# cxy1997/3D_adapt_auto_driving

Hardware: AMD Instinct MI355X
Metric: KITTI scenes/s end-to-end eval_rcnn (joint RPN+RCNN, synthetic 16384-pt scenes) (higher is better)
Workload: dtype f32; 1 GPU; BASELINE.json configs[2]: full PointRCNN RPN+RCNN inference, default.yaml shapes, random-init weights, batch=8 synthetic KITTI scenes x 16384 pts per GPU per step; scene=synth.scenes (SURVEY 8d: uniform clutter + ground + 10 dense cars), parallelism=scene-sharded x1, one final all_gather of detections, detections_gathered=652455, batch_slots=14, look_ahead=12, steps_per_launch=2

## Files before the change

3d_adapt_auto_driving_amd/csrc/layer_tile.hpp:

```cpp
#pragma once
#include "common.hpp"
#include "segmax.hpp"

namespace prcnn {

typedef float f32x4 __attribute__((ext_vector_type(4)));
constexpr int PL_ROWS = 64;
constexpr int PL_LD = 128 + 4;

constexpr int PL_MAX_BATCH = 4;
struct PLProblem {
    const unsigned int *hdr; long rows_host; int K, N; const float *A; long lda; const float *W; const float *bias; int do_relu;
    float *out; long ldo; const unsigned int *rowinfo; const int *tilecloud; int m, out_col, n_store;
    int lds_pool;
    const float *addG; const int *addIdx; const float *addW; int add_n, add_m; long add_ldg;
};
struct PLBatch { PLProblem p[PL_MAX_BATCH]; };

#define PL_LOAD_W(dst, kk)                                                                              \
    _Pragma("unroll") for (int s = 0; s < 64; ++s)                                                      \
        dst[s] = __uint_as_float(__builtin_amdgcn_raw_buffer_load_b32(wrs, lane_off, (unsigned int)((kk) + s) * row_bytes, 0));
#define PL_VM_DRAIN __builtin_amdgcn_s_waitcnt(0x0F70);
#define PL_SADD(x, y) asm volatile("s_add_u32 %0, %0, %1" : "+s"(x) : "s"(y) : "scc");

#define PL_FETCH_TILE(T, NI, soff)                                                                      \
    _Pragma("unroll") for (int i = 0; i < (NI); ++i)                                                    \
        *reinterpret_cast<f32x4 *>((T) + (r0 + 8 * i) * PL_LD + 4 * chunk) = __builtin_bit_cast(        \
            f32x4, __builtin_amdgcn_raw_buffer_load_b128(ars, a_lane, (soff) + (unsigned int)(8 * i) * a_row_bytes, 0));

#define PL_BOTH_HALVES(...) __VA_ARGS__
#define PL_ONE_HALF(...)
#define PL_MFMA(H2, wf, c, s)                                                                           \
    acc0 = __builtin_amdgcn_mfma_f32_32x32x2f32(a0.c, wf[4 * g + s], acc0, 0, 0, 0);                    \
    H2(acc1 = __builtin_amdgcn_mfma_f32_32x32x2f32(a1.c, wf[4 * g + s], acc1, 0, 0, 0);)
#define PL_STAGE_HEAD(T, H2)                                                                            \
    const float *a0p = (T) + j * PL_LD + 64 * h;                                                        \
    H2(const float *a1p = (T) + (32 + j) * PL_LD + 64 * h;)                                             \
    f32x4 a0 = *reinterpret_cast<const f32x4 *>(a0p);                                                   \
    H2(f32x4 a1 = *reinterpret_cast<const f32x4 *>(a1p);)
#define PL_STAGE_GROUPS(wf, H2, STATE, SIDE)                                                            \
    {                                                                                                   \
        STATE                                                                                           \
        _Pragma("unroll") for (int g = 0; g < 16; ++g) {                                                \
            f32x4 n0_ = a0;                                                                             \
            H2(f32x4 n1_ = a1;)                                                                         \
            if (g < 15) {                                                                               \
                n0_ = *reinterpret_cast<const f32x4 *>(a0p + 4 * (g + 1));                              \
                H2(n1_ = *reinterpret_cast<const f32x4 *>(a1p + 4 * (g + 1));)                          \
            }                                                                                           \
            __builtin_amdgcn_sched_barrier(0);                                                          \
            PL_MFMA(H2, wf, x, 0)                                                                       \
            SIDE                                                                                        \
            PL_MFMA(H2, wf, y, 1) PL_MFMA(H2, wf, z, 2) PL_MFMA(H2, wf, w, 3)                           \
            a0 = n0_;                                                                                   \
            H2(a1 = n1_;)                                                                               \
        }                                                                                               \
    }
#define PL_STAGE_SIDE(T, wf, STATE, SIDE) { PL_STAGE_HEAD(T, PL_BOTH_HALVES) PL_STAGE_GROUPS(wf, PL_BOTH_HALVES, STATE, SIDE) }
#define PL_FENCE __builtin_amdgcn_sched_barrier(0);
#define PL_NO_SIDE
#define PL_STAGE(T, wf) PL_STAGE_SIDE(T, wf, PL_NO_SIDE, PL_NO_SIDE)
#define PL_NEXT_PANEL_STATE(kn)                                                                         \
    f32x4 ar[8];                                                                                        \
    unsigned int wo_ = (unsigned int)(kn) * row_bytes;                                                  \
    unsigned int ao_ = (unsigned int)(kn) * 4u;                                                         \
    const unsigned int a8_ = 8u * a_row_bytes;
#define PL_NEXT_PANEL(TN, wn, ARS, LOFF)                                                                \
    if (g < 8) {                                                                                        \
        ar[g] = __builtin_bit_cast(f32x4, __builtin_amdgcn_raw_buffer_load_b128((ARS), a_lane, ao_, 0)); \
        PL_SADD(ao_, a8_)                                                                               \
    } else                                                                                              \
        *reinterpret_cast<f32x4 *>((TN) + (r0 + 8 * (g - 8)) * PL_LD + 4 * chunk) = ar[g - 8];          \
    _Pragma("unroll") for (int q = 0; q < 6; ++q)                                                       \
        if (6 * g + q < 64) {                                                                           \
            wn[6 * g + q] = __uint_as_float(__builtin_amdgcn_raw_buffer_load_b32(wrs, (LOFF), wo_, 0)); \
            PL_SADD(wo_, row_bytes)                                                                     \
        }                                                                                               \
    PL_FENCE
#define PL_STAGE_PREFETCH_X(T, TN, wf, wn, kn, ARS, LOFF) PL_STAGE_SIDE(T, wf, PL_NEXT_PANEL_STATE(kn), PL_NEXT_PANEL(TN, wn, ARS, LOFF))
#define PL_STAGE_PREFETCH(T, TN, wf, wn, kn) PL_STAGE_PREFETCH_X(T, TN, wf, wn, kn, ars, lane_off)
#define PL_NEXT_ROWS(TN, soff)                                                                          \
    if (g < 8)                                                                                          \
        ar[g] = __builtin_bit_cast(f32x4, __builtin_amdgcn_raw_buffer_load_b128(                        \
            ars, a_lane, (soff) + (unsigned int)(8 * g) * a_row_bytes, 0));                             \
    else                                                                                                \
        *reinterpret_cast<f32x4 *>((TN) + (r0 + 8 * (g - 8)) * PL_LD + 4 * chunk) = ar[g - 8];          \
    PL_FENCE
#define PL_STAGE_ROWS(T, TN, wf, soff) PL_STAGE_SIDE(T, wf, f32x4 ar[8];, PL_NEXT_ROWS(TN, soff))

#define PL32_NEXT_PANEL(TN, wn, kn)                                                                     \
    if (g < 4)                                                                                          \
        ar[g] = __builtin_bit_cast(f32x4, __builtin_amdgcn_raw_buffer_load_b128(                        \
            ars, a_lane, (unsigned int)(8 * g) * a_row_bytes + (unsigned int)(kn) * 4u, 0));            \
    else if (g >= 8 && g < 12)                                                                          \
        *reinterpret_cast<f32x4 *>((TN) + (r0 + 8 * (g - 8)) * PL_LD + 4 * chunk) = ar[g - 8];          \
    _Pragma("unroll") for (int q = 0; q < 6; ++q)                                                       \
        if (6 * g + q < 64)                                                                             \
            wn[6 * g + q] = __uint_as_float(__builtin_amdgcn_raw_buffer_load_b32(                       \
                wrs, lane_off, (unsigned int)((kn) + 6 * g + q) * row_bytes, 0));

__device__ __forceinline__ void pl_store_direct(const f32x16 &acc0, const f32x16 &acc1, float bcol, int do_relu, float *out, long ldo,
                                                long t, long rows, unsigned int col)
{
    const int h = (threadIdx.x & 63) >> 5;
    const long left = rows - t * PL_ROWS;
    const unsigned int o_row_bytes = (unsigned int)ldo * 4u;
    const __amdgpu_buffer_rsrc_t ors = __builtin_amdgcn_make_buffer_rsrc(
        (void *)(out + t * PL_ROWS * ldo), 0, (int)((left < PL_ROWS ? left : PL_ROWS) * (long)o_row_bytes), 0x00020000);
    const unsigned int o_lane = (unsigned int)(4 * h) * o_row_bytes + col * 4u;
#pragma unroll
    for (int r = 0; r < 16; ++r) {
        const unsigned int so = (unsigned int)((r & 3) + 8 * (r >> 2)) * o_row_bytes;
        const float v0 = acc0[r] + bcol, v1 = acc1[r] + bcol;
        __builtin_amdgcn_raw_buffer_store_b32(__float_as_uint(do_relu ? fmaxf(v0, 0.f) : v0), ors, o_lane, so, 0);
        __builtin_amdgcn_raw_buffer_store_b32(__float_as_uint(do_relu ? fmaxf(v1, 0.f) : v1), ors, o_lane, so + 32u * o_row_bytes, 0);
    }
}

template <int TR>
__device__ __forceinline__ void pl_store_rows(const float *tile, long t, long rows, int n0, const PLProblem &pb, bool with_add)
{
    const int chunk = threadIdx.x & 31, r0 = threadIdx.x >> 5;
    float *out = pb.out;
    const long ldo = pb.ldo;
    const int n_store = pb.n_store;
#pragma unroll
    for (int i = 0; i < TR / 8; ++i) {
        const int row = r0 + 8 * i;
        const long g = t * TR + row;
        if (g < rows) {
            const int c0 = n0 + 4 * chunk;
            float4 v = *reinterpret_cast<const float4 *>(tile + row * PL_LD + 4 * chunk);
            if (with_add) {
                const int *ix = pb.addIdx + g * 3;
                const float *wv = pb.addW + g * 3;
                const long cb = (g / pb.add_n) * (long)pb.add_m;
                const float4 g0 = *reinterpret_cast<const float4 *>(pb.addG + (cb + ix[0]) * pb.add_ldg + c0);
                const float4 g1 = *reinterpret_cast<const float4 *>(pb.addG + (cb + ix[1]) * pb.add_ldg + c0);
                const float4 g2 = *reinterpret_cast<const float4 *>(pb.addG + (cb + ix[2]) * pb.add_ldg + c0);
                const float w0 = wv[0], w1 = wv[1], w2 = wv[2];
                v.x = __fadd_rn(v.x, __fadd_rn(__fadd_rn(__fmul_rn(w0, g0.x), __fmul_rn(w1, g1.x)), __fmul_rn(w2, g2.x)));
                v.y = __fadd_rn(v.y, __fadd_rn(__fadd_rn(__fmul_rn(w0, g0.y), __fmul_rn(w1, g1.y)), __fmul_rn(w2, g2.y)));
                v.z = __fadd_rn(v.z, __fadd_rn(__fadd_rn(__fmul_rn(w0, g0.z), __fmul_rn(w1, g1.z)), __fmul_rn(w2, g2.z)));
                v.w = __fadd_rn(v.w, __fadd_rn(__fadd_rn(__fmul_rn(w0, g0.w), __fmul_rn(w1, g1.w)), __fmul_rn(w2, g2.w)));
                if (pb.do_relu) v = make_float4(fmaxf(v.x, 0.f), fmaxf(v.y, 0.f), fmaxf(v.z, 0.f), fmaxf(v.w, 0.f));
            }
            if (c0 + 4 <= n_store && (ldo & 3) == 0) {
                *reinterpret_cast<float4 *>(out + g * ldo + c0) = v;
            } else {
                const float e[4] = {v.x, v.y, v.z, v.w};
#pragma unroll
                for (int q = 0; q < 4; ++q)
                    if (c0 + q < n_store) out[g * ldo + c0 + q] = e[q];
            }
        }
    }
}

template <bool SEGMAX>
__device__ __forceinline__ void pl_epilogue(const f32x16 &acc0, const f32x16 &acc1, float *tile, int *ctr, long t, long rows, int n0,
                                            const PLProblem &pb)
{
    const int tid = threadIdx.x, lane = tid & 63, w = tid >> 6, j = lane & 31, h = lane >> 5;
    const int chunk = tid & 31;
    const float bcol = pb.bias[n0 + 32 * w + j];
    if constexpr (SEGMAX) {
        if (tid < PL_ROWS) {
            const unsigned int info = pb.rowinfo[t * PL_ROWS + tid];
            ctr[tid] = pb.tilecloud[t] * pb.m + (int)(info >> 16);
        }
        __syncthreads();
        const int myc = ctr[lane], prevc = ctr[lane ? lane - 1 : 0];
        const unsigned long long start = __ballot(lane == 0 || myc != prevc);
        if (!pb.lds_pool || __popcll(start) <= PK_LDS_MIN) {
            pk_segmented_max(acc0, acc1, ctr, start, h, pb.out, (int)pb.ldo, pb.out_col + n0 + 32 * w + j, bcol);
        } else {
            const float4 bias4 = *reinterpret_cast<const float4 *>(pb.bias + n0 + 4 * chunk);
            pk_park(acc0, acc1, tile, PL_LD, 32 * w + j, h);
            lds_barrier();
            pk_segmented_max_lds(tile, PL_LD, ctr, tid, pb.out, (int)pb.ldo, pb.out_col + n0, bias4);
        }
    } else {
        const bool with_add = pb.addG != nullptr;
        const int do_relu = pb.do_relu;
        __syncthreads();
#pragma unroll
        for (int r = 0; r < 16; ++r) {
            const int row = (r & 3) + 8 * (r >> 2) + 4 * h;
            const float v0 = acc0[r] + bcol, v1 = acc1[r] + bcol;
            tile[row * PL_LD + 32 * w + j] = (do_relu && !with_add) ? fmaxf(v0, 0.f) : v0;
            tile[(32 + row) * PL_LD + 32 * w + j] = (do_relu && !with_add) ? fmaxf(v1, 0.f) : v1;
        }
        __syncthreads();
        pl_store_rows<PL_ROWS>(tile, t, rows, n0, pb, with_add);
    }
}

}
```

3d_adapt_auto_driving_amd/csrc/packed_layer.hip:

```cpp
#include "layer_tile.hpp"
#include <cstdlib>

namespace prcnn {

#define PL_LOAD_A(dst, kk)                                                                              \
    _Pragma("unroll") for (int i = 0; i < 8; ++i) {                                                     \
        long g = t * PL_ROWS + r0 + 8 * i;                                                              \
        if (g >= rows) g = rows - 1;    \
        dst[i] = *reinterpret_cast<const f32x4 *>(pb.A + g * pb.lda + (kk) + 4 * chunk);               \
    }
#define PL_STORE_A(src)                                                                                 \
    _Pragma("unroll") for (int i = 0; i < 8; ++i)                                                       \
        *reinterpret_cast<f32x4 *>(tile + (r0 + 8 * i) * PL_LD + 4 * chunk) = src[i];

template <bool SEGMAX>
__global__ __launch_bounds__(256, 2) void packed_layer_kernel(const PLBatch bt)
{
    const PLProblem pb = bt.p[blockIdx.z];
    __shared__ float tile[PL_ROWS * PL_LD];
    __shared__ int ctr[PL_ROWS];
    const long t = blockIdx.x;
    const long rows = pb.hdr ? (long)pb.hdr[0] * PL_ROWS : pb.rows_host;
    const int n0 = blockIdx.y * 128;
    if (t * PL_ROWS >= rows || n0 >= pb.n_store) return;
    const int tid = threadIdx.x, lane = tid & 63, w = tid >> 6, j = lane & 31, h = lane >> 5;
    const int chunk = tid & 31, r0 = tid >> 5;
    const int K = pb.K, N = pb.N;
    f32x16 acc0 = {0}, acc1 = {0};
    const __amdgpu_buffer_rsrc_t wrs = __builtin_amdgcn_make_buffer_rsrc((void *)pb.W, 0, K * N * 4, 0x00020000);
    const unsigned int row_bytes = (unsigned int)N * 4u;
    const unsigned int lane_off = ((unsigned int)(64 * h) * (unsigned int)N + (unsigned int)(n0 + 32 * w + j)) * 4u;
    for (int k0 = 0; k0 < K; k0 += 128) {
        float wf[64];
        f32x4 ar[8];
        PL_LOAD_W(wf, k0)
        PL_LOAD_A(ar, k0)
        if (k0) __syncthreads();
        PL_STORE_A(ar)
        __syncthreads();
        PL_STAGE(tile, wf)
    }
    pl_epilogue<SEGMAX>(acc0, acc1, tile, ctr, t, rows, n0, pb);
}

template <bool SEGMAX>
__global__ __launch_bounds__(256, 2) void packed_layer_pipe_kernel(const PLBatch bt)
{
    const PLProblem pb = bt.p[blockIdx.z];
    __shared__ float tiles[2 * PL_ROWS * PL_LD];
    __shared__ int ctr[PL_ROWS];
    const long t = blockIdx.x;
    const long rows = pb.hdr ? (long)pb.hdr[0] * PL_ROWS : pb.rows_host;
    const int n0 = blockIdx.y * 128;
    if (t * PL_ROWS >= rows || n0 >= pb.n_store) return;
    const int tid = threadIdx.x, lane = tid & 63, j = lane & 31, h = lane >> 5;
    const int w = __builtin_amdgcn_readfirstlane(tid >> 6);
    const int chunk = tid & 31, r0 = tid >> 5;
    const int K = pb.K, N = pb.N;
    f32x16 acc0 = {0}, acc1 = {0};
    const __amdgpu_buffer_rsrc_t wrs = __builtin_amdgcn_make_buffer_rsrc((void *)pb.W, 0, K * N * 4, 0x00020000);
    const unsigned int row_bytes = (unsigned int)N * 4u;
    const unsigned int lane_off = ((unsigned int)(64 * h) * (unsigned int)N + (unsigned int)(n0 + 32 * w + j)) * 4u;
    const long left = rows - t * PL_ROWS;
    const unsigned int a_row_bytes = (unsigned int)pb.lda * 4u;
    const __amdgpu_buffer_rsrc_t ars = __builtin_amdgcn_make_buffer_rsrc(
        (void *)(pb.A + t * PL_ROWS * pb.lda), 0, (int)((left < PL_ROWS ? left : PL_ROWS) * (long)a_row_bytes), 0x00020000);
    const unsigned int a_lane = (unsigned int)r0 * a_row_bytes + 16u * chunk;
    float wa[64], wb[64];
    PL_LOAD_W(wa, 0)
    PL_FETCH_TILE(tiles, 8, 0)
    const int np = K >> 7;
    for (int p = 0; p < np; ++p) {
        PL_VM_DRAIN
        lds_barrier();
        const float *T = tiles + (p & 1) * (PL_ROWS * PL_LD);
        float *TN = tiles + ((p + 1) & 1) * (PL_ROWS * PL_LD);
        if (p + 1 < np) {
            PL_STAGE_PREFETCH(T, TN, wa, wb, (p + 1) * 128)
#pragma unroll
            for (int s = 0; s < 64; ++s) wa[s] = wb[s];
        } else {
            PL_STAGE(T, wa)
        }
    }
    if constexpr (!SEGMAX) {
        if (n0 + 128 <= pb.n_store && !pb.addG) {
            pl_store_direct(acc0, acc1, pb.bias[n0 + 32 * w + j], pb.do_relu, pb.out, pb.ldo, t, rows, (unsigned int)(n0 + 32 * w + j));
            return;
        }
    }
    pl_epilogue<SEGMAX>(acc0, acc1, tiles, ctr, t, rows, n0, pb);
}

template <bool ADD>
__global__ __launch_bounds__(256, 2) void packed_layer_persist_kernel(const PLProblem pb, unsigned int *__restrict__ ticket)
{
    __shared__ float tiles[2 * PL_ROWS * PL_LD];
    __shared__ unsigned int s_item[2];
    const int tid = threadIdx.x, lane = tid & 63, j = lane & 31, h = lane >> 5;
    const int w = __builtin_amdgcn_readfirstlane(tid >> 6);
    const int chunk = tid & 31, r0 = tid >> 5;
    const long rows = pb.rows_host;
    const int K = pb.K, N = pb.N;
    const unsigned int col_blocks = (unsigned int)(N >> 7);
    const unsigned int n_tiles = (unsigned int)((rows + PL_ROWS - 1) / PL_ROWS);
    const unsigned int n_items = n_tiles * col_blocks;
    const __amdgpu_buffer_rsrc_t wrs = __builtin_amdgcn_make_buffer_rsrc((void *)pb.W, 0, K * N * 4, 0x00020000);
    const unsigned int row_bytes = (unsigned int)N * 4u;
    const unsigned int a_row_bytes = (unsigned int)pb.lda * 4u;
    const unsigned int a_lane = (unsigned int)r0 * a_row_bytes + 16u * chunk;
    const int np = K >> 7;
    auto tile_rsrc = [&](unsigned int t) __attribute__((always_inline)) {
        const long left = rows - (long)t * PL_ROWS;
        return __builtin_amdgcn_make_buffer_rsrc((void *)(pb.A + (long)t * PL_ROWS * pb.lda), 0,
                                                 (int)((left < PL_ROWS ? left : PL_ROWS) * (long)a_row_bytes), 0x00020000);
    };
    auto loff = [&](unsigned int cb) __attribute__((always_inline)) {
        return ((unsigned int)(64 * h) * (unsigned int)N + (cb * 128u + (unsigned int)(32 * w + j))) * 4u;
    };
    unsigned int item = blockIdx.x;
    unsigned int t = item / col_blocks, cb = item - t * col_blocks;
    __amdgpu_buffer_rsrc_t ars = tile_rsrc(t);
    unsigned int lane_off = loff(cb);
    float wa[64], wb[64];
    PL_LOAD_W(wa, 0)
    PL_FETCH_TILE(tiles, 8, 0)
    int pp = 0;
    int slot = 1;
    PL_VM_DRAIN
    while (true) {
        f32x16 acc0 = {0}, acc1 = {0};
        unsigned int next = 0xffffffffu, tn = 0, cbn = 0, drawn = 0;
        const float bcol = pb.bias[(int)cb * 128 + 32 * w + j];
        for (int p = 0; p < np; ++p, ++pp) {
            if (p > 0) {
                PL_VM_DRAIN
                if (p == 1 && tid == 0) s_item[slot] = drawn;
            }
            lds_barrier();
            if (p == 0 && tid == 0) drawn = gridDim.x + atomicAdd(ticket, 1u);
            const float *T = tiles + (pp & 1) * (PL_ROWS * PL_LD);
            float *TN = tiles + ((pp + 1) & 1) * (PL_ROWS * PL_LD);
            if (p + 1 < np) {
                PL_STAGE_PREFETCH(T, TN, wa, wb, (p + 1) * 128)
#pragma unroll
                for (int s2 = 0; s2 < 64; ++s2) wa[s2] = wb[s2];
            } else {
                next = s_item[slot];
                if (next < n_items) {
                    tn = next / col_blocks; cbn = next - tn * col_blocks;
                    const __amdgpu_buffer_rsrc_t ars_n = tile_rsrc(tn);
                    const unsigned int loff_n = loff(cbn);
                    PL_STAGE_PREFETCH_X(T, TN, wa, wb, 0, ars_n, loff_n)
#pragma unroll
                    for (int s2 = 0; s2 < 64; ++s2) wa[s2] = wb[s2];
                    PL_VM_DRAIN
                } else {
                    PL_STAGE(T, wa)
                }
            }
        }
        if constexpr (ADD) {
            float *Tlast = tiles + ((pp - 1) & 1) * (PL_ROWS * PL_LD);
            pl_epilogue<false>(acc0, acc1, Tlast, nullptr, (long)t, rows, (int)cb * 128, pb);
            __syncthreads();
        } else {
            pl_store_direct(acc0, acc1, bcol, pb.do_relu, pb.out, pb.ldo, (long)t, rows, cb * 128u + (unsigned int)(32 * w + j));
        }
        if (next >= n_items) break;
        t = tn; cb = cbn;
        ars = tile_rsrc(t);
        lane_off = loff(cb);
        slot ^= 1;
    }
    if (tid == 0) ticket_release(ticket);
}

__global__ __launch_bounds__(256, 2) void packed_layer_stream_kernel(const PLProblem pb)
{
    __shared__ float tiles[2 * PL_ROWS * PL_LD];
    const int tid = threadIdx.x, lane = tid & 63, j = lane & 31, h = lane >> 5;
    const int w = __builtin_amdgcn_readfirstlane(tid >> 6);
    const int chunk = tid & 31, r0 = tid >> 5;
    const int n0 = blockIdx.y * 128;
    const long rows = pb.rows_host;
    const int N = pb.N;
    const long ntiles = (rows + PL_ROWS - 1) / PL_ROWS;
    long t = blockIdx.x;
    if (t >= ntiles || n0 >= pb.n_store) return;
    const __amdgpu_buffer_rsrc_t wrs = __builtin_amdgcn_make_buffer_rsrc((void *)pb.W, 0, 128 * N * 4, 0x00020000);
    const unsigned int row_bytes = (unsigned int)N * 4u;
    const unsigned int lane_off = ((unsigned int)(64 * h) * (unsigned int)N + (unsigned int)(n0 + 32 * w + j)) * 4u;
    float wf[64];
    PL_LOAD_W(wf, 0)
    const unsigned int a_row_bytes = (unsigned int)pb.lda * 4u;
    const __amdgpu_buffer_rsrc_t ars = __builtin_amdgcn_make_buffer_rsrc((void *)pb.A, 0, (int)(rows * (long)a_row_bytes), 0x00020000);
    const unsigned int a_lane = (unsigned int)r0 * a_row_bytes + 16u * chunk;
    PL_FETCH_TILE(tiles, 8, (unsigned int)(t * PL_ROWS) * a_row_bytes)
    const float bcol = pb.bias[n0 + 32 * w + j];
    const bool direct = n0 + 128 <= pb.n_store && !pb.addG;
    PL_VM_DRAIN
    for (int it = 0;; ++it) {
        lds_barrier();
        float *T = tiles + (it & 1) * (PL_ROWS * PL_LD);
        float *TN = tiles + ((it + 1) & 1) * (PL_ROWS * PL_LD);
        const long tn = t + gridDim.x;
        f32x16 acc0 = {0}, acc1 = {0};
        if (tn < ntiles) {
            const unsigned int soff = (unsigned int)(tn * PL_ROWS) * a_row_bytes;
            PL_STAGE_ROWS(T, TN, wf, soff)
        } else {
            PL_STAGE(T, wf)
        }
        if (direct) {
            pl_store_direct(acc0, acc1, bcol, pb.do_relu, pb.out, pb.ldo, t, rows, (unsigned int)(n0 + 32 * w + j));
        } else {
            pl_epilogue<false>(acc0, acc1, T, nullptr, t, rows, n0, pb);
            __syncthreads();
        }
        if (tn >= ntiles) break;
        t = tn;
    }
}

__global__ __launch_bounds__(256, 2) void packed_layer_pipe32_kernel(const PLBatch bt)
{
    const PLProblem pb = bt.p[blockIdx.z];
    const long rows = pb.rows_host;
    const int K = pb.K, N = pb.N;
    constexpr int R = 32;
    __shared__ float tiles[2 * R * PL_LD];
    const long t = blockIdx.x;
    const int n0 = blockIdx.y * 128;
    if (t * R >= rows || n0 >= pb.n_store) return;
    const int tid = threadIdx.x, lane = tid & 63, j = lane & 31, h = lane >> 5;
    const int w = __builtin_amdgcn_readfirstlane(tid >> 6);
    const int chunk = tid & 31, r0 = tid >> 5;
    f32x16 acc0 = {0};
    const __amdgpu_buffer_rsrc_t wrs = __builtin_amdgcn_make_buffer_rsrc((void *)pb.W, 0, K * N * 4, 0x00020000);
    const unsigned int row_bytes = (unsigned int)N * 4u;
    const unsigned int lane_off = ((unsigned int)(64 * h) * (unsigned int)N + (unsigned int)(n0 + 32 * w + j)) * 4u;
    const long left = rows - t * R;
    const unsigned int a_row_bytes = (unsigned int)pb.lda * 4u;
    const __amdgpu_buffer_rsrc_t ars =
        __builtin_amdgcn_make_buffer_rsrc((void *)(pb.A + t * R * pb.lda), 0, (int)((left < R ? left : R) * (long)a_row_bytes), 0x00020000);
    const unsigned int a_lane = (unsigned int)r0 * a_row_bytes + 16u * chunk;
    float wa[64], wb[64];
    PL_LOAD_W(wa, 0)
    PL_FETCH_TILE(tiles, R / 8, 0)
    const int np = K >> 7;
    for (int p = 0; p < np; ++p) {
        PL_VM_DRAIN
        lds_barrier();
        const float *T = tiles + (p & 1) * (R * PL_LD);
        float *TN = tiles + ((p + 1) & 1) * (R * PL_LD);
        PL_STAGE_HEAD(T, PL_ONE_HALF)
        if (p + 1 < np) {
            PL_STAGE_GROUPS(wa, PL_ONE_HALF, f32x4 ar[4];, PL32_NEXT_PANEL(TN, wb, (p + 1) * 128) PL_FENCE)
#pragma unroll
            for (int s = 0; s < 64; ++s) wa[s] = wb[s];
        } else {
            PL_STAGE_GROUPS(wa, PL_ONE_HALF, PL_NO_SIDE, PL_FENCE)
        }
    }
    const float bcol = pb.bias[n0 + 32 * w + j];
    const int do_relu = pb.do_relu;
    __syncthreads();
#pragma unroll
    for (int r = 0; r < 16; ++r) {
        const float v = acc0[r] + bcol;
        tiles[((r & 3) + 8 * (r >> 2) + 4 * h) * PL_LD + 32 * w + j] = do_relu ? fmaxf(v, 0.f) : v;
    }
    __syncthreads();
    pl_store_rows<R>(tiles, t, rows, n0, pb, false);
}

}

using namespace prcnn;

namespace {
enum PLForm { PL_ONE, PL_PIPE, PL_PIPE32, PL_STREAM, PL_PERSIST };
struct PLPlan { PLForm form; long gx; int gy; };
long env_long(const char *v, long dflt) { return v ? atol(v) : dflt; }

PLPlan pl_plan(const PLProblem &p, long tiles, bool segmax, bool single)
{
    static const long stream_min = env_long(getenv("PRCNN_PL_STREAM_MIN"), 512), stream_cap = env_long(getenv("PRCNN_PL_STREAM_CAP"), 512),
                      persist_min = env_long(getenv("PRCNN_PL_PERSIST_MIN"), 256);
    const int col_blocks = (p.n_store + 127) / 128;
    const long items = tiles * col_blocks;
    const bool host_plain = !p.hdr && !segmax;
    if (p.K == 128) {
        if (host_plain && items >= stream_min && p.rows_host * p.lda * 4 < (1L << 31)) {
            const long cap = stream_cap / col_blocks > 0 ? stream_cap / col_blocks : 1;
            return {PL_STREAM, tiles < cap ? tiles : cap, col_blocks};
        }
        return {PL_ONE, tiles, col_blocks};
    }
    if (host_plain && !p.addG && items < 256) return {PL_PIPE32, (p.rows_host + 31) / 32, col_blocks};
    if (host_plain && single && p.n_store == p.N && items > stream_cap && items >= persist_min)
        return {PL_PERSIST, items < stream_cap ? items : stream_cap, 1};
    return {PL_PIPE, tiles, col_blocks};
}

int pl_launch(PLForm form, const PLBatch &bt, int k, long gx, int gy, bool segmax, hipStream_t st, const char *what)
{
    const dim3 grid((unsigned)gx, gy, k), wg(256);
    switch (form) {
    case PL_ONE:
        if (segmax) hipLaunchKernelGGL(packed_layer_kernel<true>, grid, wg, 0, st, bt);
        else hipLaunchKernelGGL(packed_layer_kernel<false>, grid, wg, 0, st, bt);
        break;
    case PL_PIPE:
        if (segmax) hipLaunchKernelGGL(packed_layer_pipe_kernel<true>, grid, wg, 0, st, bt);
        else hipLaunchKernelGGL(packed_layer_pipe_kernel<false>, grid, wg, 0, st, bt);
        break;
    case PL_PIPE32: hipLaunchKernelGGL(packed_layer_pipe32_kernel, grid, wg, 0, st, bt); break;
    case PL_STREAM: hipLaunchKernelGGL(packed_layer_stream_kernel, grid, wg, 0, st, bt.p[0]); break;
    case PL_PERSIST: {
        unsigned int *ticket = next_ticket(st);
        if (!ticket) { set_error("%s: cannot set up the item ticket", what); return PRCNN_ELAUNCH; }
        if (bt.p[0].addG) hipLaunchKernelGGL(packed_layer_persist_kernel<true>, grid, wg, 0, st, bt.p[0], ticket);
        else hipLaunchKernelGGL(packed_layer_persist_kernel<false>, grid, wg, 0, st, bt.p[0], ticket);
        break;
    }
    }
    return check_launch(what);
}

PLProblem pl_problem(const prcnn_layer_problem &q, bool segmax)
{
    PLProblem p = {};
    p.hdr = q.hdr; p.rows_host = q.rows; p.K = q.K; p.N = q.N; p.A = q.A; p.lda = q.lda; p.W = q.W; p.bias = q.bias;
    p.do_relu = segmax ? 1 : q.relu; p.out = q.out; p.ldo = q.ldo; p.n_store = segmax ? q.N : q.n_store;
    if (segmax) {
        p.rowinfo = q.rowinfo; p.tilecloud = q.tilecloud; p.m = q.m; p.out_col = q.out_col;
        p.lds_pool = (((uintptr_t)q.out | (uintptr_t)q.bias) & 15) == 0 && (q.ldo & 3) == 0 && (q.out_col & 3) == 0;
    }
    return p;
}
}

extern "C" int prcnn_packed_layer_batch(int nprob, const prcnn_layer_problem *pr, int segmax, void *stream)
{
    PRCNN_REQUIRE(nprob >= 0 && nprob <= PL_MAX_BATCH && (nprob == 0 || pr), "packed_layer: 0..%d problems", PL_MAX_BATCH);
    hipStream_t st = (hipStream_t)stream;
    const char *what = segmax ? "packed_layer_segmax" : "packed_layer";
    PLBatch bt;
    long tiles_of[PL_MAX_BATCH];
    int k = 0;
    for (int i = 0; i < nprob; ++i) {
        const prcnn_layer_problem &q = pr[i];
        PRCNN_REQUIRE(q.K > 0 && q.N > 0 && q.K % 128 == 0 && q.N % 128 == 0, "packed_layer: K=%d, N=%d must be multiples of 128", q.K, q.N);
        PRCNN_REQUIRE(q.lda >= q.K && q.lda % 4 == 0, "packed_layer: bad leading dimension of A");
        long tiles;
        if (segmax) {
            PRCNN_REQUIRE(q.b >= 0 && q.m >= 0 && q.max_tiles >= 0 && q.out_col >= 0 && q.ldo >= q.out_col + q.N, "packed_layer_segmax: bad layout");
            if ((long)q.b * q.m == 0) continue;
            PRCNN_REQUIRE(q.A && q.W && q.bias && q.rowinfo && q.tilecloud && q.hdr && q.out, "packed_layer_segmax: null pointer");
            PRCNN_REQUIRE(((uintptr_t)q.A & 15) == 0 && q.max_tiles <= 0x7fffffffL, "packed_layer_segmax: alignment / size");
            if (!q.out_is_zero && hipMemset2DAsync(q.out + q.out_col, (size_t)q.ldo * sizeof(float), 0, (size_t)q.N * sizeof(float),
                                                    (size_t)q.b * q.m, st) != hipSuccess) {
                set_error("packed_layer_segmax: cannot zero the output slice");
                return PRCNN_ELAUNCH;
            }
            tiles = q.max_tiles;
        } else {
            PRCNN_REQUIRE(q.n_store >= 1 && q.n_store <= q.N && q.ldo >= q.n_store, "packed_layer: n_store=%d outside 1..N (or ldo too small)", q.n_store);
            tiles = q.hdr ? q.max_tiles : (q.rows + PL_ROWS - 1) / PL_ROWS;
            PRCNN_REQUIRE(tiles >= 0 && tiles <= 0x7fffffffL && q.rows >= 0, "packed_layer: bad row count");
            if (tiles > 0) {
                PRCNN_REQUIRE(q.A && q.W && q.bias && q.out, "packed_layer: null pointer");
                PRCNN_REQUIRE(((uintptr_t)q.A & 15) == 0 && (((uintptr_t)q.out & 15) == 0 || (q.ldo & 3) != 0), "packed_layer: 16-byte alignment required");
            }
        }
        if (tiles == 0) continue;
        tiles_of[k] = tiles;
        bt.p[k++] = pl_problem(q, segmax);
    }
    if (k == 0) return PRCNN_OK;
    PLPlan plan[PL_MAX_BATCH];
    bool together = true;
    long gx = 0;
    int gy = 0;
    for (int i = 0; i < k; ++i) {
        plan[i] = pl_plan(bt.p[i], tiles_of[i], segmax, k == 1);
        together = together && plan[i].form == plan[0].form && (plan[i].form == PL_ONE || plan[i].form == PL_PIPE || plan[i].form == PL_PIPE32);
        if (plan[i].gx > gx) gx = plan[i].gx;
        if (plan[i].gy > gy) gy = plan[i].gy;
    }
    if (together || k == 1) return pl_launch(plan[0].form, bt, k, gx, gy, segmax, st, what);
    for (int i = 0; i < k; ++i) {
        PLBatch one;
        one.p[0] = bt.p[i];
        const int rc = pl_launch(plan[i].form, one, 1, plan[i].gx, plan[i].gy, segmax, st, what);
        if (rc != PRCNN_OK) return rc;
    }
    return PRCNN_OK;
}

extern "C" int prcnn_packed_layer(const unsigned int *hdr, long rows, long max_tiles, int K, int N, int n_store, const float *A,
                                  long lda, const float *W, const float *bias, int relu, float *out, long ldo, void *stream)
{
    prcnn_layer_problem q = {};
    q.hdr = hdr; q.rows = rows; q.max_tiles = max_tiles; q.K = K; q.N = N; q.n_store = n_store; q.A = A; q.lda = lda; q.W = W;
    q.bias = bias; q.relu = relu; q.out = out; q.ldo = ldo;
    return prcnn_packed_layer_batch(1, &q, 0, stream);
}

extern "C" int prcnn_packed_layer_segmax(int b, int m, long max_tiles, int K, int N, const float *A, long lda, const float *W,
                                         const float *bias, const unsigned int *rowinfo, const int *tilecloud,
                                         const unsigned int *hdr, float *out, int out_stride, int out_col, int out_is_zero, void *stream)
{
    prcnn_layer_problem q = {};
    q.hdr = hdr; q.max_tiles = max_tiles; q.K = K; q.N = N; q.n_store = N; q.A = A; q.lda = lda; q.W = W; q.bias = bias; q.relu = 1;
    q.out = out; q.ldo = out_stride; q.b = b; q.m = m; q.rowinfo = rowinfo; q.tilecloud = tilecloud; q.out_col = out_col;
    q.out_is_zero = out_is_zero;
    return prcnn_packed_layer_batch(1, &q, 1, stream);
}


extern "C" int prcnn_packed_layer_interp(long rows, int K, int N, const float *A, long lda, const float *W, const float *bias, int relu,
                                         float *out, long ldo, int n_per_cloud, int m_known, const float *G, long ldg, const int *idx,
                                         const float *weight, void *stream)
{
    PRCNN_REQUIRE(rows >= 0 && K > 0 && N > 0 && K % 128 == 0 && N % 128 == 0, "packed_layer_interp: K=%d, N=%d must be multiples of 128", K, N);
    PRCNN_REQUIRE(lda >= K && lda % 4 == 0 && ldo >= N && ldo % 4 == 0 && ldg >= N && ldg % 4 == 0, "packed_layer_interp: bad leading dimensions");
    PRCNN_REQUIRE(n_per_cloud >= 1 && m_known >= 1 && rows % n_per_cloud == 0, "packed_layer_interp: rows must be whole clouds");
    if (rows == 0) return PRCNN_OK;
    PRCNN_REQUIRE(A && W && bias && out && G && idx && weight, "packed_layer_interp: null pointer");
    PRCNN_REQUIRE((((uintptr_t)A | (uintptr_t)out | (uintptr_t)G) & 15) == 0, "packed_layer_interp: 16-byte alignment required");
    const long tiles = (rows + PL_ROWS - 1) / PL_ROWS;
    PRCNN_REQUIRE(tiles <= 0x7fffffffL, "packed_layer_interp: too many rows");
    prcnn_layer_problem q = {};
    q.rows = rows; q.K = K; q.N = N; q.n_store = N; q.A = A; q.lda = lda; q.W = W; q.bias = bias; q.relu = relu; q.out = out; q.ldo = ldo;
    PLBatch bt;
    PLProblem &p = bt.p[0] = pl_problem(q, false);
    p.addG = G; p.addIdx = idx; p.addW = weight; p.add_n = n_per_cloud; p.add_m = m_known; p.add_ldg = ldg;
    const PLPlan plan = pl_plan(p, tiles, false, true);
    return pl_launch(plan.form, bt, 1, plan.gx, plan.gy, false, (hipStream_t)stream, "packed_layer_interp");
}
```

3d_adapt_auto_driving_amd/csrc/sa_wide.hpp:

```cpp
#pragma once
#include "common.hpp"

namespace prcnn {

typedef float f32x4 __attribute__((ext_vector_type(4)));

constexpr int SW_R = 32;
constexpr int SW_LD = 128 + 4;
constexpr int SW_PANEL = SW_R * SW_LD;

__device__ __forceinline__ void sw_segmented_max(const f32x16 &acc, const int *ctr, unsigned int start, int h, float *__restrict__ out,
                                                 int out_stride, int col, float bias)
{
    auto rowof = [](int q) { return (q & 3) + 8 * (q >> 2); };
    auto upto = [](int row) { return row >= 31 ? 0xffffffffu : ((2u << row) - 1u); };
    auto flush = [&](int row, float v) {
        atomicMax(reinterpret_cast<int *>(out + (long)ctr[row] * out_stride + col), __float_as_int(fmaxf(v + bias, 0.f)));
    };
    float cur = acc[0];
#pragma unroll
    for (int q = 1; q < 16; ++q) {
        const float v = acc[q];
        const int prev = rowof(q - 1), row = rowof(q);
        const unsigned int m0 = upto(row) & ~upto(prev), m1 = upto(row + 4) & ~upto(prev + 4);
        const bool b0 = (start & m0) != 0, b1 = (start & m1) != 0;
        if (b0 | b1) {
            if (h ? b1 : b0) {
                flush(prev + 4 * h, cur);
                cur = v;
            } else {
                cur = fmax_raw(cur, v);
            }
        } else {
            cur = fmax_raw(cur, v);
        }
    }
    flush(rowof(15) + 4 * h, cur);
}

#define SW_VM_DRAIN __builtin_amdgcn_s_waitcnt(0x0F70);
#define SW_STAGE(T, wf, wn, RS, VOFF, SOFF, RB, FIRST)                                                    \
    {                                                                                                     \
        const float *ap = (T) + j * SW_LD + 64 * h;                                                       \
        f32x4 a = *reinterpret_cast<const f32x4 *>(ap);                                                   \
        _Pragma("unroll") for (int g = 0; g < 16; ++g) {                                                  \
            f32x4 nx = a;                                                                                 \
            if (g < 15) nx = *reinterpret_cast<const f32x4 *>(ap + 4 * (g + 1));                          \
            __builtin_amdgcn_sched_barrier(0);                                                            \
            if ((FIRST) && g == 0) {                                                                      \
                const f32x16 zero = {0};                                                                  \
                acc = __builtin_amdgcn_mfma_f32_32x32x2f32(a.x, wf[0], zero, 0, 0, 0);                    \
            } else {                                                                                      \
                acc = __builtin_amdgcn_mfma_f32_32x32x2f32(a.x, wf[4 * g + 0], acc, 0, 0, 0);             \
            }                                                                                             \
            _Pragma("unroll") for (int q = 0; q < 6; ++q)       \
                if (6 * g + q < 64)                                                                       \
                    wn[6 * g + q] = __uint_as_float(__builtin_amdgcn_raw_buffer_load_b32(                 \
                        RS, VOFF, (SOFF) + (unsigned int)(6 * g + q) * (RB), 0));                         \
            __builtin_amdgcn_sched_barrier(0);                                                            \
            acc = __builtin_amdgcn_mfma_f32_32x32x2f32(a.y, wf[4 * g + 1], acc, 0, 0, 0);                 \
            acc = __builtin_amdgcn_mfma_f32_32x32x2f32(a.z, wf[4 * g + 2], acc, 0, 0, 0);                 \
            acc = __builtin_amdgcn_mfma_f32_32x32x2f32(a.w, wf[4 * g + 3], acc, 0, 0, 0);                 \
            a = nx;                                                                                       \
        }                                                                                                 \
    }

}
```

3d_adapt_auto_driving_amd/csrc/sa_wide3.hip:

```cpp
#include <hip/hip_runtime.h>

#include "common.hpp"
#include "sa_wide.hpp"
#include "../../include/prcnn_hip.h"

namespace prcnn {

struct SaWide3Args {
    int n, m, c0, c1, c2, c3;
    const unsigned int *hdr;
    const float4 *rowdxyz;
    const float *F;
    const float *wxyz;
    const unsigned int *rowinfo;
    const int *tilecloud;
    const float *wcat;
    const float *b1, *b2, *b3;
    float *out;
    int out_stride, out_col;
    unsigned int *ticket;
};

struct S3Stage {
    int layer, nb, kp, kpn;
    unsigned int rb, soff;
};

__global__ __launch_bounds__(256, 2) void sa_wide3_kernel(const SaWide3Args a)
{
    extern __shared__ __align__(16) float sw_lds[];
    const int kp0 = a.c0 >> 7, kp1 = a.c1 >> 7, kp2 = a.c2 >> 7, nb3 = a.c3 >> 7;
    const int kx = kp0 > kp2 ? kp0 : kp2;
    float *X = sw_lds;
    float *A1 = sw_lds + kx * SW_PANEL;
    float4 *s_d = reinterpret_cast<float4 *>(A1 + kp1 * SW_PANEL);
    int *ctr = reinterpret_cast<int *>(s_d + SW_R);
    unsigned int *slot = reinterpret_cast<unsigned int *>(ctr + SW_R);
    float *sb1 = reinterpret_cast<float *>(slot + 2), *sb2 = sb1 + a.c1, *sb3 = sb2 + a.c2, *swx = sb3 + a.c3;
    const int tid = threadIdx.x, lane = tid & 63, j = lane & 31, h = lane >> 5;
    const int w = __builtin_amdgcn_readfirstlane(tid >> 6);
    const int chunk = tid & 31, r0 = tid >> 5;
    const bool rowcloud = a.tilecloud == nullptr;
    const long nrows = (long)a.hdr[1];
    const long units = rowcloud ? (nrows + 31) >> 5 : 2L * (long)a.hdr[0];
    const long last_row = rowcloud ? nrows - 1 : 0x7fffffffffffL;
    const int ns1 = kp0 * kp1, ns2 = kp1 * kp2, ns = ns1 + ns2 + kp2 * nb3;
    const unsigned int o2 = (unsigned int)(a.c0 * a.c1) * 4u, o3 = o2 + (unsigned int)(a.c1 * a.c2) * 4u;
    const unsigned int total = o3 + (unsigned int)(a.c2 * a.c3) * 4u;
    const __amdgpu_buffer_rsrc_t rs = __builtin_amdgcn_make_buffer_rsrc((void *)a.wcat, 0, (int)total, 0x00020000);
    const unsigned int lane_k = (unsigned int)(64 * h), lane_c = (unsigned int)(32 * w + j) * 4u;
    const unsigned int voff1 = lane_k * (unsigned int)a.c1 * 4u + lane_c, voff2 = lane_k * (unsigned int)a.c2 * 4u + lane_c,
                       voff3 = lane_k * (unsigned int)a.c3 * 4u + lane_c;
    const float4 *F4 = reinterpret_cast<const float4 *>(a.F);
    const int q0 = a.c0 >> 2;

    auto stage_of = [&](int sc) __attribute__((always_inline)) {
        S3Stage st;
        int si;
        unsigned int base;
        if (sc < ns1) { st.layer = 0; st.kpn = kp0; si = sc; st.rb = (unsigned int)a.c1 * 4u; base = 0u; }
        else if (sc < ns1 + ns2) { st.layer = 1; st.kpn = kp1; si = sc - ns1; st.rb = (unsigned int)a.c2 * 4u; base = o2; }
        else { st.layer = 2; st.kpn = kp2; si = sc - ns1 - ns2; st.rb = (unsigned int)a.c3 * 4u; base = o3; }
        st.nb = si / st.kpn;
        st.kp = si - st.nb * st.kpn;
        st.soff = base + (unsigned int)(st.kp * 128) * st.rb + (unsigned int)st.nb * 512u;
        return st;
    };

    if (tid == 0) slot[0] = atomicAdd(a.ticket, 1u);
    for (int i = tid; i < a.c1; i += 256) sb1[i] = a.b1[i];
    for (int i = tid; i < a.c2; i += 256) sb2[i] = a.b2[i];
    for (int i = tid; i < a.c3; i += 256) sb3[i] = a.b3[i];
    for (int i = tid; i < 3 * a.c1; i += 256) swx[i] = a.wxyz[i];
    __syncthreads();
    long u = __builtin_amdgcn_readfirstlane((int)slot[0]);
    if (u >= units) { if (tid == 0) ticket_release(a.ticket); return; }
    float wa[64], wb[64];
    f32x16 acc;
#pragma unroll
    for (int s = 0; s < 64; ++s) wa[s] = __uint_as_float(__builtin_amdgcn_raw_buffer_load_b32(rs, voff1, (unsigned int)s * (unsigned int)a.c1 * 4u, 0));

    for (unsigned int served = 0; u < units; ++served) {
        const long t = u >> 1;
        const long row0 = rowcloud ? u * 32 : t * 64 + 32 * (u & 1);
        {
            const int cloud = rowcloud ? 0 : a.tilecloud[t];
            unsigned int info[4];
            long prow[4];
#pragma unroll
            for (int i = 0; i < 4; ++i) {
                info[i] = a.rowinfo[min(row0 + r0 + 8 * i, last_row)];
                prow[i] = rowcloud ? (long)(info[i] >> 16) * a.n + (long)(info[i] & 0x1ffu) : (long)cloud * a.n + (long)(info[i] & 0xffffu);
            }
            if (tid == 0) slot[(served + 1) & 1] = atomicAdd(a.ticket, 1u);
            if (tid < SW_R) {
                const unsigned int wd = a.rowinfo[min(row0 + tid, last_row)];
                ctr[tid] = rowcloud ? (int)(wd >> 16) * a.m + (int)((wd >> 9) & 0x7fu) : cloud * a.m + (int)(wd >> 16);
                s_d[tid] = a.rowdxyz[min(row0 + tid, last_row)];
            }
            for (int pc = 0; pc < kp0; ++pc) {
                float4 v[4];
#pragma unroll
                for (int i = 0; i < 4; ++i) v[i] = F4[prow[i] * q0 + pc * 32 + chunk];
#pragma unroll
                for (int i = 0; i < 4; ++i) *reinterpret_cast<float4 *>(X + pc * SW_PANEL + (r0 + 8 * i) * SW_LD + 4 * chunk) = v[i];
            }
        }
        SW_VM_DRAIN
        lds_barrier();
        for (int s = 0; s < ns; s += 2) {
#pragma unroll
            for (int half = 0; half < 2; ++half) {
                const int sc = s + half;
                const S3Stage st = stage_of(sc);
                const S3Stage nst = stage_of(sc + 1 == ns ? 0 : sc + 1);
                const float *T = (st.layer == 0 ? X : (st.layer == 1 ? A1 : X)) + st.kp * SW_PANEL;
                const unsigned int voffn = nst.layer == 0 ? voff1 : (nst.layer == 1 ? voff2 : voff3);
                if (st.layer > 0 && st.kp == 0 && st.nb == 0) lds_barrier();
                if (half == 0) { SW_STAGE(T, wa, wb, rs, voffn, nst.soff, nst.rb, st.kp == 0) } else { SW_STAGE(T, wb, wa, rs, voffn, nst.soff, nst.rb, st.kp == 0) }
                SW_VM_DRAIN
                if (st.kp == st.kpn - 1) {
                    const int col = st.nb * 128 + 32 * w + j;
                    if (st.layer == 0) {
                        const float bcol = sb1[col], wxc = swx[col], wyc = swx[a.c1 + col], wzc = swx[2 * a.c1 + col];
                        float *Y = A1 + st.nb * SW_PANEL;
#pragma unroll
                        for (int r = 0; r < 16; ++r) {
                            const int row = (r & 3) + 8 * (r >> 2) + 4 * h;
                            const float4 d = s_d[row];
                            const float p = acc[r] + bcol;
                            Y[row * SW_LD + 32 * w + j] = fmaxf(fmaf(wzc, d.z, fmaf(wyc, d.y, fmaf(wxc, d.x, p))), 0.f);
                        }
                    } else if (st.layer == 1) {
                        const float bcol = sb2[col];
                        float *Y = X + st.nb * SW_PANEL;
#pragma unroll
                        for (int r = 0; r < 16; ++r) Y[((r & 3) + 8 * (r >> 2) + 4 * h) * SW_LD + 32 * w + j] = fmaxf(acc[r] + bcol, 0.f);
                    } else {
                        const int myc = ctr[j], prevc = ctr[j ? j - 1 : 0];
                        const unsigned int start = (unsigned int)__ballot(lane < 32 && (lane == 0 || myc != prevc));
                        sw_segmented_max(acc, ctr, start, h, a.out, a.out_stride, a.out_col + col, sb3[col]);
                    }
                }
            }
        }
        const long un = __builtin_amdgcn_readfirstlane((int)slot[(served + 1) & 1]);
        lds_barrier();
        u = un;
    }
    if (tid == 0) ticket_release(a.ticket);
}

}

using namespace prcnn;

static size_t sa_wide3_lds(int c0, int c1, int c2, int c3)
{
    const int kp0 = c0 / 128, kp1 = c1 / 128, kp2 = c2 / 128;
    return (size_t)((kp0 > kp2 ? kp0 : kp2) + kp1) * SW_PANEL * sizeof(float) + SW_R * sizeof(float4) + SW_R * sizeof(int) +
           2 * sizeof(unsigned int) + (size_t)(c1 + c2 + c3 + 3 * c1) * sizeof(float);
}

extern "C" int prcnn_sa_wide_fused3_supported(int c0, int c1, int c2, int c3)
{
    if (c0 <= 0 || c1 <= 0 || c2 <= 0 || c3 <= 0 || c0 % 128 || c1 % 128 || c2 % 128 || c3 % 128) return 0;
    const int kp0 = c0 / 128, kp1 = c1 / 128, kp2 = c2 / 128, nb3 = c3 / 128;
    if ((kp0 * kp1 + kp1 * kp2 + kp2 * nb3) % 2) return 0;
    return sa_wide3_lds(c0, c1, c2, c3) <= 96 * 1024 ? 1 : 0;
}

extern "C" int prcnn_sa_wide_fused3(int b, int n, int m, int c0, int c1, int c2, int c3, long max_tiles, const float *F, const float *wxyz,
                                    const unsigned int *rowinfo, const float *rowdxyz, const int *tilecloud, const unsigned int *hdr,
                                    const float *wcat, const float *b1, const float *b2, const float *b3, float *out, int out_stride,
                                    int out_col, int out_is_zero, void *stream)
{
    PRCNN_REQUIRE(b >= 0 && n >= 0 && m >= 0 && max_tiles >= 0, "sa_wide_fused3: bad sizes");
    PRCNN_REQUIRE(prcnn_sa_wide_fused3_supported(c0, c1, c2, c3), "sa_wide_fused3: unsupported widths %d-%d-%d-%d", c0, c1, c2, c3);
    PRCNN_REQUIRE(n <= 65536 && m <= 65536, "sa_wide_fused3: cloud too large for the 16-bit row descriptors");
    PRCNN_REQUIRE(out_stride >= out_col + c3 && out_col >= 0, "sa_wide_fused3: bad output slice");
    if ((long)b * m == 0) return PRCNN_OK;
    PRCNN_REQUIRE(F && wxyz && rowinfo && rowdxyz && hdr && wcat && b1 && b2 && b3 && out, "sa_wide_fused3: null pointer");
    PRCNN_REQUIRE(tilecloud || (n <= 512 && m <= 128 && b <= 65536), "sa_wide_fused3: a list without tilecloud holds clouds of <= 512 points, <= 128 centres");
    PRCNN_REQUIRE((((uintptr_t)F | (uintptr_t)wcat | (uintptr_t)rowdxyz) & 15) == 0, "sa_wide_fused3: 16-byte alignment required");
    hipStream_t st = (hipStream_t)stream;
    if (!out_is_zero && hipMemset2DAsync(out + out_col, (size_t)out_stride * sizeof(float), 0, (size_t)c3 * sizeof(float), (size_t)b * m, st) != hipSuccess) {
        set_error("sa_wide_fused3: cannot zero the output slice");
        return PRCNN_ELAUNCH;
    }
    if (max_tiles == 0) return PRCNN_OK;
    const size_t lds = sa_wide3_lds(c0, c1, c2, c3);
    const int rc = ensure_dynamic_lds((const void *)sa_wide3_kernel, lds, "sa_wide_fused3");
    if (rc != PRCNN_OK) return rc;
    SaWide3Args a;
    a.n = n; a.m = m; a.c0 = c0; a.c1 = c1; a.c2 = c2; a.c3 = c3; a.hdr = hdr; a.rowdxyz = (const float4 *)rowdxyz; a.F = F; a.wxyz = wxyz;
    a.rowinfo = rowinfo; a.tilecloud = tilecloud; a.wcat = wcat; a.b1 = b1; a.b2 = b2; a.b3 = b3; a.out = out; a.out_stride = out_stride;
    a.out_col = out_col;
    a.ticket = next_ticket(st);
    if (!a.ticket) { set_error("sa_wide_fused3: cannot set up the unit ticket"); return PRCNN_ELAUNCH; }
    const long units = 2 * max_tiles;
    const long grid = units < mfma_grid_cap() ? units : mfma_grid_cap();
    hipLaunchKernelGGL(sa_wide3_kernel, dim3((unsigned)grid), dim3(256), lds, st, a);
    return check_launch("sa_wide_fused3");
}
```

3d_adapt_auto_driving_amd/dropin/pointnet2_cuda.py:

```python
import ctypes
import importlib
import os
import sys

import torch

_pkg_dir = os.path.dirname(os.path.dirname(os.path.abspath(__file__)))
if os.path.dirname(_pkg_dir) not in sys.path:
    sys.path.insert(0, os.path.dirname(_pkg_dir))
_lib = importlib.import_module(os.path.basename(_pkg_dir) + "._lib")
IS_HIP_EXTENSION = True


def _chk(dtype, *tensors):
    for t in tensors:
        if not t.is_cuda:
            raise RuntimeError("pointnet2_cuda: tensor must be a CUDA tensor")
        if not t.is_contiguous():
            raise RuntimeError("pointnet2_cuda: tensor must be contiguous")
        if t.dtype != dtype:
            raise RuntimeError("pointnet2_cuda: expected %s, got %s" % (dtype, t.dtype))


def ball_query_wrapper(b, n, m, radius, nsample, new_xyz, xyz, idx):
# ... 287 lines not shown
                                    group_all=False, hdr_c1=None, centre_rows=False):
    _chk(torch.float32, xyz); _chk(torch.int32, limit)
    b, n, _ = xyz.shape
    dev = xyz.device
    new1 = torch.empty((b, m1, 3), dtype=torch.float32, device=dev)
    if want_idx:
        idx1 = torch.empty((b, m1, ns1), dtype=torch.int32, device=dev)
        idx2 = torch.empty((b, m2, ns2), dtype=torch.int32, device=dev)
    else:
        idx1 = torch.empty((b, m1, ns1), dtype=torch.int32, device="meta")
        idx2 = torch.empty((b, m2, ns2), dtype=torch.int32, device="meta")
    rep1 = torch.empty((b, m1), dtype=torch.int32, device=dev)
    new2 = torch.empty((b, m2, 3), dtype=torch.float32, device=dev)
    rep2 = torch.empty((b, m2), dtype=torch.int32, device=dev)
    if (hdr1 is None) != (hdr2 is None):
        raise ValueError("rcnn_roi_geometry_packs: both headers or none")
    packs = []
    for idx, lim_, rep_, crep_, hdr in ((idx1, limit, None, rep1, hdr1), (idx2, None, rep1, rep2, hdr2)):
        m, ns = idx.shape[1], idx.shape[2]
        cap = (m * ns + 63) // 64
        pk = BallPack()
        pk.idx, pk.limit, pk.rep, pk.crep = idx, lim_, rep_, crep_
        pk.rowinfo = torch.empty((b * cap * 64,), dtype=torch.int32, device=dev)
        pk.rowdxyz = torch.empty((b * cap * 64, 4), dtype=torch.float32, device=dev)
        pk.tilecloud = None if row_clouds else torch.empty((b * cap,), dtype=torch.int32, device=dev)
        pk.max_tiles = b * cap
        if hdr is not None:
            _chk(torch.int32, hdr)
            if hdr.numel() != 4:
                raise ValueError("rcnn_roi_geometry_packs: a header must hold 4 int32")
        pk.hdr = hdr if hdr is not None else torch.empty((4,), dtype=torch.int32, device=dev)
        packs.append(pk)
    p1, p2 = packs
    p3 = None
    if group_all:
        if not row_clouds or (hdr3 is None) != (hdr1 is None):
            raise ValueError("rcnn_roi_geometry_packs: the GroupAll list comes in the row-carried form, its header like the others")
        p3 = BallPack()
        key = (m2, str(dev))
        if key not in _ARANGE:
            _ARANGE[key] = torch.arange(m2, dtype=torch.int32, device=dev)
        p3.idx = _ARANGE[key].view(1, 1, m2).expand(b, 1, m2)
        p3.limit, p3.rep, p3.crep = None, rep2, None
        p3.rowinfo = torch.empty((b * m2,), dtype=torch.int32, device=dev)
        p3.rowdxyz = torch.empty((b * m2, 4), dtype=torch.float32, device=dev)
        p3.tilecloud = None
        p3.max_tiles = (b * m2 + 63) // 64
        if hdr3 is not None:
            _chk(torch.int32, hdr3)
        p3.hdr = hdr3 if hdr3 is not None else torch.empty((4,), dtype=torch.int32, device=dev)
    crows = None
    if centre_rows:
        if (hdr_c1 is None) != (hdr1 is None):
            raise ValueError("rcnn_roi_geometry_packs: the centre rows' header comes like the others")
        if hdr_c1 is not None:
            _chk(torch.int32, hdr_c1)
        crows = (torch.empty((b * m1,), dtype=torch.int32, device=dev), hdr_c1 if hdr_c1 is not None else torch.empty((4,), dtype=torch.int32, device=dev))
    _lib.call("prcnn_rcnn_roi_geometry_packs", b, n, m1, float(r1), ns1, m2, float(r2), ns2, xyz.data_ptr(), limit.data_ptr(), new1.data_ptr(),
              idx1.data_ptr() if want_idx else None, rep1.data_ptr(), new2.data_ptr(), idx2.data_ptr() if want_idx else None, rep2.data_ptr(),
              p1.rowinfo.data_ptr(), p1.rowdxyz.data_ptr(), _lib.ptr(p1.tilecloud), p1.hdr.data_ptr(),
              p2.rowinfo.data_ptr(), p2.rowdxyz.data_ptr(), _lib.ptr(p2.tilecloud), p2.hdr.data_ptr(),
              None if p3 is None else p3.rowinfo.data_ptr(), None if p3 is None else p3.rowdxyz.data_ptr(),
              None if p3 is None else p3.hdr.data_ptr(), None if crows is None else crows[0].data_ptr(),
              None if crows is None else crows[1].data_ptr(), 1 if hdr1 is not None else 0, _lib.current_stream(xyz))
    return (new1, idx1, rep1, new2, idx2, rep2, p1, p2) + ((p3,) if p3 is not None else ()) + ((crows,) if crows is not None else ())


def dup_rep_wrapper(sel, n, limit=None, prev=None):
    _chk(torch.int32, sel)
    for t in (limit, prev):
        if t is not None:
            _chk(torch.int32, t)
    b, m = sel.shape
    rep = torch.empty((b, m), dtype=torch.int32, device=sel.device)
    _lib.call("prcnn_dup_rep", b, n, m, sel.data_ptr(), _lib.ptr(limit), _lib.ptr(prev), rep.data_ptr(), _lib.current_stream(sel))
    return rep


def ball_pack_groups_wrapper(idx, xyz, new_xyz, group, hdr=None):
    _chk(torch.int32, idx); _chk(torch.float32, xyz, new_xyz)
    b, m, ns = idx.shape
    if group < 1 or b % group:
        raise ValueError("ball_pack_groups: %d clouds do not split into lists of %d" % (b, group))
    lists, cap = b // group, (m * ns + 63) // 64
    L = group * cap
    rowinfo = torch.empty((lists, L * 64), dtype=torch.int32, device=idx.device)
    rowdxyz = torch.empty((lists, L * 64, 4), dtype=torch.float32, device=idx.device)
    tilecloud = torch.empty((lists, L), dtype=torch.int32, device=idx.device)
    if hdr is not None:
        _chk(torch.int32, hdr)
        if tuple(hdr.shape) != (lists, 4):
            raise ValueError("ball_pack_groups: hdr must be (lists, 4)")
        _lib.call("prcnn_ball_pack_ex", b, group, xyz.size(1), m, ns, idx.data_ptr(), None, None, None, xyz.data_ptr(), new_xyz.data_ptr(),
                  rowinfo.data_ptr(), rowdxyz.data_ptr(), tilecloud.data_ptr(), hdr.data_ptr(), 1, _lib.current_stream(idx))
    else:
        hdr = torch.empty((lists, 4), dtype=torch.int32, device=idx.device)
        _lib.call("prcnn_ball_pack_groups", b, group, xyz.size(1), m, ns, idx.data_ptr(), None, xyz.data_ptr(), new_xyz.data_ptr(),
                  rowinfo.data_ptr(), rowdxyz.data_ptr(), tilecloud.data_ptr(), hdr.data_ptr(), _lib.current_stream(idx))
    out = []
    for l in range(lists):
        pk = BallPack()
        pk.idx, pk.limit, pk.rep, pk.crep = idx[l * group:(l + 1) * group], None, None, None
        pk.rowinfo, pk.rowdxyz, pk.tilecloud, pk.hdr, pk.max_tiles = rowinfo[l], rowdxyz[l], tilecloud[l], hdr[l], L
        out.append(pk)
    return out


def sa_packed_mlp_wrapper(new_xyz, xyz, P, wxyz, pack, w2t, b2, w3t, b3, out, out_col, zeroed=False):
    _chk(torch.float32, new_xyz, xyz, P, wxyz, w2t, b2, w3t, b3, out)
    b, n, c1 = P.shape
    if c1 != 128 or w2t.shape != (128, 128) or w3t.size(0) != 128:
        raise RuntimeError("pointnet2_cuda: sa_packed_mlp needs 128-wide (zero-padded) layers 1 and 2")
    _lib.call("prcnn_sa_packed_mlp", b, n, new_xyz.size(1), w3t.size(1), pack.max_tiles,
              P.data_ptr(), wxyz.data_ptr(), pack.rowinfo.data_ptr(), pack.rowdxyz.data_ptr(), _lib.ptr(pack.tilecloud), pack.hdr.data_ptr(),
              w2t.data_ptr(), b2.data_ptr(), w3t.data_ptr(), b3.data_ptr(), out.data_ptr(), out.size(-1), out_col, int(zeroed),
              _lib.current_stream(xyz))
    return out


def sa_packed_mlp_batch_wrapper(problems):
    arr = (_lib.SaProblem * len(problems))()
    for q, prob in zip(arr, problems):
        new_xyz, xyz, P, wxyz, pack, w2t, b2, w3t, b3, out, out_col, zeroed = prob[:12]
        q.c1, q.c2 = (int(v) for v in prob[12]) if len(prob) > 12 and prob[12] is not None else (0, 0)
        _chk(torch.float32, new_xyz, xyz, wxyz, w2t, b2, w3t, b3, out)
        b, n, c1 = P.shape
        if c1 == 64:
            if not (P.is_cuda and P.dtype == torch.float32 and P.stride() == (n * 128, 128, 1) and P.data_ptr() % 16 == 0):
                raise RuntimeError("pointnet2_cuda: sa_packed_mlp_batch: a 64-wide P must be a column slice of a contiguous (b, n, 128) tensor")
            if not (len(problems) == 2 and all(len(pp) > 12 and pp[12] is not None and pp[12][0] == 64 and pp[12][1] in (64, 96) for pp in problems)):
                raise RuntimeError("pointnet2_cuda: sa_packed_mlp_batch: a 64-wide P needs two problems of real widths 64-64 / 64-96")
        else:
            _chk(torch.float32, P)
        if c1 not in (64, 128) or w2t.shape != (128, 128) or tuple(w3t.shape) != (128, 128):
            raise RuntimeError("pointnet2_cuda: sa_packed_mlp_batch takes 128-128-128 (zero-padded) problems")
        q.b, q.n, q.m, q.c3, q.max_tiles = b, n, new_xyz.size(1), 128, pack.max_tiles
        q.P, q.wxyz, q.rowinfo, q.rowdxyz = P.data_ptr(), wxyz.data_ptr(), pack.rowinfo.data_ptr(), pack.rowdxyz.data_ptr()
        q.tilecloud, q.hdr = pack.tilecloud.data_ptr(), pack.hdr.data_ptr()
        q.w2t, q.b2, q.w3t, q.b3 = w2t.data_ptr(), b2.data_ptr(), w3t.data_ptr(), b3.data_ptr()
        q.out, q.out_stride, q.out_col, q.out_is_zero = out.data_ptr(), out.size(-1), int(out_col), int(bool(zeroed))
    _lib.call("prcnn_sa_packed_mlp_batch", len(problems), arr, _lib.current_stream(problems[0][1]))
    return [p[9] for p in problems]


def packed_gather_affine_wrapper(new_xyz, xyz, P, wxyz, pack, out):
    _chk(torch.float32, new_xyz, xyz, P, wxyz, out)
    b, n, c1 = P.shape
    _lib.call("prcnn_packed_gather_affine", b, n, c1, pack.max_tiles,
              P.data_ptr(), wxyz.data_ptr(), pack.rowinfo.data_ptr(), pack.rowdxyz.data_ptr(), pack.tilecloud.data_ptr(), pack.hdr.data_ptr(),
              out.data_ptr(), _lib.current_stream(xyz))
    return out


def packed_layer_wrapper(a, wt, bias, relu, out, pack=None):
    _chk(torch.float32, wt, bias)
    for t in (a, out):
        if not t.is_cuda or t.dtype != torch.float32 or t.dim() != 2 or t.stride(1) != 1:
            raise RuntimeError("pointnet2_cuda: packed_layer expects 2-D float32 CUDA matrices with unit column stride")
    R, K = a.shape
    N = wt.size(1)
    n_store = out.size(1)
    if wt.size(0) != K or out.size(0) != R or n_store > N:
        raise RuntimeError("pointnet2_cuda: packed_layer shape mismatch")
    if pack is not None and pack.tilecloud is None:
        raise RuntimeError("pointnet2_cuda: packed_layer does not take a list whose rows carry their cloud (its tile count is not in hdr[0])")
    _lib.call("prcnn_packed_layer", None if pack is None else pack.hdr.data_ptr(), R, 0 if pack is None else pack.max_tiles,
              K, N, n_store, a.data_ptr(), a.stride(0), wt.data_ptr(), bias.data_ptr(), int(bool(relu)), out.data_ptr(), out.stride(0),
              _lib.current_stream(a))
    return out


_SPLIT_W = {}


def rows_layer_bf16x3_wrapper(a, wt, bias, relu, out):
    _chk(torch.float32, wt, bias)
    R, K = a.shape
    N = wt.size(1)
    key = (wt.data_ptr(), wt._version, K, N, str(wt.device))
    ws = _SPLIT_W.get(key)
    if ws is None:
        ws = torch.empty(((K // 16) * (N // 32) * 3 * 64 * 16,), dtype=torch.uint8, device=wt.device)
        _lib.call("prcnn_split_weights_bf16x3", K, N, wt.data_ptr(), ws.data_ptr(), _lib.current_stream(wt))
        _SPLIT_W[key] = ws
    _lib.call("prcnn_rows_layer_bf16x3", R, K, N, out.size(1), a.data_ptr(), a.stride(0), ws.data_ptr(), bias.data_ptr(), int(bool(relu)),
              out.data_ptr(), out.stride(0), _lib.current_stream(a))
    return out


def resplit_weights_bf16x3(tensors):
    done = 0
    for key in list(_SPLIT_W):
        ptr, _, K, N, dev = key
        for t in tensors:
            lo = t.data_ptr()
            if str(t.device) == dev and lo <= ptr and ptr + K * N * 4 <= lo + t.numel() * t.element_size():
                ws = _SPLIT_W.pop(key)
                _lib.call("prcnn_split_weights_bf16x3", K, N, ptr, ws.data_ptr(), _lib.current_stream(t))
                _SPLIT_W[(ptr, t._version, K, N, dev)] = ws
                done += 1
                break
    return done


def packed_layer_interp_wrapper(a, wt, bias, relu, out, G, idx, weight):
    _chk(torch.float32, wt, bias, G, weight)
    _chk(torch.int32, idx)
    for t in (a, out):
        if not t.is_cuda or t.dtype != torch.float32 or t.dim() != 2 or t.stride(1) != 1:
            raise RuntimeError("pointnet2_cuda: packed_layer_interp expects 2-D float32 CUDA matrices with unit column stride")
    R, K = a.shape
    N = wt.size(1)
    B, n = idx.shape[0], idx.shape[1]
    if wt.size(0) != K or tuple(out.shape) != (R, N) or R != B * n or G.shape[0] != B or G.shape[2] != N or tuple(weight.shape) != tuple(idx.shape):
        raise RuntimeError("pointnet2_cuda: packed_layer_interp shape mismatch")
    _lib.call("prcnn_packed_layer_interp", R, K, N, a.data_ptr(), a.stride(0), wt.data_ptr(), bias.data_ptr(), int(bool(relu)),
              out.data_ptr(), out.stride(0), n, G.shape[1], G.data_ptr(), G.stride(1), idx.data_ptr(), weight.data_ptr(),
              _lib.current_stream(a))
    return out


def sa_wide_fused_supported(c1, c2, c3):
    return bool(_lib.load().prcnn_sa_wide_fused_supported(int(c1), int(c2), int(c3)))


def sa_wide_fused_wrapper(new_xyz, xyz, P, wxyz, pack, w2t, b2, w3t, b3, out, out_col, zeroed=False):
    _chk(torch.float32, new_xyz, xyz, P, wxyz, w2t, b2, w3t, b3, out)
    b, n, c1 = P.shape
    if w2t.size(0) != c1 or w3t.size(0) != w2t.size(1) or wxyz.size(1) != c1:
        raise RuntimeError("pointnet2_cuda: sa_wide_fused shape mismatch")
    _lib.call("prcnn_sa_wide_fused", b, n, new_xyz.size(1), c1, w2t.size(1), w3t.size(1), pack.max_tiles, P.data_ptr(), wxyz.data_ptr(),
              pack.rowinfo.data_ptr(), pack.rowdxyz.data_ptr(), pack.tilecloud.data_ptr(), pack.hdr.data_ptr(), w2t.data_ptr(),
              b2.data_ptr(), w3t.data_ptr(), b3.data_ptr(), out.data_ptr(), out.size(-1), out_col, int(bool(zeroed)),
              _lib.current_stream(xyz))
    return out


def sa_wide_fused3_supported(c0, c1, c2, c3):
    return bool(_lib.load().prcnn_sa_wide_fused3_supported(int(c0), int(c1), int(c2), int(c3)))


def sa_wide_fused3_wrapper(new_xyz, xyz, feats, wcat, b1, wxyz, pack, b2, b3, widths, out, out_col, zeroed=False):
    _chk(torch.float32, new_xyz, xyz, feats, wcat, b1, wxyz, b2, b3, out)
    b, n, c0 = feats.shape
    c0w, c1, c2, c3 = (int(v) for v in widths)
    if c0 != c0w or wcat.numel() != c0 * c1 + c1 * c2 + c2 * c3 or wxyz.size(1) != c1 or b1.numel() != c1 or b2.numel() != c2 or b3.numel() != c3:
        raise RuntimeError("pointnet2_cuda: sa_wide_fused3 shape mismatch")
    _lib.call("prcnn_sa_wide_fused3", b, n, new_xyz.size(1), c0, c1, c2, c3, pack.max_tiles, feats.data_ptr(), wxyz.data_ptr(),
              pack.rowinfo.data_ptr(), pack.rowdxyz.data_ptr(), _lib.ptr(pack.tilecloud), pack.hdr.data_ptr(), wcat.data_ptr(),
              b1.data_ptr(), b2.data_ptr(), b3.data_ptr(), out.data_ptr(), out.size(-1), out_col, int(bool(zeroed)),
              _lib.current_stream(xyz))
    return out


def packed_gather_affine_batch_wrapper(problems):
    arr = (_lib.GatherProblem * len(problems))()
    for q, (new_xyz, xyz, P, wxyz, pack, out) in zip(arr, problems):
        _chk(torch.float32, new_xyz, xyz, P, wxyz, out)
        q.b, q.n, q.c1 = P.shape
        q.max_tiles = pack.max_tiles
        q.P, q.wxyz, q.out = P.data_ptr(), wxyz.data_ptr(), out.data_ptr()
        q.rowinfo, q.rowdxyz, q.tilecloud, q.hdr = pack.rowinfo.data_ptr(), pack.rowdxyz.data_ptr(), pack.tilecloud.data_ptr(), pack.hdr.data_ptr()
    _lib.call("prcnn_packed_gather_affine_batch", len(problems), arr, _lib.current_stream(problems[0][2]))
    return [p[5] for p in problems]


def packed_layer_batch_wrapper(problems):
    arr = (_lib.LayerProblem * len(problems))()
    for q, (a, wt, bias, relu, out, pack) in zip(arr, problems):
        _chk(torch.float32, wt, bias)
        if a.dim() != 2 or out.dim() != 2 or a.stride(1) != 1 or out.stride(1) != 1 or not a.is_cuda:
            raise RuntimeError("pointnet2_cuda: packed_layer expects 2-D float32 CUDA matrices with unit column stride")
        q.K, q.N = wt.shape
        q.n_store = out.size(1)
        q.A, q.lda, q.W, q.bias, q.relu = a.data_ptr(), a.stride(0), wt.data_ptr(), bias.data_ptr(), int(bool(relu))
        q.out, q.ldo = out.data_ptr(), out.stride(0)
        q.hdr, q.rows, q.max_tiles = (None, a.size(0), 0) if pack is None else (pack.hdr.data_ptr(), 0, pack.max_tiles)
    _lib.call("prcnn_packed_layer_batch", len(problems), arr, 0, _lib.current_stream(problems[0][0]))
    return [p[4] for p in problems]


def packed_layer_segmax_batch_wrapper(problems):
    arr = (_lib.LayerProblem * len(problems))()
    for q, (a, wt, bias, pack, b, m, out, out_col, zeroed) in zip(arr, problems):
        _chk(torch.float32, a, wt, bias, out)
        q.K, q.N = wt.shape
        q.n_store = q.N
        q.A, q.lda, q.W, q.bias, q.relu = a.data_ptr(), a.stride(0), wt.data_ptr(), bias.data_ptr(), 1
        q.out, q.ldo, q.out_col, q.out_is_zero = out.data_ptr(), out.size(-1), out_col, int(bool(zeroed))
        q.b, q.m = b, m
        q.hdr, q.max_tiles, q.rowinfo, q.tilecloud = pack.hdr.data_ptr(), pack.max_tiles, pack.rowinfo.data_ptr(), pack.tilecloud.data_ptr()
    _lib.call("prcnn_packed_layer_batch", len(problems), arr, 1, _lib.current_stream(problems[0][0]))
    return [p[6] for p in problems]


def rows_dot_wrapper(a, wt, bias, out):
    _chk(torch.float32, wt, bias)
    if a.dim() != 2 or a.stride(1) != 1 or out.stride(1) != 1 or not a.is_cuda:
        raise RuntimeError("pointnet2_cuda: rows_dot expects 2-D float32 CUDA matrices with unit column stride")
    _lib.call("prcnn_rows_dot", a.size(0), a.size(1), wt.size(1), a.data_ptr(), a.stride(0), wt.data_ptr(), bias.data_ptr(),
              out.data_ptr(), out.stride(0), _lib.current_stream(a))
    return out


def rpn_tail_wrapper(known, idx, weight, wcat, bcat, wc2, bc2, feats, cls, reg):
    _chk(torch.float32, known, weight, wcat, bcat, wc2, bc2, feats, cls, reg); _chk(torch.int32, idx)
    b, m, c = known.shape
    if c != 256 or tuple(wcat.shape) != (768, 128) or tuple(bcat.shape) != (5, 128) or wc2.numel() != 128 or feats.size(-1) != 128:
        raise RuntimeError("pointnet2_cuda: rpn_tail is written for 256 interpolated channels and 128-wide layers")
    _lib.call("prcnn_rpn_tail", b, idx.size(1), m, known.data_ptr(), idx.data_ptr(), weight.data_ptr(), wcat.data_ptr(),
              bcat.data_ptr(), wc2.data_ptr(), bc2.data_ptr(), reg.size(-1), feats.data_ptr(), cls.data_ptr(), reg.data_ptr(),
              _lib.current_stream(known))
    return feats, cls, reg


def rpn_tail_lin_wrapper(G, idx, weight, wcat, bcat, wc2, bc2, feats, cls, reg):
    _chk(torch.float32, G, weight, wcat, bcat, wc2, bc2, feats, cls, reg); _chk(torch.int32, idx)
    b, m, c = G.shape
    if c != 128 or tuple(wcat.shape) != (512, 128) or tuple(bcat.shape) != (5, 128) or wc2.numel() != 128 or feats.size(-1) != 128:
        raise RuntimeError("pointnet2_cuda: rpn_tail_lin is written for a 128-wide coarse product and 128-wide layers")
    _lib.call("prcnn_rpn_tail_lin", b, idx.size(1), m, G.data_ptr(), idx.data_ptr(), weight.data_ptr(), wcat.data_ptr(),
              bcat.data_ptr(), wc2.data_ptr(), bc2.data_ptr(), reg.size(-1), feats.data_ptr(), cls.data_ptr(), reg.data_ptr(),
              _lib.current_stream(G))
    return feats, cls, reg


def rpn_tail_boxes_supported(channels, loc_scope, loc_bin_size, num_head_bin, xz_fine):
    return bool(_lib.call("prcnn_rpn_tail_boxes_supported", int(channels), float(loc_scope), float(loc_bin_size), int(num_head_bin),
                          int(bool(xz_fine))))


def rpn_tail_lin_boxes_wrapper(G, idx, weight, wcat, bcat, wc2, bc2, n_reg, loc_scope, loc_bin_size, num_head_bin, xz_fine, anchor_size,
                               xyz, feats, cls, boxes):
    _chk(torch.float32, G, weight, wcat, bcat, wc2, bc2, feats, cls, boxes, xyz); _chk(torch.int32, idx)
    b, m, c = G.shape
    if c != 128 or tuple(wcat.shape) != (512, 128) or tuple(bcat.shape) != (5, 128) or wc2.numel() != 128 or feats.size(-1) != 128:
        raise RuntimeError("pointnet2_cuda: rpn_tail_lin is written for a 128-wide coarse product and 128-wide layers")
    if boxes.size(-1) != 7 or boxes.numel() != 7 * b * idx.size(1) or xyz.numel() != 3 * b * idx.size(1):
        raise RuntimeError("pointnet2_cuda: rpn_tail_lin_boxes wants xyz (b,n,3) and boxes (b,n,7)")
    anchor = (ctypes.c_float * 3)(*[float(v) for v in anchor_size])
    _lib.call("prcnn_rpn_tail_lin_boxes", b, idx.size(1), m, G.data_ptr(), idx.data_ptr(), weight.data_ptr(), wcat.data_ptr(),
              bcat.data_ptr(), wc2.data_ptr(), bc2.data_ptr(), int(n_reg), float(loc_scope), float(loc_bin_size), int(num_head_bin),
              int(bool(xz_fine)), ctypes.cast(anchor, ctypes.c_void_p), xyz.data_ptr(), feats.data_ptr(), cls.data_ptr(),
              boxes.data_ptr(), _lib.current_stream(G))
    return feats, cls, boxes


def selftest_fmod_two_pi(a):
    _chk(torch.float32, a)
    mine, lib = torch.empty_like(a), torch.empty_like(a)
    _lib.call("prcnn_selftest_fmod_two_pi", a.numel(), a.data_ptr(), mine.data_ptr(), lib.data_ptr(), _lib.current_stream(a))
    return mine, lib


def packed_layer_segmax_wrapper(a, wt, bias, pack, b, m, out, out_col, zeroed=False):
    _chk(torch.float32, a, wt, bias, out)
    K, N = wt.shape
    _lib.call("prcnn_packed_layer_segmax", b, m, pack.max_tiles, K, N, a.data_ptr(), a.stride(0), wt.data_ptr(), bias.data_ptr(),
              pack.rowinfo.data_ptr(), pack.tilecloud.data_ptr(), pack.hdr.data_ptr(), out.data_ptr(), out.size(-1), out_col, int(zeroed),
              _lib.current_stream(a))
    return out


def sa_xyz_mlp_supported(c1, c2, c3, nsample):
    return bool(_lib.load().prcnn_sa_xyz_mlp_supported(int(c1), int(c2), int(c3), int(nsample)))


def sa_xyz_mlp_wrapper(new_xyz, xyz, idx, w1, b1, w2, b2, w3, b3, out, out_col):
    _chk(torch.float32, new_xyz, xyz, w1, b1, w2, b2, w3, b3, out); _chk(torch.int32, idx)
    b, n, _ = xyz.shape
    _lib.call("prcnn_sa_xyz_mlp", b, n, idx.size(1), idx.size(2), w1.size(1), w2.size(1), w3.size(1),
              new_xyz.data_ptr(), xyz.data_ptr(), idx.data_ptr(), w1.data_ptr(), b1.data_ptr(), w2.data_ptr(),
              b2.data_ptr(), w3.data_ptr(), b3.data_ptr(), out.data_ptr(), out.size(-1), out_col,
              _lib.current_stream(xyz))
    return out


def pooled_tiles_wrapper(cnt, rows_per_cloud):
    _chk(torch.int32, cnt)
    clouds = cnt.numel()
    tilemap = torch.empty((max(1, clouds * (rows_per_cloud // 64)),), dtype=torch.int32, device=cnt.device)
    hdr = torch.empty((4,), dtype=torch.int32, device=cnt.device)
    _lib.call("prcnn_pooled_tiles", clouds, rows_per_cloud, cnt.data_ptr(), tilemap.data_ptr(), hdr.data_ptr(), _lib.current_stream(cnt))
    return tilemap, hdr


def pooled_rows_wrapper(cnt, rows_per_cloud, hdr=None):
    _chk(torch.int32, cnt)
    clouds = cnt.numel()
    rowmap = torch.empty((max(1, clouds * rows_per_cloud),), dtype=torch.int32, device=cnt.device)
    zero = hdr is not None
    if zero:
        _chk(torch.int32, hdr)
        if hdr.numel() != 4:
            raise ValueError("pooled_rows: hdr must hold 4 int32")
    else:
        hdr = torch.empty((4,), dtype=torch.int32, device=cnt.device)
    _lib.call("prcnn_pooled_rows", clouds, rows_per_cloud, cnt.data_ptr(), rowmap.data_ptr(), hdr.data_ptr(), int(zero), _lib.current_stream(cnt))
    return rowmap, hdr


def rcnn_point_mlp_rows_wrapper(rows, fcol, wu1, bu1, wu2, bu2, wm, bm, wp, bp, p, rowlist):
    _chk(torch.float32, rows, wu1, bu1, wu2, bu2, wm, bm, wp, bp, p)
    rowmap, hdr = rowlist
    _chk(torch.int32, rowmap, hdr)
    _lib.call("prcnn_rcnn_point_mlp_rows", rows.size(0), rows.size(1), int(fcol), rows.data_ptr(), wu1.data_ptr(), bu1.data_ptr(),
              wu2.data_ptr(), bu2.data_ptr(), wm.data_ptr(), bm.data_ptr(), wp.data_ptr(), bp.data_ptr(), p.data_ptr(),
              rowmap.data_ptr(), hdr.data_ptr(), _lib.current_stream(rows))
    return p


def sa_xyz_mlp_packed_wrapper(new_xyz, xyz, pack, w1, b1, w2, b2, w3, b3, out, out_col, zeroed=False):
    _chk(torch.float32, w1, b1, w2, b2, w3, b3, out)
    _lib.call("prcnn_sa_xyz_mlp_packed", new_xyz.size(0), new_xyz.size(1), w1.size(1), w2.size(1), w3.size(1), pack.max_tiles,
              pack.rowinfo.data_ptr(), pack.rowdxyz.data_ptr(), pack.tilecloud.data_ptr(), pack.hdr.data_ptr(), w1.data_ptr(),
              b1.data_ptr(), w2.data_ptr(), b2.data_ptr(), w3.data_ptr(), b3.data_ptr(), out.data_ptr(), out.size(-1), out_col,
              int(zeroed), _lib.current_stream(out))
    return out


def rcnn_point_mlp_wrapper(rows, fcol, wu1, bu1, wu2, bu2, wm, bm, wp, bp, xfeat, merged, p, tiles=None):
    _chk(torch.float32, rows, wu1, bu1, wu2, bu2, wm, bm, wp, bp, p)
    if (xfeat is None) != (merged is None):
        raise RuntimeError("pointnet2_cuda: rcnn_point_mlp takes xfeat and merged together or neither")
    if xfeat is not None:
        _chk(torch.float32, xfeat, merged)
    _lib.call("prcnn_rcnn_point_mlp", rows.size(0), rows.size(1), int(fcol), rows.data_ptr(), wu1.data_ptr(), bu1.data_ptr(),
              wu2.data_ptr(), bu2.data_ptr(), wm.data_ptr(), bm.data_ptr(), wp.data_ptr(), bp.data_ptr(), _lib.ptr(xfeat),
              _lib.ptr(merged), p.data_ptr(), None if tiles is None else tiles[0].data_ptr(),
              None if tiles is None else tiles[1].data_ptr(), _lib.current_stream(rows))
    return p


def rows_gemm128_rows_wrapper(a, wt, bias, relu, out, rowlist):
    if a.dim() != 2 or a.stride(1) != 1 or not a.is_cuda or a.dtype != torch.float32 or a.shape[1] != 128:
        raise RuntimeError("pointnet2_cuda: rows_gemm128_rows expects a 2-D float32 CUDA matrix of 128 columns with unit column stride")
    _chk(torch.float32, wt, bias, out)
    rowmap, hdr = rowlist
    _chk(torch.int32, rowmap, hdr)
    _lib.call("prcnn_rows_gemm128_rows", a.shape[0], a.data_ptr(), a.stride(0), 0, wt.data_ptr(), bias.data_ptr(), int(bool(relu)), out.data_ptr(),
              rowmap.data_ptr(), hdr.data_ptr(), _lib.current_stream(a))
    return out


def rows_gemm128_wrapper(a, wt, bias, relu, out=None):
    if a.dim() != 2 or a.stride(1) != 1 or not a.is_cuda or a.dtype != torch.float32:
        raise RuntimeError("pointnet2_cuda: rows_gemm128 expects a 2-D float32 CUDA matrix with unit column stride")
    _chk(torch.float32, wt, bias)
    R, K = a.shape
    if out is None:
        out = torch.empty((R, 128), dtype=torch.float32, device=a.device)
    ld = a.stride(0)
    off1 = a.data_ptr() + 128 * 4
    _lib.call("prcnn_rows_gemm128", R, K // 128, a.data_ptr(), ld, 0, off1 if K == 256 else None, ld, 0, wt.data_ptr(),
              bias.data_ptr(), int(bool(relu)), out.data_ptr(), _lib.current_stream(a))
    return out
```

3d_adapt_auto_driving_amd/net/fast_infer.py:

```python
import contextlib
import os
import typing

import torch

from ..pointnet2 import pointnet2_utils as pu
from ..pointnet2 import fused_mlp
from .._lib import has_entry
from .. import kitti_utils
from .. import roipool3d_utils
from .. import iou3d_utils


USE_ROIPOOL_CANONICAL = True
USE_RCNN_POINT_MLP = True
USE_XYZ_MLP = True
USE_PACKED = os.environ.get("PRCNN_NO_PACK") is None
USE_POOL_DEDUP = os.environ.get("PRCNN_NO_POOL_DEDUP") is None
NESTED_FPS_MAX_N = int(os.environ.get("PRCNN_NESTED_FPS", "4096"))
USE_POINT_LAYER = os.environ.get("PRCNN_LIB_GEMM") is None
PAD128 = USE_PACKED and USE_POINT_LAYER
USE_RPN_TAIL = os.environ.get("PRCNN_NO_RPN_TAIL") is None
USE_SCALE_BATCH = True
USE_SA_NARROW = True
USE_WIDE_FUSED = True
EARLY_LEVELS = int(os.environ.get("PRCNN_EARLY_LEVELS", "4"))
EARLY_FP = int(os.environ.get("PRCNN_EARLY_FP", "2"))
USE_FP_LINEAR = os.environ.get("PRCNN_NO_FP_LINEAR") is None


class ZeroArena:
    SIZES = {}

    def __init__(self, key, device):
        self.key, self.device = key, device
        self.used = 0
        self.parts = []
        total = ZeroArena.SIZES.get(key)
        self.buf = torch.zeros((total,), dtype=torch.float32, device=device) if total else None

    def take(self, shape, dtype=torch.float32):
        n = torch.Size(shape).numel()
        n4 = (n + 3) // 4 * 4
        if self.buf is None or self.used + n4 > self.buf.numel():
            self.used += n4
            part = torch.zeros(tuple(shape), dtype=dtype, device=self.device)
            self.parts.append(part)
            return part
        out = self.buf[self.used:self.used + n].view(dtype).view(tuple(shape))
        self.used += n4
        return out

    def done(self):
        if self.buf is None or self.used > self.buf.numel():
            ZeroArena.SIZES[self.key] = self.used

    def rezero(self):
        if self.buf is not None:
            self.buf.zero_()
        for part in self.parts:
            part.zero_()


def pl_ext():
    return iou3d_utils.iou3d_cuda


def _round4(c):
    return (c + 3) // 4 * 4


def _round128(c):
    return (c + 127) // 128 * 128


def _pad2(t, rows, cols):
    o = t.new_zeros((rows, cols))
    o[:t.shape[0], :t.shape[1]] = t
    return o.contiguous()


def _pad1(t, n):
    o = t.new_zeros((n,))
    o[:t.shape[0]] = t
    return o


USE_ROWS_GEMM128 = os.environ.get("PRCNN_ROWS_GEMM") is not None


_STRICT = [False]


def _lib_gemm_allowed():
    return (not _STRICT[0] or not USE_PACKED or not USE_POINT_LAYER or not USE_RCNN_POINT_MLP or not USE_POOL_DEDUP
            or not USE_ROIPOOL_CANONICAL or os.environ.get("PRCNN_ALLOW_LIB_GEMM") == "1")


def gemm_bias_act(a, wt, bias, relu):
    if (USE_ROWS_GEMM128 and a.is_cuda and wt.shape[1] == 128 and wt.shape[0] in (128, 256) and a.shape[1] == wt.shape[0]
            and a.shape[0] % 64 == 0 and a.shape[0] >= 4096 and a.stride(1) == 1 and a.stride(0) % 4 == 0
            and a.data_ptr() % 16 == 0):
        return pu.pointnet2.rows_gemm128_wrapper(a, wt, bias, relu)
    if a.is_cuda and not _lib_gemm_allowed():
        raise RuntimeError("FastPointRCNN: a %dx%d layer over %d rows would run on a GEMM library although no A/B switch selects one "
                           "(shape not covered by csrc/packed_layer.hip?); set PRCNN_ALLOW_LIB_GEMM=1 to permit it"
                           % (wt.shape[0], wt.shape[1], a.shape[0]))
    if relu:
        try:
            return torch._addmm_activation(bias, a, wt)
        except (AttributeError, RuntimeError):
            return torch.addmm(bias, a, wt).relu_()
    return torch.addmm(bias, a, wt)


SPLIT_BF16 = os.environ.get("PRCNN_SPLIT_BF16") == "1"


def point_layer(a, wt, bias, relu, n_out=None):
    K, N = wt.shape
    n_out = N if n_out is None else n_out
    if (USE_PACKED and K % 128 == 0 and N % 128 == 0 and a.dim() == 2 and a.shape[1] == K and a.stride(1) == 1
            and a.stride(0) % 4 == 0 and a.data_ptr() % 16 == 0):
        out = torch.empty((a.shape[0], n_out), dtype=torch.float32, device=a.device)
        if SPLIT_BF16 and getattr(pu.pointnet2, "IS_HIP_EXTENSION", False):
            return pu.pointnet2.rows_layer_bf16x3_wrapper(a, wt, bias, relu, out)
        return pu.pointnet2.packed_layer_wrapper(a, wt, bias, relu, out)
    y = gemm_bias_act(a, wt, bias, relu)
    return y if n_out == N else y[:, :n_out].contiguous()


PackedWeights = typing.NamedTuple("PackedWeights", [(name, torch.Tensor) for name in ("wf", "wx", "b1", "w2", "b2", "w3", "b3")])


class _Mlp:

    def __init__(self, layers, grouped_c=None, pad128=False, in_parts=None, pad_out=False):
        self.layers = []
        self.n_out = layers[-1][0].shape[0]
        self.split = self.packed = self.packed_widths = self.wide = self.wide_cat = self.narrow = None
        if pad128 and grouped_c is None:
            for i, (w, b, relu) in enumerate(layers):
                np_ = _round128(w.shape[0])
                if i == 0 and in_parts:
                    assert sum(in_parts) == w.shape[1]
                    wt = w.new_zeros((sum(_round128(c) for c in in_parts), np_))
                    src = dst = 0
                    for c in in_parts:
                        wt[dst:dst + c, :w.shape[0]] = w[:, src:src + c].t()
                        src, dst = src + c, dst + _round128(c)
                else:
                    wt = _pad2(w.t(), _round128(w.shape[1]), np_)
                self.layers.append((wt.contiguous(), _pad1(b, np_), relu))
            self.padded = not pad_out
            w, b, relu = layers[-1]
            if self.padded and w.shape[0] <= 4 and not relu:
                self.narrow = (_pad2(w.t(), _round128(w.shape[1]), w.shape[0]), b.clone())
            return
        self.padded = False
        for i, (w, b, relu) in enumerate(layers):
            if i == 0 and grouped_c is not None:
                c, c4 = grouped_c, _round4(grouped_c)
                wt = w.new_zeros((c4 + 4, w.shape[0]))
                if c:
                    wt[:c] = w[:, 3:3 + c].t()
                wt[c4:c4 + 3] = w[:, 0:3].t()
            else:
                k = w.shape[1]
                wt = w.new_zeros((_round4(k), w.shape[0]))
                wt[:k] = w.t()
            self.layers.append((wt.contiguous(), b.clone(), relu))

        if grouped_c is not None and grouped_c >= 32 and grouped_c % 4 == 0 and self.layers[0][2]:
            wt, b, _ = self.layers[0]
            c4 = _round4(grouped_c)
            self.split = (wt[:grouped_c].contiguous(), wt[c4:c4 + 3].contiguous(), b)
        if self.split is not None and len(self.layers) == 3 and all(l[2] for l in self.layers):
            wf, wx, b1 = self.split
            (w2, b2, _), (w3, b3, _) = self.layers[1], self.layers[2]
            c1, c2, c3 = wf.shape[1], w2.shape[1], w3.shape[1]
            kin = _round128(wf.shape[0]) if PAD128 else wf.shape[0]
            if c1 <= 128 and c2 <= 128 and c3 in (128, 256) and w2.shape[0] == c1 and w3.shape[0] == c2:
                self.packed = PackedWeights(_pad2(wf, kin, 128), _pad2(wx, 3, 128), _pad1(b1, 128),
                                            _pad2(w2, 128, 128), _pad1(b2, 128), _pad2(w3, 128, c3), b3)
                self.packed_widths = (c1, c2)
            elif c3 % 128 == 0 and w2.shape[0] == c1 and w3.shape[0] == c2:
                c1p, c2p = _round128(c1), _round128(c2)
                self.wide = PackedWeights(_pad2(wf, kin, c1p), _pad2(wx, 3, c1p), _pad1(b1, c1p),
                                          _pad2(w2, c1p, c2p), _pad1(b2, c2p), _pad2(w3, c2p, c3), b3)
                self.wide_cat = torch.cat([t.reshape(-1) for t in (self.wide.wf, self.wide.w2, self.wide.w3)]).contiguous()

    @property
    def out_width(self):
        return self.layers[-1][0].shape[1]

    @property
    def on_packed(self):
        return self.packed is not None or self.wide is not None

    def __call__(self, a, start=0):
        last = len(self.layers) - 1
        for i, (wt, b, relu) in enumerate(self.layers[start:], start):
            if USE_POINT_LAYER and i == last and self.narrow is not None and a.stride(1) == 1:
                out = torch.empty((a.shape[0], self.n_out), dtype=torch.float32, device=a.device)
                a = pu.pointnet2.rows_dot_wrapper(a, self.narrow[0], self.narrow[1], out)
            elif USE_POINT_LAYER:
                a = point_layer(a, wt, b, relu, self.n_out if (self.padded and i == last) else None)
            else:
                a = gemm_bias_act(a, wt, b, relu)
        return a


def _fold_shared_mlp(mlp, fresh=None):
    if fresh is None:
        layers = fused_mlp.folded_layers(mlp)
    else:
        if id(mlp) not in fresh:
            fresh[id(mlp)] = fused_mlp.fold_fresh(mlp)
        layers = fresh[id(mlp)]
    if layers is None:
        raise NotImplementedError("fast path: unsupported SharedMLP structure")
    return [(w, b, True) for w, b in layers]


def _fold_head(seq):
    out = []
    for block in seq:
        if isinstance(block, torch.nn.Dropout):
            continue
        fb = fused_mlp._fold_block(block)
        if fb is not None:
            out.append((fb[0], fb[1], True))
            continue
        names = [n for n, _ in block.named_children()]
        if names != ["conv"]:
            raise NotImplementedError("fast path: unsupported head block %s" % names)
        conv = block.conv
        w = conv.weight.detach().reshape(conv.out_channels, conv.in_channels)
        b = conv.bias.detach() if conv.bias is not None else w.new_zeros(conv.out_channels)
        out.append((w, b, False))
    return out


def _state_tensors(model):
    return list(model.parameters()) + list(model.buffers())


def _state_version(tensors):
    return sum(t._version for t in tensors)


def _state_shapes(model):
    return [(n, tuple(t.shape)) for n, t in list(model.named_parameters()) + list(model.named_buffers())]


def _mlp_tensors(name, mlp):
    out = []
    for i, (wt, b, _) in enumerate(mlp.layers):
        out += [("%s.layers[%d].w" % (name, i), wt), ("%s.layers[%d].b" % (name, i), b)]
    for form in ("split", "packed", "wide", "narrow"):
        for i, t in enumerate(getattr(mlp, form) or ()):
            out.append(("%s.%s[%d]" % (name, form, i), t))
    if mlp.wide_cat is not None:
        out.append((name + ".wide_cat", mlp.wide_cat))
    return out


class Scale(typing.NamedTuple):
    radius: float
    nsample: int
    mlp: _Mlp
    cin: int

    @property
    def on_packed(self):
        return self.mlp.on_packed or self.cin == 0


class SaLevel(typing.NamedTuple):
    npoint: int
    scales: list
    pcat: typing.Optional[tuple]

    @property
    def on_packed(self):
        return all(sc.on_packed for sc in self.scales)

    @property
    def columns(self):
        return [sum(sc.mlp.out_width for sc in self.scales[:j]) for j in range(len(self.scales))]

    @property
    def padded_width(self):
        width = sum(sc.mlp.out_width for sc in self.scales)
        return _round128(width) if PAD128 else width


class RcnnLevel(typing.NamedTuple):
    npoint: typing.Optional[int]
    radius: typing.Optional[float]
    nsample: typing.Optional[int]
    mlp: _Mlp
    cin: int


def _narrow_pair_weights(scales):
    pk = [sc.mlp.packed for sc in scales]
    if not (len(scales) == 2 and all(p is not None and p.w3.shape[1] == 128 for p in pk)
            and all(c1 == 64 and c2 in (64, 96) for c1, c2 in (sc.mlp.packed_widths for sc in scales))
            and pk[0].wf.shape[0] == pk[1].wf.shape[0] and pk[0].wf.shape[0] % 128 == 0):
        return None
    return (torch.cat([p.wf[:, :64] for p in pk], 1).contiguous(), torch.cat([p.b1[:64] for p in pk]).contiguous())


class FastPointRCNN:
    def __init__(self, model, cfg, _fresh=None):
        assert not model.training, "FastPointRCNN is an inference engine: call model.eval() first"
        if cfg.RCNN.ENABLED and cfg.RCNN.USE_INTENSITY:
            raise NotImplementedError("fast path: cfg.RCNN.USE_INTENSITY (reflectance as an RCNN input feature) is not covered")
        self.model, self.cfg = model, cfg
        self.in_feat = int(model.rpn.backbone_net.SA_modules[0].mlps[0][0].conv.in_channels) - 3
        self._state = _state_tensors(model)
        self._folded_at = _state_version(self._state)
        self._shapes = _state_shapes(model)
        rpn = model.rpn
        bb = rpn.backbone_net
        self.sa = []
        for sa in bb.SA_modules:
            cins = [mlp[0].conv.in_channels - 3 for mlp in sa.mlps]
            scales = [Scale(g.radius, g.nsample, _Mlp(_fold_shared_mlp(mlp, _fresh), grouped_c=cin), cin) for g, mlp, cin in zip(sa.groupers, sa.mlps, cins)]
            self.sa.append(SaLevel(sa.npoint, scales, _narrow_pair_weights(scales)))
        sa_w = [sum(sc.mlp.n_out for sc in level.scales) for level in self.sa]
        folded = [_fold_shared_mlp(fp.mlp, _fresh) for fp in bb.FP_modules]
        self.fp = []
        for k, lay in enumerate(folded):
            known = sa_w[-1] if k == len(folded) - 1 else folded[k + 1][-1][0].shape[0]
            skip = self.in_feat if k == 0 else sa_w[k - 1]
            self.fp.append(_Mlp(lay, pad128=PAD128, in_parts=[c for c in (known, skip) if c], pad_out=True))
        self.rpn_cls = _Mlp(_fold_head(rpn.rpn_cls_layer), pad128=PAD128)
        self.rpn_reg = _Mlp(_fold_head(rpn.rpn_reg_layer), pad128=PAD128)
        self.rpn_tail = self._fold_rpn_tail() if (USE_RPN_TAIL and PAD128 and USE_POINT_LAYER) else None
        self._zero_bias = self.rpn_cls.layers[0][0].new_zeros((max([1024] + [m.layers[0][0].shape[1] for m in self.fp]),))
        self._groupall = {}
        self._pm_ok = self._is_covered = None
        if cfg.RCNN.ENABLED:
            r = model.rcnn_net
            self.xyz_up = _Mlp(_fold_shared_mlp(r.xyz_up_layer, _fresh))
            self.merge_down = _Mlp(_fold_shared_mlp(r.merge_down_layer, _fresh))
            self.rcnn_sa = []
            for sa in r.SA_modules:
                mlp, g = sa.mlps[0], sa.groupers[0]
                cin = mlp[0].conv.in_channels - 3
                self.rcnn_sa.append(RcnnLevel(sa.npoint, getattr(g, "radius", None), getattr(g, "nsample", None),
                                              _Mlp(_fold_shared_mlp(mlp, _fresh), grouped_c=cin), cin))
            self.rcnn_cls = _Mlp(_fold_head(r.cls_layer), pad128=PAD128)
            self.rcnn_reg = _Mlp(_fold_head(r.reg_layer), pad128=PAD128)
            self.rcnn_head1 = None
            c0, r0 = self.rcnn_cls.layers[0], self.rcnn_reg.layers[0]
            if (USE_POINT_LAYER and USE_PACKED and len(self.rcnn_cls.layers) > 1 and len(self.rcnn_reg.layers) > 1 and c0[2] and r0[2] and
                    c0[0].shape == r0[0].shape and c0[0].shape[0] % 128 == 0 and c0[0].shape[1] % 128 == 0):
                self.rcnn_head1 = (torch.cat([c0[0], r0[0]], 1).contiguous(), torch.cat([c0[1], r0[1]]).contiguous(), c0[0].shape[1])

    def _covered(self):
        try:
            ok = bool(PAD128 and self.rpn_tail is not None) and all(level.on_packed for level in self.sa)
            if self.cfg.RCNN.ENABLED:
                ok = ok and self._point_mlp_ok() and all(level.mlp.on_packed for level in self.rcnn_sa)
            return ok
        except Exception:
            return False

    @contextlib.contextmanager
    def _strictly(self):
        if self._is_covered is None:
            self._is_covered = self._covered()
        prev, _STRICT[0] = _STRICT[0], bool(self._is_covered)
        try:
            yield
        finally:
            _STRICT[0] = prev

    def _fold_rpn_tail(self):
        fp0, cl, rg = self.fp[0], self.rpn_cls, self.rpn_reg
        shapes = lambda m: [tuple(l[0].shape) for l in m.layers]
        relus = lambda m: [bool(l[2]) for l in m.layers]
        if (shapes(fp0) != [(256, 128), (128, 128)] or relus(fp0) != [True, True] or
                shapes(cl) != [(128, 128), (128, 128)] or relus(cl) != [True, False] or cl.narrow is None or cl.n_out != 1 or
                shapes(rg) != [(128, 128), (128, 128)] or relus(rg) != [True, False] or rg.n_out % 4 or not 4 <= rg.n_out <= 128):
            return None
        mats = [fp0.layers[0], fp0.layers[1], cl.layers[0], rg.layers[0], rg.layers[1]]
        return {"wcat": torch.cat([m[0] for m in mats], dim=0).contiguous(), "bcat": torch.stack([m[1] for m in mats]).contiguous(),
                "wc2": cl.narrow[0].contiguous().view(-1), "bc2": cl.narrow[1].contiguous(), "n_reg": rg.n_out,
                "w1": mats[0][0].contiguous(), "wcat_lin": torch.cat([m[0] for m in mats[1:]], dim=0).contiguous(),
                "zero128": torch.zeros((128,), dtype=torch.float32, device=mats[0][0].device)}

    def check_weights(self):
        if _state_version(self._state) != self._folded_at:
            raise RuntimeError("FastPointRCNN: the model's parameters changed after the engine was built "
                               "(load the checkpoint first, then construct the engine / PipelinedRunner)")

    def weight_tensors(self):
        out = []
        for k, level in enumerate(self.sa):
            for j, sc in enumerate(level.scales):
                out += _mlp_tensors("sa[%d][%d]" % (k, j), sc.mlp)
        for k, m in enumerate(self.fp):
            out += _mlp_tensors("fp[%d]" % k, m)
        out += _mlp_tensors("rpn_cls", self.rpn_cls) + _mlp_tensors("rpn_reg", self.rpn_reg)
        out += [("rpn_tail[%s]" % key, self.rpn_tail[key]) for key in ("wcat", "bcat", "wc2", "bc2", "w1", "wcat_lin") if self.rpn_tail is not None]
        if self.cfg.RCNN.ENABLED:
            out += _mlp_tensors("xyz_up", self.xyz_up) + _mlp_tensors("merge_down", self.merge_down)
            for k, level in enumerate(self.rcnn_sa):
                out += _mlp_tensors("rcnn_sa[%d]" % k, level.mlp)
            out += _mlp_tensors("rcnn_cls", self.rcnn_cls) + _mlp_tensors("rcnn_reg", self.rcnn_reg)
            if self.rcnn_head1 is not None:
                out += list(zip(("rcnn_head1.w", "rcnn_head1.b"), self.rcnn_head1))
        return out + [("sa._pcat[%d]" % i, t) for level in self.sa if level.pcat is not None for i, t in enumerate(level.pcat)]

    @torch.no_grad()
    def reload_weights(self):
        model = self.model
        assert not model.training, "FastPointRCNN is an inference engine: call model.eval() first"
        now = _state_shapes(model)
        if [n for n, _ in now] != [n for n, _ in self._shapes]:
            odd = sorted(set(n for n, _ in now) ^ set(n for n, _ in self._shapes))
            raise ValueError("FastPointRCNN.reload_weights: the model's parameters and buffers are not the ones the engine was built for "
                             "(%s)" % ", ".join(odd[:4] or ["their order changed"]))
        for (n, shape), (_, built) in zip(now, self._shapes):
            if shape != built:
                raise ValueError("FastPointRCNN.reload_weights: %s has shape %s, the engine was built for %s" % (n, shape, built))
        folds = {}
        try:
            fresh = FastPointRCNN(model, self.cfg, _fresh=folds)
        except (AssertionError, NotImplementedError, IndexError, RuntimeError) as e:
            raise ValueError("FastPointRCNN.reload_weights: the model no longer folds into this engine (%s: %s)" % (type(e).__name__, e))
        mine, new = self.weight_tensors(), fresh.weight_tensors()
        if len(mine) != len(new):
            raise ValueError("FastPointRCNN.reload_weights: the model folds into %d weight tensors, the engine holds %d" % (len(new), len(mine)))
        for (n, old), (n2, t) in zip(mine, new):
            if n != n2 or old.shape != t.shape or old.dtype != t.dtype or old.device != t.device:
                raise ValueError("FastPointRCNN.reload_weights: %s is %s %s on %s, the engine holds %s %s %s on %s"
                                 % (n2, tuple(t.shape), t.dtype, t.device, n, tuple(old.shape), old.dtype, old.device))
        cached = [m for m in model.modules() if "_prcnn_folded" in m.__dict__]
        for m in cached:
            if id(m) not in folds:
                folds[id(m)] = fused_mlp.fold_fresh(m)
            bad = fused_mlp.refold_mismatch(m, folds[id(m)])
            if bad:
                raise ValueError("FastPointRCNN.reload_weights: " + bad)
        for m in cached:
            fused_mlp.refold_in_place(m, folds[id(m)])
        for (_, old), (_, t) in zip(mine, new):
            old.copy_(t)
        if SPLIT_BF16 and getattr(pu.pointnet2, "IS_HIP_EXTENSION", False) and has_entry(pu.pointnet2, "resplit_weights_bf16x3"):
            pu.pointnet2.resplit_weights_bf16x3([t for _, t in mine])
        self._state = _state_tensors(model)
        self._folded_at = _state_version(self._state)

    @torch.no_grad()
    def geometry_begin(self, xyz):
        state = {"l_xyz": [xyz], "sa": []}
        self._geometry_level(state, 0)
        return state

    @torch.no_grad()
    def geometry_finish(self, state):
        for k in range(len(state["sa"]), len(self.sa)):
            self._geometry_level(state, k)
        l_xyz = state["l_xyz"]
        interp = []
        ext = pu.pointnet2
        for k in range(len(self.fp)):
            unknown, known = l_xyz[k], l_xyz[k + 1]
            if has_entry(ext, "three_nn_weights_wrapper"):
                B, n, m = unknown.shape[0], unknown.shape[1], known.shape[1]
                idx = torch.empty((B, n, 3), dtype=torch.int32, device=unknown.device)
                weight = torch.empty((B, n, 3), dtype=torch.float32, device=unknown.device)
                ext.three_nn_weights_wrapper(B, n, m, unknown, known, idx, weight)
            else:
                dist, idx = pu.three_nn(unknown, known)
                dist_recip = 1.0 / (dist + 1e-8)
                weight = (dist_recip / torch.sum(dist_recip, dim=2, keepdim=True)).contiguous()
            interp.append((idx, weight))
        return {"l_xyz": l_xyz, "sa": state["sa"], "fp": interp}

    @staticmethod
    def _sample(cur_xyz, npoint, nested, roi_clouds=False):
        ext = pu.pointnet2
        n = cur_xyz.shape[1]
        fits = n <= 1024 if roi_clouds else (has_entry(ext, "fps_new_xyz_supported") and ext.fps_new_xyz_supported(n, npoint))
        if has_entry(ext, "fps_new_xyz_wrapper") and fits:
            nested = nested and n <= NESTED_FPS_MAX_N and has_entry(ext, "fps_new_xyz_nested_wrapper") and ext.fps_new_xyz_nested_supported(n, npoint)
            return ext.fps_new_xyz_wrapper(cur_xyz, ext.PrefixExpected(npoint) if nested else npoint)
        sel = pu.furthest_point_sample(cur_xyz, npoint)
        return sel, torch.gather(cur_xyz, 1, sel.long().unsqueeze(-1).expand(-1, -1, 3)).contiguous()

    def _geometry_level(self, state, k):
        npoint, scales, _ = self.sa[k]
        cur = state["l_xyz"][-1]
        ext = pu.pointnet2
        sel, new_xyz = self._sample(cur, npoint, k >= 1)
        if has_entry(ext, "ball_query_full_wrapper"):
            B_, N_ = cur.shape[0], cur.shape[1]
            idxs = []
            for sc in scales:
                ix = torch.empty((B_, npoint, sc.nsample), dtype=torch.int32, device=cur.device)
                ext.ball_query_full_wrapper(B_, N_, npoint, sc.radius, sc.nsample, new_xyz, cur, ix)
                idxs.append(ix)
        else:
            idxs = [pu.ball_query(sc.radius, sc.nsample, cur, new_xyz) for sc in scales]
        lev = {"sel": sel, "new_xyz": new_xyz, "idx": idxs, "pack": [None] * len(scales)}
        if not state.get("defer_packs"):
            self._pack_level(k, cur, lev)
        state["sa"].append(lev)
        state["l_xyz"].append(new_xyz)

    def _pack_level(self, k, cur, lev, arena=None):
        hdr = (lambda: (None, None, None, arena.take((4,), torch.int32))) if (arena is not None and getattr(pu.pointnet2, "IS_HIP_EXTENSION", False)) else (lambda: ())
        lev["pack"] = self._row_lists(k, lev, lambda ix: pu.pointnet2.ball_pack_wrapper(ix, cur, lev["new_xyz"], *hdr()))

    def _row_lists(self, k, lev, make):
        return [make(ix) if (USE_PACKED and sc.on_packed) else None for ix, sc in zip(lev["idx"], self.sa[k].scales)]

    @torch.no_grad()
    def geometry_group(self, xyz_list, on_batch_done=None, group_sa=True):
        sizes = [x.shape[0] for x in xyz_list]
        if len(xyz_list) == 1:
            geo1 = [self.geometry(xyz_list[0])]
            if on_batch_done is not None:
                on_batch_done(0)
            return geo1
        x0, whole = xyz_list[0], None
        if (x0.is_contiguous() and all(x.is_contiguous() and x.shape[1:] == x0.shape[1:] and x.dtype == x0.dtype for x in xyz_list)
                and all(xyz_list[i + 1].data_ptr() == xyz_list[i].data_ptr() + xyz_list[i].numel() * 4 for i in range(len(xyz_list) - 1))
                and x0._base is not None and x0._base.is_contiguous() and x0._base.dim() == 3 and x0._base.shape[1:] == x0.shape[1:]):
            lo_ = (x0.data_ptr() - x0._base.data_ptr()) // (x0[0].numel() * 4)
            if 0 <= lo_ and lo_ + sum(sizes) <= x0._base.shape[0] and x0._base[lo_].data_ptr() == x0.data_ptr():
                whole = x0._base[lo_:lo_ + sum(sizes)]
        state = {"l_xyz": [whole if whole is not None else torch.cat(list(xyz_list), dim=0)], "sa": [], "defer_packs": True}
        arena = ZeroArena(("geo", tuple(sizes), tuple(x0.shape[1:]), str(x0.device)), x0.device)
        self._geometry_level(state, 0)
        geo = self.geometry_finish(state)
        groups = self._point_groups(geo["l_xyz"][0])
        ext = pu.pointnet2
        same = len(set(sizes)) == 1 and has_entry(ext, "ball_pack_groups_wrapper")
        gpacks = None
        n_early = 0
        if group_sa:
            for k in range(min(EARLY_LEVELS, len(self.sa))):
                self._pack_level(k, geo["l_xyz"][k], geo["sa"][k], arena)
            self._xyz_level(geo, arena)
            while n_early < len(geo["sa"]) and geo["sa"][n_early].get("out") is not None:
                n_early += 1
        arena.done()
        if same and n_early < len(geo["sa"]):
            gpacks = [self._row_lists(k, lev, lambda ix: ext.ball_pack_groups_wrapper(ix, geo["l_xyz"][k], lev["new_xyz"], sizes[0]))
                      for k, lev in enumerate(geo["sa"])]
        out, lo = [], 0
        for bi, b in enumerate(sizes):
            hi = lo + b
            g = {"l_xyz": [t[lo:hi] for t in geo["l_xyz"]], "fp": [(i[lo:hi], w[lo:hi]) for i, w in geo["fp"]], "sa": [],
                 "groups": None if groups is None else (groups[0][lo:hi], groups[1][lo:hi])}
            if geo.get("fp_out"):
                g["fp_out"] = {kk: v[lo:hi] for kk, v in geo["fp_out"].items()}
            for k, lev in enumerate(geo["sa"]):
                part = {"sel": lev["sel"][lo:hi], "new_xyz": lev["new_xyz"][lo:hi], "idx": [ix[lo:hi] for ix in lev["idx"]],
                        "pack": [None] * len(lev["idx"])}
                if k < n_early:
                    part["out"] = lev["out"][lo:hi]
                elif gpacks is not None:
                    part["pack"] = [None if p is None else p[bi] for p in gpacks[k]]
                else:
                    self._pack_level(k, g["l_xyz"][k], part)
                g["sa"].append(part)
            if n_early == 0:
                self._xyz_level(g)
            out.append(g)
            if on_batch_done is not None:
                on_batch_done(bi)
            lo = hi
        return out

    def _point_groups(self, xyz):
        rp = roipool3d_utils.roipool3d_cuda
        if not (self.cfg.RCNN.ENABLED and has_entry(rp, "point_groups") and xyz.shape[1] % 64 == 0 and xyz.shape[1] <= 65536):
            return None
        return rp.point_groups(xyz)

    @torch.no_grad()
    def geometry(self, xyz):
        geo = self.geometry_finish(self.geometry_begin(xyz))
        geo["groups"] = self._point_groups(xyz)
        self._xyz_level(geo)
        return geo

    def _xyz_level(self, geo, arena=None):
        if not (USE_PACKED and USE_XYZ_MLP and self.sa and self.sa[0].scales and all(sc.cin == 0 for sc in self.sa[0].scales)):
            return
        l_xyz, prev = geo["l_xyz"], None
        B = l_xyz[0].shape[0]
        for k in range(min(EARLY_LEVELS, len(self.sa))):
            level, lev = self.sa[k], geo["sa"][k]
            packs = lev.get("pack") or [None] * len(level.scales)
            if not level.on_packed or any(pk is None for pk in packs):
                return
            oshape = (B, level.npoint, level.padded_width)
# ... 10 lines not shown

    @staticmethod
    def _sa_scale(xyz, new_xyz, feats, idx, mlp, cin, out, out_col, P_pre=None, pack=None, zeroed=False, dense=False):
        ext = pu.pointnet2
        B, N, _ = xyz.shape
        M, ns = idx.shape[1], idx.shape[2]
        if USE_PACKED and mlp.packed is not None:
            wf, wx, b1, w2, b2, w3, b3 = mlp.packed
            P = P_pre if P_pre is not None else point_layer(feats.view(B * N, feats.shape[2]), wf, b1, False).view(B, N, 128)
            pk = pack if pack is not None else ext.ball_pack_wrapper(idx, xyz, new_xyz)
            ext.sa_packed_mlp_wrapper(new_xyz, xyz, P, wx, pk, w2, b2, w3, b3, out, out_col, zeroed)
            return
        if USE_PACKED and mlp.wide is not None:
            wf, wx, b1, w2, b2, w3, b3 = mlp.wide
            pk = pack if pack is not None else ext.ball_pack_wrapper(idx, xyz, new_xyz)
            if (dense and USE_WIDE_FUSED and has_entry(ext, "sa_wide_fused3_wrapper") and feats.is_contiguous() and
                    feats.shape[2] == wf.shape[0] and ext.sa_wide_fused3_supported(wf.shape[0], wf.shape[1], w2.shape[1], w3.shape[1])):
                ext.sa_wide_fused3_wrapper(new_xyz, xyz, feats, mlp.wide_cat, b1, wx, pk, b2, b3,
                                           (wf.shape[0], wf.shape[1], w2.shape[1], w3.shape[1]), out, out_col, zeroed)
                return
            P = point_layer(feats.view(B * N, feats.shape[2]), wf, b1, False).view(B, N, -1)
            if (dense and USE_WIDE_FUSED and has_entry(ext, "sa_wide_fused_wrapper") and
                    ext.sa_wide_fused_supported(wf.shape[1], w2.shape[1], w3.shape[1])):
                ext.sa_wide_fused_wrapper(new_xyz, xyz, P, wx, pk, w2, b2, w3, b3, out, out_col, zeroed)
                return
            rows = pk.max_tiles * 64
            a1 = torch.empty((rows, wf.shape[1]), dtype=torch.float32, device=xyz.device)
            ext.packed_gather_affine_wrapper(new_xyz, xyz, P, wx, pk, a1)
            y2 = torch.empty((rows, w2.shape[1]), dtype=torch.float32, device=xyz.device)
            ext.packed_layer_wrapper(a1, w2, b2, True, y2, pk)
            ext.packed_layer_segmax_wrapper(y2, w3, b3, pk, B, M, out, out_col, zeroed)
            return
        if feats is not None and feats.shape[2] != cin:
            feats = feats[:, :, :cin].contiguous()
        if (mlp.split is not None and len(mlp.layers) == 3 and mlp.layers[1][2] and mlp.layers[2][2] and
                ext.sa_mlp_fused_supported(mlp.split[0].shape[1], mlp.layers[1][0].shape[1],
                                           mlp.layers[2][0].shape[1], ns)):
            wf, wx, b1 = mlp.split
            P = P_pre if P_pre is not None else gemm_bias_act(feats.view(B * N, cin), wf, b1, False).view(B, N, -1)
            ext.sa_mlp_fused_wrapper(new_xyz, xyz, P, wx, idx, mlp.layers[1][0], mlp.layers[1][1],
                                     mlp.layers[2][0], mlp.layers[2][1], out, out_col)
            return
        if (cin == 0 and USE_XYZ_MLP and len(mlp.layers) == 3 and all(l[2] for l in mlp.layers) and
                ext.sa_xyz_mlp_supported(mlp.layers[0][0].shape[1], mlp.layers[1][0].shape[1], mlp.layers[2][0].shape[1], ns)):
            (w1, b1, _), (w2, b2, _), (w3, b3, _) = mlp.layers
            if USE_PACKED:
                pk = pack if pack is not None else ext.ball_pack_wrapper(idx, xyz, new_xyz)
                ext.sa_xyz_mlp_packed_wrapper(new_xyz, xyz, pk, w1, b1, w2, b2, w3, b3, out, out_col, zeroed)
            else:
                ext.sa_xyz_mlp_wrapper(new_xyz, xyz, idx, w1, b1, w2, b2, w3, b3, out, out_col)
            return
        if mlp.split is not None and M * ns > N:
            wf, wx, b1 = mlp.split
            P = torch.addmm(b1, feats.view(B * N, cin), wf).view(B, N, -1)
            y = torch.empty((B, M * ns, wf.shape[1]), dtype=torch.float32, device=xyz.device)
            ext.gather_affine_relu_pm_wrapper(new_xyz, xyz, P, wx, idx, y)
            y = mlp(y.view(B * M * ns, -1), start=1)
        else:
            grouped = torch.empty((B, M * ns, _round4(cin) + 4), dtype=torch.float32, device=xyz.device)
            ext.group_cat_pm_wrapper(B, N, M, cin, ns, new_xyz, xyz, feats, idx, grouped)
            y = mlp(grouped.view(B * M * ns, -1))
        ext.maxpool_pm_wrapper(y, ns, out, out_col)

    @staticmethod
    def _sa_level_wide(xyz, new_xyz, feats, level, idxs, packs, out, zeroed):
        ext = pu.pointnet2
        B, N, _ = xyz.shape
        M = new_xyz.shape[1]
        dev = xyz.device
        wides = [sc.mlp.wide for sc in level.scales]
        flat = feats.view(B * N, feats.shape[2])
        Ps = [torch.empty((B * N, w.wf.shape[1]), dtype=torch.float32, device=dev) for w in wides]
        ext.packed_layer_batch_wrapper([(flat, w.wf, w.b1, False, P, None) for w, P in zip(wides, Ps)])
        pks = [pk if pk is not None else ext.ball_pack_wrapper(idx, xyz, new_xyz) for pk, idx in zip(packs, idxs)]
        a1s = [torch.empty((pk.max_tiles * 64, w.wf.shape[1]), dtype=torch.float32, device=dev) for pk, w in zip(pks, wides)]
        ext.packed_gather_affine_batch_wrapper([(new_xyz, xyz, P.view(B, N, -1), w.wx, pk, a1) for P, w, pk, a1 in zip(Ps, wides, pks, a1s)])
        y2s = [torch.empty((pk.max_tiles * 64, w.w2.shape[1]), dtype=torch.float32, device=dev) for pk, w in zip(pks, wides)]
        ext.packed_layer_batch_wrapper([(a1, w.w2, w.b2, True, y2, pk) for a1, w, y2, pk in zip(a1s, wides, y2s, pks)])
        ext.packed_layer_segmax_batch_wrapper([(y2, w.w3, w.b3, pk, B, M, out, c, zeroed) for y2, w, pk, c in zip(y2s, wides, pks, level.columns)])

    def _sa_level(self, level, lev, cur_xyz, cur_feat, out, pre):
        scales = level.scales
        packs = lev.get("pack") or [None] * len(scales)
        ext = pu.pointnet2
        if (USE_SCALE_BATCH and USE_PACKED and 2 <= len(scales) <= 4 and all(sc.mlp.wide is not None for sc in scales) and
                has_entry(ext, "packed_layer_batch_wrapper")):
            self._sa_level_wide(cur_xyz, lev["new_xyz"], cur_feat, level, lev["idx"], packs, out, pre)
        elif (USE_SCALE_BATCH and USE_PACKED and len(scales) == 2 and cur_feat is not None and cur_feat.shape[2] % 128 == 0 and
              all(sc.mlp.packed is not None and sc.mlp.packed.w3.shape[1] == 128 and sc.mlp.packed.wf.shape[0] == cur_feat.shape[2] for sc in scales) and
              all(pk is not None for pk in packs) and has_entry(ext, "sa_packed_mlp_batch_wrapper")
              and has_entry(ext, "packed_layer_batch_wrapper")):
            B, N, _ = cur_xyz.shape
            flat = cur_feat.view(B * N, cur_feat.shape[2])
            if USE_SA_NARROW and level.pcat is not None and getattr(ext, "IS_HIP_EXTENSION", False):
                Pcat = torch.empty((B * N, 128), dtype=torch.float32, device=cur_xyz.device)
                wcat, bcat = level.pcat
                ext.packed_layer_wrapper(flat, wcat, bcat, False, Pcat)
                Ps = [Pcat.view(B, N, 128)[:, :, 64 * k:64 * k + 64] for k in range(2)]
            else:
                Ps = [torch.empty((B * N, 128), dtype=torch.float32, device=cur_xyz.device) for _ in scales]
                ext.packed_layer_batch_wrapper([(flat, sc.mlp.packed.wf, sc.mlp.packed.b1, False, P, None) for sc, P in zip(scales, Ps)])
                Ps = [P.view(B, N, 128) for P in Ps]
            ext.sa_packed_mlp_batch_wrapper([(lev["new_xyz"], cur_xyz, P, m.packed.wx, pack, m.packed.w2, m.packed.b2, m.packed.w3, m.packed.b3,
                                              out, col, pre, m.packed_widths) for m, pack, P, col in zip((sc.mlp for sc in scales), packs, Ps, level.columns)])
        else:
            for sc, idx, pack, col in zip(scales, lev["idx"], packs, level.columns):
                self._sa_scale(cur_xyz, lev["new_xyz"], cur_feat, idx, sc.mlp, sc.cin, out, col, pack=pack, zeroed=pre)

    def _backbone(self, xyz, geo, fuse_tail=False, feats0=None):
        l_xyz, l_feat = geo["l_xyz"], [feats0]
        B = xyz.shape[0]
        shapes = [(B, level.npoint, level.padded_width) for level in self.sa]
        pres = [bool(USE_PACKED and level.on_packed) for level in self.sa]
        early = [lev.get("out") if (lev.get("out") is not None and tuple(lev["out"].shape) == sh) else None for lev, sh in zip(geo["sa"], shapes)]
        sizes = [sh[0] * sh[1] * sh[2] if (pr and e is None) else 0 for sh, pr, e in zip(shapes, pres, early)]
        arena = torch.zeros((sum(sizes),), dtype=torch.float32, device=xyz.device) if sum(sizes) else None
        offs = [sum(sizes[:k]) for k in range(len(sizes))]
        for k, (level, lev) in enumerate(zip(self.sa, geo["sa"])):
            if early[k] is not None:
                l_feat.append(early[k])
                continue
            cur_xyz, cur_feat = l_xyz[len(l_feat) - 1], l_feat[-1]
            width = sum(sc.mlp.out_width for sc in level.scales)
            pre = pres[k]
            out = (arena[offs[k]:offs[k] + sizes[k]].view(shapes[k]) if pre
                   else torch.empty(shapes[k], dtype=torch.float32, device=xyz.device))
            if level.padded_width > width and not pre:
                out[:, :, width:] = 0
            self._sa_level(level, lev, cur_xyz, cur_feat, out, pre)
            l_feat.append(out)
        for i in range(-1, -(len(self.fp) + 1), -1):
            k = len(self.fp) + i
            if geo.get("fp_out", {}).get(k) is not None:
                l_feat[k] = geo["fp_out"][k]
                continue
            known_feat, skip = l_feat[k + 1], l_feat[k]
            idx, weight = geo["fp"][k]
            if fuse_tail and k == 0 and self.rpn_tail is not None and skip is None and known_feat.shape[2] == 256:
                return None, (known_feat, idx, weight)
            l_feat[k] = self._fp_module(k, known_feat, skip, idx, weight)
        return (l_feat[0], None) if fuse_tail else l_feat[0]

    def _fp_module(self, k, known_feat, skip, idx, weight):
        ext = pu.pointnet2
        B, n = idx.shape[0], idx.shape[1]
        c2 = known_feat.shape[2]
        c1 = 0 if skip is None else skip.shape[2]
        mlp = self.fp[k]
        wt, b1, relu1 = mlp.layers[0]
        if (USE_FP_LINEAR and USE_POINT_LAYER and PAD128 and c1 and c1 % 128 == 0 and c2 % 128 == 0 and wt.shape[0] == c2 + c1
                and wt.shape[1] % 128 == 0 and len(mlp.layers) >= 2 and has_entry(ext, "packed_layer_interp_wrapper")):
            m = known_feat.shape[1]
            N1 = wt.shape[1]
            G = point_layer(known_feat.view(B * m, c2), wt[:c2], self._zero_bias[:N1], False).view(B, m, N1)
            y1 = torch.empty((B * n, N1), dtype=torch.float32, device=known_feat.device)
            ext.packed_layer_interp_wrapper(skip.view(B * n, c1), wt[c2:], b1, relu1, y1, G, idx, weight)
            return mlp(y1, start=1).view(B, n, -1)
        buf = torch.empty((B, n, c2 + c1), dtype=torch.float32, device=known_feat.device)
        if c1 and c1 % 4 == 0 and c2 % 4 == 0 and has_entry(ext, "three_interpolate_cat_pm_wrapper"):
            ext.three_interpolate_cat_pm_wrapper(known_feat, idx, weight, skip, buf)
        else:
            ext.three_interpolate_pm_wrapper(known_feat, idx, weight, buf, 0)
            if c1:
                buf[:, :, c2:] = skip
        return self.fp[k](buf.view(B * n, c2 + c1)).view(B, n, -1)

    @torch.no_grad()
    def _tail_decode_cfg(self, N):
        cfg, pl = self.cfg, self.model.rpn.proposal_layer
        M = cfg[pl.mode].RPN_POST_NMS_TOP_N
        ext3 = pl_ext()
        if not (USE_FP_LINEAR and self.rpn_tail is not None and getattr(pl, "fused", False) and N <= 65536
                and cfg.TEST.RPN_DISTANCE_BASED_PROPOSE and M <= 128 and cfg.RPN.NMS_TYPE in ("normal", "rotate")
                and has_entry(pu.pointnet2, "rpn_tail_lin_boxes_wrapper") and has_entry(ext3, "rpn_proposals_boxes")
                and pu.pointnet2.rpn_tail_boxes_supported(self.rpn_tail["n_reg"], cfg.RPN.LOC_SCOPE, cfg.RPN.LOC_BIN_SIZE,
                                                         cfg.RPN.NUM_HEAD_BIN, cfg.RPN.LOC_XZ_FINE)):
            return None
        return (cfg.RPN.LOC_SCOPE, cfg.RPN.LOC_BIN_SIZE, cfg.RPN.NUM_HEAD_BIN, cfg.RPN.LOC_XZ_FINE, pl._anchor)

    def rpn_stage(self, pts_input, geo=None, want_reg=False):
        self.check_weights()
        if pts_input.shape[-1] != 3 + self.in_feat:
            raise ValueError("pts_input has %d channels, the backbone was built for 3 + %d" % (pts_input.shape[-1], self.in_feat))
        feats0 = None
        if self.in_feat:
            xyz = pts_input[..., 0:3].contiguous()
            feats0 = pts_input.new_zeros((pts_input.shape[0], pts_input.shape[1], _round128(self.in_feat) if PAD128 else self.in_feat))
            feats0[..., :self.in_feat] = pts_input[..., 3:]
        else:
            xyz = pts_input.contiguous()
        if geo is None:
            geo = self.geometry(xyz)
        B, N, _ = xyz.shape
        with self._strictly():
            feats, tail = self._backbone(xyz, geo, fuse_tail=True, feats0=feats0)
        rpn_boxes = None
        if tail is not None:
            known_feat, idx, weight = tail
            tw = self.rpn_tail
            feats = torch.empty((B, N, 128), dtype=torch.float32, device=xyz.device)
            rpn_cls = torch.empty((B, N, 1), dtype=torch.float32, device=xyz.device)
            dec = None if want_reg or self.in_feat else self._tail_decode_cfg(N)
            rpn_reg = torch.empty((B, N, tw["n_reg"]), dtype=torch.float32, device=xyz.device) if dec is None else None
            if USE_FP_LINEAR and has_entry(pu.pointnet2, "rpn_tail_lin_wrapper"):
                m = known_feat.shape[1]
                G = point_layer(known_feat.view(B * m, known_feat.shape[2]), tw["w1"], tw["zero128"], False).view(B, m, 128)
                if dec is not None:
                    rpn_boxes = torch.empty((B, N, 7), dtype=torch.float32, device=xyz.device)
                    pu.pointnet2.rpn_tail_lin_boxes_wrapper(G, idx, weight, tw["wcat_lin"], tw["bcat"], tw["wc2"], tw["bc2"], tw["n_reg"],
                                                            dec[0], dec[1], dec[2], dec[3], dec[4], xyz, feats, rpn_cls, rpn_boxes)
                else:
                    pu.pointnet2.rpn_tail_lin_wrapper(G, idx, weight, tw["wcat_lin"], tw["bcat"], tw["wc2"], tw["bc2"], feats, rpn_cls, rpn_reg)
            else:
                pu.pointnet2.rpn_tail_wrapper(known_feat, idx, weight, tw["wcat"], tw["bcat"], tw["wc2"], tw["bc2"], feats, rpn_cls, rpn_reg)
        else:
            flat = feats.view(B * N, -1)
            rpn_cls = self.rpn_cls(flat).view(B, N, -1)
            rpn_reg = self.rpn_reg(flat).view(B, N, -1)
            if feats.shape[2] != self.fp[0].n_out:
                feats = feats[:, :, :self.fp[0].n_out].contiguous()
        out = {"rpn_cls": rpn_cls, "rpn_reg": rpn_reg, "rpn_boxes": rpn_boxes, "backbone_xyz": xyz, "rpn_features": feats, "groups": geo.get("groups")}
        out["rpn_scores_raw"] = rpn_cls[:, :, 0].contiguous()
        return out

    @torch.no_grad()
    def point_aux(self, st):
        if "seg_result" not in st:
            ext = pu.pointnet2
            if has_entry(ext, "point_aux_wrapper"):
                sc, xyz = st["rpn_scores_raw"], st["backbone_xyz"]
                seg, depth, dn = torch.empty_like(sc), torch.empty_like(sc), torch.empty_like(sc)
                ext.point_aux_wrapper(sc, xyz, float(self.cfg.RPN.SCORE_THRESH), seg, depth, dn)
                st["seg_result"], st["pts_depth"], st["depth_norm"] = seg, depth, dn
                return
            st["seg_result"] = (torch.sigmoid(st["rpn_scores_raw"]) > self.cfg.RPN.SCORE_THRESH).float()
            st["pts_depth"] = torch.norm(st["backbone_xyz"], p=2, dim=2)
            st["depth_norm"] = (st["pts_depth"] / 70.0 - 0.5).contiguous()

    @torch.no_grad()
    def propose(self, st):
        if self.cfg.RCNN.ENABLED:
            self.point_aux(st)
        if st.get("rpn_boxes") is not None:
            cfg, pl = self.cfg, self.model.rpn.proposal_layer
            boxes, scores = st["rpn_boxes"], st["rpn_scores_raw"]
            M = cfg[pl.mode].RPN_POST_NMS_TOP_N
            rois = torch.empty((boxes.shape[0], M, 7), dtype=torch.float32, device=boxes.device)
            roi_scores = torch.empty((boxes.shape[0], M), dtype=torch.float32, device=boxes.device)
            pl_ext().rpn_proposals_boxes(scores, boxes, cfg[pl.mode].RPN_PRE_NMS_TOP_N, M, cfg[pl.mode].RPN_NMS_THRESH,
                                         cfg.RPN.NMS_TYPE == "rotate", rois, roi_scores)
            return rois, roi_scores
        return self.model.rpn.proposal_layer(st["rpn_scores_raw"], st["rpn_reg"], st["backbone_xyz"])

    @torch.no_grad()
    def rcnn_stage(self, st, rois):
        return self.rcnn_features(self.rcnn_geometry(st, rois))

    @torch.no_grad()
    def rcnn_geometry(self, st, rois):
        self.point_aux(st)
        return self._rcnn_geometry(st["backbone_xyz"], st["rpn_features"], st["seg_result"], st["pts_depth"], rois,
                                   depth_norm=st["depth_norm"], groups=st.get("groups"))

    @torch.no_grad()
    def rcnn_features(self, rg):
        with self._strictly():
            return self._rcnn_features(rg)

    @torch.no_grad()
    def forward(self, pts_input, geo=None, want_reg=True):
        out = self.rpn_stage(pts_input, geo, want_reg=want_reg)
        rois, roi_scores_raw = self.propose(out)
        out.update({"rois": rois, "roi_scores_raw": roi_scores_raw})
        if not self.cfg.RCNN.ENABLED:
            return out
        out.update(self.rcnn_stage(out, rois))
        return out

    def _point_mlp_ok(self):
        if self._pm_ok is None:
            ok = len(self.xyz_up.layers) == 2 and len(self.merge_down.layers) == 1 and len(self.rcnn_sa) > 0
            if ok:
                (wu1, _, r1), (wu2, _, r2) = self.xyz_up.layers
                (wm, _, r3), = self.merge_down.layers
                sa1, mlp1 = self.rcnn_sa[0], self.rcnn_sa[0].mlp
                ok = (tuple(wu1.shape) == (8, 128) and tuple(wu2.shape) == (128, 128) and tuple(wm.shape) == (256, 128)
                      and r1 and r2 and r3 and mlp1.split is not None and tuple(mlp1.split[0].shape) == (128, 128)
                      and len(mlp1.layers) == 3 and sa1.npoint is not None
                      and pu.pointnet2.sa_mlp_fused_supported(128, mlp1.layers[1][0].shape[1], mlp1.layers[2][0].shape[1], sa1.nsample))
            self._pm_ok = bool(ok)
        return self._pm_ok

    def _rcnn(self, xyz, feats, seg_mask, pts_depth, rois, depth_norm=None, groups=None):
        return self._rcnn_features(self._rcnn_geometry(xyz, feats, seg_mask, pts_depth, rois, depth_norm=depth_norm, groups=groups))

    @staticmethod
    def _groupall_fused3_ok(mlp, below):
        ext = pu.pointnet2
        if not (USE_PACKED and mlp.packed is None and mlp.wide is not None and USE_WIDE_FUSED
                and has_entry(ext, "sa_wide_fused3_wrapper") and mlp.wide_cat is not None):
            return False
        w = mlp.wide
        return bool(below.out_width == w.wf.shape[0] and ext.sa_wide_fused3_supported(w.wf.shape[0], w.wf.shape[1], w.w2.shape[1], w.w3.shape[1]))

    def _pool_canonical(self, xyz, feats, seg_mask, pts_depth, rois, depth_norm, groups):
        R = self.cfg.RCNN
        B, M, P, W = rois.shape[0], rois.shape[1], R.NUM_POINTS, 8 + feats.shape[2]
        pooled = torch.empty((B, M, P, W), dtype=torch.float32, device=xyz.device)
        empty = torch.empty((B, M), dtype=torch.int32, device=xyz.device)
# ... 213 lines not shown
```

include/prcnn_hip.h:

```cpp
#ifndef PRCNN_HIP_H
#define PRCNN_HIP_H

#ifdef __cplusplus
extern "C" {
#endif

#define PRCNN_OK 0
#define PRCNN_EINVAL (-1)
#define PRCNN_ELAUNCH (-2)

int prcnn_version(void);
const char *prcnn_last_error(void);
int prcnn_opt_n_threads(int work_size);


int prcnn_ball_query(int b, int n, int m, float radius, int nsample,
                     const float *new_xyz, const float *xyz, int *idx, void *stream);

int prcnn_ball_query_full(int b, int n, int m, float radius, int nsample, const float *new_xyz, const float *xyz, int *idx,
                          void *stream);

int prcnn_set_ball_query_mode(int mode);

int prcnn_group_points(int b, int c, int n, int npoints, int nsample,
                       const float *points, const int *idx, float *out, void *stream);
int prcnn_group_points_grad(int b, int c, int n, int npoints, int nsample,
                            const float *grad_out, const int *idx, float *grad_points, void *stream);

int prcnn_ball_query_limit(int b, int n, int m, float radius, int nsample, const float *new_xyz, const float *xyz,
                           const int *limit, int *idx, void *stream);

int prcnn_gather_points(int b, int c, int n, int npoints,
                        const float *points, const int *idx, float *out, void *stream);
int prcnn_gather_points_grad(int b, int c, int n, int npoints,
                             const float *grad_out, const int *idx, float *grad_points, void *stream);

int prcnn_furthest_point_sampling(int b, int n, int m,
                                  const float *xyz, float *temp, int *idx, void *stream);

int prcnn_set_fps_arithmetic(int mode);

int prcnn_fps_new_xyz(int b, int n, int m, const float *xyz, int *idx, float *new_xyz, void *stream);

int prcnn_fps_new_xyz_nested(int b, int n, int m, const float *xyz, int *idx, float *new_xyz, void *stream);
int prcnn_fps_nested_supported(int n, int m);
int prcnn_fps_prefix_check(int b, int n, int m, const float *xyz, int *idx, float *new_xyz, int *rejected, void *stream);
int prcnn_fps_new_xyz_flagged(int b, int n, int m, const float *xyz, int *idx, float *new_xyz, const int *rejected, void *stream);

int prcnn_three_nn(int b, int n, int m, const float *unknown, const float *known,
                   float *dist2, int *idx, void *stream);

int prcnn_three_nn_weights(int b, int n, int m, const float *unknown, const float *known, int *idx, float *weight,
                           void *stream);
int prcnn_three_interpolate(int b, int c, int m, int n, const float *points,
                            const int *idx, const float *weight, float *out, void *stream);
int prcnn_three_interpolate_grad(int b, int c, int n, int m, const float *grad_out,
                                 const int *idx, const float *weight, float *grad_points, void *stream);

int prcnn_query_and_group(int b, int n, int m, int c, float radius, int nsample,
                          const float *new_xyz, const float *xyz, const float *features,
                          int *idx, float *out, void *stream);


int prcnn_bias_relu_inplace(long outer, int c, long inner, const float *bias, float *x, void *stream);

int prcnn_maxpool_bias_relu(int b, int c, int npoint, int nsample, const float *bias,
                            const float *in, float *out, void *stream);


int prcnn_group_cat_pm(int b, int n, int m, int c, int nsample, const float *new_xyz, const float *xyz,
                       const float *features, const int *idx, float *out, void *stream);
int prcnn_gather_affine_relu_pm(int b, int n, int m, int cout, int nsample, const float *new_xyz,
                                const float *xyz, const float *P, const float *wxyz, const int *idx,
                                float *out, void *stream);
int prcnn_sa_mlp_fused(int b, int n, int m, int nsample, int c1, int c2, int c3, const float *new_xyz,
                       const float *xyz, const float *P, const float *wxyz, const int *idx, const float *w2t,
                       const float *b2, const float *w3t, const float *b3, float *out, int out_stride,
                       int out_col, void *stream);

int prcnn_ball_pack(int b, int n, int m, int nsample, const int *idx, const int *limit, const float *xyz,
                    const float *new_xyz, unsigned int *rowinfo, float *rowdxyz, int *tilecloud, unsigned int *hdr,
                    void *stream);
int prcnn_ball_pack_groups(int b, int group, int n, int m, int nsample, const int *idx, const int *limit, const float *xyz,
                           const float *new_xyz, unsigned int *rowinfo, float *rowdxyz, int *tilecloud, unsigned int *hdr,
                           void *stream);

int prcnn_ball_pack_ex(int b, int group, int n, int m, int nsample, const int *idx, const int *limit, const int *rep, const int *crep,
                       const float *xyz, const float *new_xyz, unsigned int *rowinfo, float *rowdxyz, int *tilecloud, unsigned int *hdr,
                       int hdr_is_zero, void *stream);

int prcnn_ball_pack_rep(int b, int n, int m, int nsample, const int *idx, const int *limit, const int *rep, const int *crep,
                        const float *xyz, const float *new_xyz, unsigned int *rowinfo, float *rowdxyz, int *tilecloud,
                        unsigned int *hdr, void *stream);

int prcnn_dup_rep(int b, int n, int m, const int *sel, const int *limit, const int *prev, int *rep, void *stream);

int prcnn_rcnn_roi_geometry(int b, int n, int m1, float r1, int ns1, int m2, float r2, int ns2, const float *xyz,
                            const int *limit, float *new_xyz1, int *idx1, int *rep1, float *new_xyz2, int *idx2, int *rep2,
                            void *stream);
int prcnn_rcnn_roi_geometry_packs(int b, int n, int m1, float r1, int ns1, int m2, float r2, int ns2, const float *xyz,
                                  const int *limit, float *new_xyz1, int *idx1, int *rep1, float *new_xyz2, int *idx2, int *rep2,
                                  unsigned int *rowinfo1, float *rowdxyz1, int *tilecloud1, unsigned int *hdr1,
                                  unsigned int *rowinfo2, float *rowdxyz2, int *tilecloud2, unsigned int *hdr2,
                                  unsigned int *rowinfo3, float *rowdxyz3, unsigned int *hdr3, int *crows1, unsigned int *hdr_c1,
                                  int hdr_is_zero, void *stream);
int prcnn_sa_packed_mlp(int b, int n, int m, int c3, long max_tiles, const float *P, const float *wxyz,
                        const unsigned int *rowinfo, const float *rowdxyz, const int *tilecloud,
                        const unsigned int *hdr, const float *w2t, const float *b2, const float *w3t,
                        const float *b3, float *out, int out_stride, int out_col, int out_is_zero, void *stream);

int prcnn_sa_wide_fused_supported(int c1, int c2, int c3);
int prcnn_sa_wide_fused(int b, int n, int m, int c1, int c2, int c3, long max_tiles, const float *P, const float *wxyz,
                        const unsigned int *rowinfo, const float *rowdxyz, const int *tilecloud, const unsigned int *hdr,
                        const float *w2, const float *b2, const float *w3, const float *b3, float *out, int out_stride,
                        int out_col, int out_is_zero, void *stream);

int prcnn_sa_wide_fused3_supported(int c0, int c1, int c2, int c3);
int prcnn_sa_wide_fused3(int b, int n, int m, int c0, int c1, int c2, int c3, long max_tiles, const float *F, const float *wxyz,
                         const unsigned int *rowinfo, const float *rowdxyz, const int *tilecloud, const unsigned int *hdr,
                         const float *wcat, const float *b1, const float *b2, const float *b3, float *out, int out_stride,
                         int out_col, int out_is_zero, void *stream);

typedef struct prcnn_gather_problem {
    int b, n, c1; long max_tiles; const float *P; const float *wxyz; const unsigned int *rowinfo; const float *rowdxyz;
    const int *tilecloud; const unsigned int *hdr; float *out;
} prcnn_gather_problem;
typedef struct prcnn_layer_problem {
    const unsigned int *hdr; long rows; long max_tiles; int K, N, n_store; const float *A; long lda; const float *W;
    const float *bias; int relu; float *out; long ldo;
    int b, m; const unsigned int *rowinfo; const int *tilecloud; int out_col, out_is_zero;
} prcnn_layer_problem;
typedef struct prcnn_sa_problem {
    int b, n, m, c3; long max_tiles; const float *P; const float *wxyz; const unsigned int *rowinfo; const float *rowdxyz;
    const int *tilecloud; const unsigned int *hdr; const float *w2t; const float *b2; const float *w3t; const float *b3;
    float *out; int out_stride, out_col, out_is_zero;
    int c1, c2;
} prcnn_sa_problem;
int prcnn_sa_packed_mlp_batch(int nprob, const prcnn_sa_problem *problems, void *stream);
int prcnn_packed_gather_affine_batch(int nprob, const prcnn_gather_problem *problems, void *stream);
int prcnn_packed_layer_batch(int nprob, const prcnn_layer_problem *problems, int segmax, void *stream);
int prcnn_packed_gather_affine(int b, int n, int c1, long max_tiles, const float *P, const float *wxyz,
                               const unsigned int *rowinfo, const float *rowdxyz, const int *tilecloud,
                               const unsigned int *hdr, float *out, void *stream);
int prcnn_packed_layer(const unsigned int *hdr, long rows, long max_tiles, int K, int N, int n_store, const float *A,
                       long lda, const float *W, const float *bias, int relu, float *out, long ldo, void *stream);
int prcnn_split_weights_bf16x3(int K, int N, const float *W, void *out, void *stream);
int prcnn_rows_layer_bf16x3(long rows, int K, int N, int n_store, const float *A, long lda, const void *wsplit, const float *bias,
                            int relu, float *out, long ldo, void *stream);
int prcnn_packed_layer_interp(long rows, int K, int N, const float *A, long lda, const float *W, const float *bias, int relu,
                              float *out, long ldo, int n_per_cloud, int m_known, const float *G, long ldg, const int *idx,
                              const float *weight, void *stream);
int prcnn_sa_xyz_mlp_packed(int b, int m, int c1, int c2, int c3, long max_tiles, const unsigned int *rowinfo,
                            const float *rowdxyz, const int *tilecloud, const unsigned int *hdr, const float *w1,
                            const float *b1, const float *w2, const float *b2, const float *w3, const float *b3,
                            float *out, int out_stride, int out_col, int out_is_zero, void *stream);
int prcnn_rows_dot(long rows, int K, int n, const float *A, long lda, const float *W, const float *bias, float *out,
                   long ldo, void *stream);
int prcnn_rpn_tail(int b, int n, int m, const float *known, const int *idx, const float *weight, const float *wcat,
                   const float *bcat, const float *wc2, const float *bc2, int n_reg, float *feats, float *cls, float *reg,
                   void *stream);
int prcnn_rpn_tail_lin(int b, int n, int m, const float *G, const int *idx, const float *weight, const float *wcat,
                       const float *bcat, const float *wc2, const float *bc2, int n_reg, float *feats, float *cls,
                       float *reg, void *stream);
int prcnn_rpn_tail_boxes_supported(int channels, float loc_scope, float loc_bin_size, int num_head_bin, int xz_fine);
int prcnn_selftest_fmod_two_pi(long n, const float *a, float *out_mine, float *out_lib, void *stream);
int prcnn_rpn_tail_lin_boxes(int b, int n, int m, const float *G, const int *idx, const float *weight, const float *wcat,
                             const float *bcat, const float *wc2, const float *bc2, int n_reg, float loc_scope, float loc_bin_size,
                             int num_head_bin, int xz_fine, const float *anchor_size_host, const float *xyz, float *feats,
                             float *cls, float *boxes, void *stream);
int prcnn_packed_layer_segmax(int b, int m, long max_tiles, int K, int N, const float *A, long lda, const float *W,
                              const float *bias, const unsigned int *rowinfo, const int *tilecloud,
                              const unsigned int *hdr, float *out, int out_stride, int out_col, int out_is_zero, void *stream);

int prcnn_rcnn_point_mlp(long r, int ld, int fcol, const float *rows, const float *wu1, const float *bu1,
                         const float *wu2, const float *bu2, const float *wm, const float *bm, const float *wp,
                         const float *bp, float *xfeat, float *merged, float *p, const int *tilemap,
                         const unsigned int *ntiles, void *stream);
int prcnn_pooled_tiles(int clouds, int rows_per_cloud, const int *cnt, int *tilemap, unsigned int *hdr, void *stream);
int prcnn_pooled_rows(int clouds, int rows_per_cloud, const int *cnt, int *rowmap, unsigned int *hdr, int hdr_is_zero, void *stream);
int prcnn_rcnn_point_mlp_rows(long r, int ld, int fcol, const float *rows, const float *wu1, const float *bu1,
                              const float *wu2, const float *bu2, const float *wm, const float *bm, const float *wp,
                              const float *bp, float *p, const int *rowmap, const unsigned int *hdr, void *stream);

int prcnn_rows_gemm128_rows(long r, const float *src, int ld, int col, const float *w, const float *bias, int relu, float *out,
                            const int *rowmap, const unsigned int *hdr, void *stream);
int prcnn_rows_gemm128(long r, int npanel, const float *src0, int ld0, int col0, const float *src1, int ld1, int col1,
                       const float *w, const float *bias, int relu, float *out, void *stream);

int prcnn_sa_xyz_mlp_supported(int c1, int c2, int c3, int nsample);
int prcnn_sa_xyz_mlp(int b, int n, int m, int nsample, int c1, int c2, int c3, const float *new_xyz,
                     const float *xyz, const int *idx, const float *w1, const float *b1, const float *w2,
                     const float *b2, const float *w3, const float *b3, float *out, int out_stride, int out_col,
                     void *stream);
int prcnn_maxpool_pm(long rows_out, int ns, int c, const float *in, float *out, int out_stride,
                     int out_col, void *stream);
int prcnn_three_interpolate_pm(int b, int c, int m, int n, const float *features, const int *idx,
                               const float *weight, float *out, int out_stride, int out_col, void *stream);
int prcnn_three_interpolate_cat_pm(int b, int c, int m, int n, const float *features, const int *idx, const float *weight,
                                   const float *skip, int c_skip, float *out, void *stream);


int prcnn_boxes_overlap_bev(int num_a, const float *boxes_a, int num_b, const float *boxes_b,
                            float *ans_overlap, void *stream);
int prcnn_boxes_iou_bev(int num_a, const float *boxes_a, int num_b, const float *boxes_b,
                        float *ans_iou, void *stream);
int prcnn_nms(int boxes_num, const float *boxes, long long *keep_host, float thresh, void *stream);
int prcnn_nms_normal(int boxes_num, const float *boxes, long long *keep_host, float thresh, void *stream);

int prcnn_nms_device(int nprob, int n_max, const int *counts, const float *boxes, float thresh,
                     int rotated, int max_keep, int *keep, int *num_keep, void *stream);

int prcnn_point_aux(long rows, float thresh, const float *scores, const float *xyz, float *seg, float *depth, float *depth_norm,
                    void *stream);

int prcnn_rpn_proposals(int b, int n, int channels, float loc_scope, float loc_bin_size, int num_head_bin,
                        int xz_fine, const float *anchor_size_host, int pre_nms_top_n, int post_nms_top_n,
                        float nms_thresh, int rotated_nms, const float *xyz, const float *scores,
                        const float *reg, float *rois, float *roi_scores, void *stream);
int prcnn_rpn_proposals_boxes(int b, int n, int pre_nms_top_n, int post_nms_top_n, float nms_thresh, int rotated_nms,
                              const float *scores, const float *boxes, float *rois, float *roi_scores, void *stream);

int prcnn_rcnn_postprocess(int b, int m, int channels, float loc_scope, float loc_bin_size, int num_head_bin,
                           int y_by_bin, float loc_y_scope, float loc_y_bin_size, const float *anchor_size_host,
                           float score_thresh, float nms_thresh, const float *rois, const float *rcnn_reg,
                           const float *rcnn_cls, float *pred_boxes3d, float *boxes, float *scores, int *num,
                           void *stream);
int prcnn_rcnn_postprocess_blobs(int b, int m, int channels, float loc_scope, float loc_bin_size, int num_head_bin,
                                 int y_by_bin, float loc_y_scope, float loc_y_bin_size, const float *anchor_size_host,
                                 float score_thresh, float nms_thresh, const float *rois, const float *rcnn_reg,
                                 const float *rcnn_cls, float *pred_boxes3d, float *blobs, int scenes_per_blob, void *stream);


int prcnn_roipool3d(int batch_size, int pts_num, int boxes_num, int feature_in_len,
                    int sampled_pts_num, const float *xyz, const float *boxes3d,
                    const float *pts_feature, float *pooled_features, int *pooled_empty_flag,
                    void *stream);

int prcnn_roipool3d_canonical(int batch_size, int pts_num, int boxes_num, int feature_len, int sampled_pts_num,
                              float pool_extra_width, const float *xyz, const float *rois, const float *feats,
                              const float *seg_mask, const float *depth, float *pooled, int *pooled_empty_flag,
                              int *pooled_cnt, const float *pxyz, const float *aabb, void *stream);
int prcnn_roipool3d_canonical_xyz(int batch_size, int pts_num, int boxes_num, int feature_len, int sampled_pts_num,
                                  float pool_extra_width, const float *xyz, const float *rois, const float *feats,
                                  const float *seg_mask, const float *depth, float *pooled, int *pooled_empty_flag,
                                  int *pooled_cnt, const float *pxyz, const float *aabb, float *xyz_out, void *stream);
int prcnn_point_groups(int b, int n, const float *xyz, float *pxyz, float *aabb, void *stream);

int prcnn_host_pts_in_boxes3d(int boxes_num, int pts_num, const float *pts, const float *boxes3d, long long *flags);
int prcnn_host_roipool3d(int boxes_num, int pts_num, int feature_len, int sampled, const float *pts,
                         const float *boxes3d, const float *pts_feature, float *pooled_pts, float *pooled_features,
                         long long *empty);


int prcnn_rotate_iou_eval(int n, int k, const float *boxes, const float *query_boxes,
                          float *iou, int criterion, void *stream);

int prcnn_rotate_iou_eval_segmented(int nseg, long long total, const long long *out_off, const int *box_off,
                                    const int *q_off, const float *boxes, const float *query_boxes, float *iou,
                                    int criterion, void *stream);

int prcnn_bev_best_match(int nseg, int n, int k, const int *box_off, const int *q_off, const float *boxes,
                         const float *query_boxes, int criterion, float *row_val, int *row_idx, float *col_val, int *col_idx,
                         void *stream);

int prcnn_eval_align(int nseg, int n, const int *box_off, const int *q_off, double *location, double *dimensions,
                     const double *alpha, const double *rotation_y, const double *gt_dimensions, const float *row_val,
                     const int *row_idx, int mode, int *branch, void *stream);


enum { PRCNN_CALIB_ROW = 35 };
int prcnn_input_stage(int b, int n_max, int stride, int lidar_frame, int image_filter, const int *counts,
                      const float *raw, const float *calib, const float *scope_host, int npoints, float far_depth,
                      int npoints_faraway, const unsigned long long *seeds, float *out, int *stats, int *choice,
                      void *stream);

int prcnn_valid_flags(int b, int n_max, int stride, int lidar_frame, int image_filter, const int *counts, const float *raw,
                      const float *calib, const float *scope_host, float far_depth, float *rect, unsigned char *cls,
                      void *stream);


int prcnn_kitti_image_stats(int n_gt, int n_dt, int n_dc, const double *overlaps, const double *gt_datas,
                            const double *dt_datas, const long long *ignored_gt, const long long *ignored_det,
                            const double *dc_bboxes, int metric, double min_overlap, double thresh, int compute_fp,
                            int compute_aos, long long *tp_fp_fn, double *similarity, double *thresholds,
                            int *n_thresholds);

int prcnn_kitti_collect_scores(int n_img, const long long *gt_nums, const long long *dt_nums,
                               const double *overlaps_flat, const double *gt_datas, const double *dt_datas,
                               const long long *ignored_gts, const long long *ignored_dets, int metric,
                               double min_overlap, double *scores_out, long long *n_scores);

int prcnn_kitti_accumulate_pr(int n_img, const long long *gt_nums, const long long *dt_nums, const long long *dc_nums,
                              const double *overlaps_flat, const double *gt_datas, const double *dt_datas,
                              const double *dontcares, const long long *ignored_gts, const long long *ignored_dets,
                              int metric, double min_overlap, const double *thresholds, int n_thresh, int compute_aos,
                              double *pr);

enum {
    PRCNN_SN_T = 0, PRCNN_SN_R = 3, PRCNN_SN_XLO = 12, PRCNN_SN_XHI, PRCNN_SN_YLO, PRCNN_SN_ZLO, PRCNN_SN_ZHI, PRCNN_SN_SCALE = 17,
    PRCNN_SN_FSCALE = 50, PRCNN_SN_SHIFT = 53, PRCNN_SN_FLAG1 = 57, PRCNN_SN_FLAG2 = 58, PRCNN_SN_BOXD = 64
};
enum { PRCNN_SN_CNT = 0, PRCNN_SN_RIDX = 13, PRCNN_SN_BOXI = 16 };
typedef struct prcnn_sn_batch {
    int n_scenes, max_tiles, max_boxes, avoid;
// ... 156 lines not shown
```

Baseline: 8949 scenes/s.

## Pre-pack GEMM weights into lane-contiguous panels for 128-bit loads

After: 9031 scenes/s, median of 6. About the same (+0.9%).

```diff
diff --git a/3d_adapt_auto_driving_amd/csrc/layer_tile.hpp b/3d_adapt_auto_driving_amd/csrc/layer_tile.hpp
--- a/3d_adapt_auto_driving_amd/csrc/layer_tile.hpp
+++ b/3d_adapt_auto_driving_amd/csrc/layer_tile.hpp
@@ -11,15 +11,29 @@
 constexpr int PL_MAX_BATCH = 4;
 struct PLProblem {
     const unsigned int *hdr; long rows_host; int K, N; const float *A; long lda; const float *W; const float *bias; int do_relu;
+    int w_panels;
     float *out; long ldo; const unsigned int *rowinfo; const int *tilecloud; int m, out_col, n_store;
     int lds_pool;
     const float *addG; const int *addIdx; const float *addW; int add_n, add_m; long add_ldg;
 };
 struct PLBatch { PLProblem p[PL_MAX_BATCH]; };
 
+template <bool PANELS>
+__device__ __forceinline__ unsigned int pl_w_lane(int lane, int N, int col0 )
+{
+    if constexpr (PANELS) return ((unsigned int)(col0 >> 5) * 1024u + (unsigned int)lane) * 16u;
+    return ((unsigned int)(64 * (lane >> 5)) * (unsigned int)N + (unsigned int)(col0 + (lane & 31))) * 4u;
+}
+#define PL_W(wf, s) wf[(s) >> 2][(s) & 3]
 #define PL_LOAD_W(dst, kk)                                                                              \
-    _Pragma("unroll") for (int s = 0; s < 64; ++s)                                                      \
-        dst[s] = __uint_as_float(__builtin_amdgcn_raw_buffer_load_b32(wrs, lane_off, (unsigned int)((kk) + s) * row_bytes, 0));
+    if constexpr (PANELS) {                                                                             \
+        _Pragma("unroll") for (int q = 0; q < 16; ++q)                                                  \
+            dst[q] = __builtin_bit_cast(f32x4, __builtin_amdgcn_raw_buffer_load_b128(                   \
+                wrs, lane_off, (unsigned int)(kk) * row_bytes + (unsigned int)q * 1024u, 0));           \
+    } else {                                                                                            \
+        _Pragma("unroll") for (int s = 0; s < 64; ++s)                                                  \
+            PL_W(dst, s) = __uint_as_float(__builtin_amdgcn_raw_buffer_load_b32(wrs, lane_off, (unsigned int)((kk) + s) * row_bytes, 0)); \
+    }
 #define PL_VM_DRAIN __builtin_amdgcn_s_waitcnt(0x0F70);
 #define PL_SADD(x, y) asm volatile("s_add_u32 %0, %0, %1" : "+s"(x) : "s"(y) : "scc");
 
@@ -31,8 +45,8 @@
 #define PL_BOTH_HALVES(...) __VA_ARGS__
 #define PL_ONE_HALF(...)
 #define PL_MFMA(H2, wf, c, s)                                                                           \
-    acc0 = __builtin_amdgcn_mfma_f32_32x32x2f32(a0.c, wf[4 * g + s], acc0, 0, 0, 0);                    \
-    H2(acc1 = __builtin_amdgcn_mfma_f32_32x32x2f32(a1.c, wf[4 * g + s], acc1, 0, 0, 0);)
+    acc0 = __builtin_amdgcn_mfma_f32_32x32x2f32(a0.c, wf[g][s], acc0, 0, 0, 0);                         \
+    H2(acc1 = __builtin_amdgcn_mfma_f32_32x32x2f32(a1.c, wf[g][s], acc1, 0, 0, 0);)
 #define PL_STAGE_HEAD(T, H2)                                                                            \
     const float *a0p = (T) + j * PL_LD + 64 * h;                                                        \
     H2(const float *a1p = (T) + (32 + j) * PL_LD + 64 * h;)                                             \
@@ -64,18 +78,29 @@
     f32x4 ar[8];                                                                                        \
     unsigned int wo_ = (unsigned int)(kn) * row_bytes;                                                  \
     unsigned int ao_ = (unsigned int)(kn) * 4u;                                                         \
-    const unsigned int a8_ = 8u * a_row_bytes;
+    const unsigned int a8_ = 8u * a_row_bytes;                                                          \
+    const unsigned int ws_ = PANELS ? 1024u : row_bytes;
+#define PL_NEXT_W(wn, LOFF)                                                                             \
+    if constexpr (PANELS) {                                                                             \
+        _Pragma("unroll") for (int q = 0; q < 2; ++q)                                                   \
+            if (g < 8) {                                                                                \
+                wn[2 * g + q] = __builtin_bit_cast(f32x4, __builtin_amdgcn_raw_buffer_load_b128(wrs, (LOFF), wo_, 0)); \
+                PL_SADD(wo_, ws_)                                                                       \
+            }                                                                                           \
+    } else {                                                                                            \
+        _Pragma("unroll") for (int q = 0; q < 6; ++q)                                                   \
+            if (6 * g + q < 64) {                                                                       \
+                PL_W(wn, 6 * g + q) = __uint_as_float(__builtin_amdgcn_raw_buffer_load_b32(wrs, (LOFF), wo_, 0)); \
+                PL_SADD(wo_, ws_)                                                                       \
+            }                                                                                           \
+    }
 #define PL_NEXT_PANEL(TN, wn, ARS, LOFF)                                                                \
     if (g < 8) {                                                                                        \
         ar[g] = __builtin_bit_cast(f32x4, __builtin_amdgcn_raw_buffer_load_b128((ARS), a_lane, ao_, 0)); \
         PL_SADD(ao_, a8_)                                                                               \
     } else                                                                                              \
         *reinterpret_cast<f32x4 *>((TN) + (r0 + 8 * (g - 8)) * PL_LD + 4 * chunk) = ar[g - 8];          \
-    _Pragma("unroll") for (int q = 0; q < 6; ++q)                                                       \
-        if (6 * g + q < 64) {                                                                           \
-            wn[6 * g + q] = __uint_as_float(__builtin_amdgcn_raw_buffer_load_b32(wrs, (LOFF), wo_, 0)); \
-            PL_SADD(wo_, row_bytes)                                                                     \
-        }                                                                                               \
+    PL_NEXT_W(wn, LOFF)                                                                                 \
     PL_FENCE
 #define PL_STAGE_PREFETCH_X(T, TN, wf, wn, kn, ARS, LOFF) PL_STAGE_SIDE(T, wf, PL_NEXT_PANEL_STATE(kn), PL_NEXT_PANEL(TN, wn, ARS, LOFF))
 #define PL_STAGE_PREFETCH(T, TN, wf, wn, kn) PL_STAGE_PREFETCH_X(T, TN, wf, wn, kn, ars, lane_off)
@@ -88,16 +113,17 @@
     PL_FENCE
 #define PL_STAGE_ROWS(T, TN, wf, soff) PL_STAGE_SIDE(T, wf, f32x4 ar[8];, PL_NEXT_ROWS(TN, soff))
 
+#define PL32_NEXT_PANEL_STATE(kn)                                                                       \
+    f32x4 ar[4];                                                                                        \
+    unsigned int wo_ = (unsigned int)(kn) * row_bytes;                                                  \
+    const unsigned int ws_ = PANELS ? 1024u : row_bytes;
 #define PL32_NEXT_PANEL(TN, wn, kn)                                                                     \
     if (g < 4)                                                                                          \
         ar[g] = __builtin_bit_cast(f32x4, __builtin_amdgcn_raw_buffer_load_b128(                        \
             ars, a_lane, (unsigned int)(8 * g) * a_row_bytes + (unsigned int)(kn) * 4u, 0));            \
     else if (g >= 8 && g < 12)                                                                          \
         *reinterpret_cast<f32x4 *>((TN) + (r0 + 8 * (g - 8)) * PL_LD + 4 * chunk) = ar[g - 8];          \
-    _Pragma("unroll") for (int q = 0; q < 6; ++q)                                                       \
-        if (6 * g + q < 64)                                                                             \
-            wn[6 * g + q] = __uint_as_float(__builtin_amdgcn_raw_buffer_load_b32(                       \
-                wrs, lane_off, (unsigned int)((kn) + 6 * g + q) * row_bytes, 0));
+    PL_NEXT_W(wn, lane_off)
 
 __device__ __forceinline__ void pl_store_direct(const f32x16 &acc0, const f32x16 &acc1, float bcol, int do_relu, float *out, long ldo,
                                                 long t, long rows, unsigned int col)
diff --git a/3d_adapt_auto_driving_amd/csrc/packed_layer.hip b/3d_adapt_auto_driving_amd/csrc/packed_layer.hip
--- a/3d_adapt_auto_driving_amd/csrc/packed_layer.hip
+++ b/3d_adapt_auto_driving_amd/csrc/packed_layer.hip
@@ -13,7 +13,7 @@
     _Pragma("unroll") for (int i = 0; i < 8; ++i)                                                       \
         *reinterpret_cast<f32x4 *>(tile + (r0 + 8 * i) * PL_LD + 4 * chunk) = src[i];
 
-template <bool SEGMAX>
+template <bool SEGMAX, bool PANELS>
 __global__ __launch_bounds__(256, 2) void packed_layer_kernel(const PLBatch bt)
 {
     const PLProblem pb = bt.p[blockIdx.z];
@@ -29,9 +29,9 @@
     f32x16 acc0 = {0}, acc1 = {0};
     const __amdgpu_buffer_rsrc_t wrs = __builtin_amdgcn_make_buffer_rsrc((void *)pb.W, 0, K * N * 4, 0x00020000);
     const unsigned int row_bytes = (unsigned int)N * 4u;
-    const unsigned int lane_off = ((unsigned int)(64 * h) * (unsigned int)N + (unsigned int)(n0 + 32 * w + j)) * 4u;
+    const unsigned int lane_off = pl_w_lane<PANELS>(lane, N, n0 + 32 * w);
     for (int k0 = 0; k0 < K; k0 += 128) {
-        float wf[64];
+        f32x4 wf[16];
         f32x4 ar[8];
         PL_LOAD_W(wf, k0)
         PL_LOAD_A(ar, k0)
@@ -43,7 +43,10 @@
     pl_epilogue<SEGMAX>(acc0, acc1, tile, ctr, t, rows, n0, pb);
 }
 
-template <bool SEGMAX>
+#define PL_PANEL_TOP                                                                                    \
+    PL_VM_DRAIN                  \
+    lds_barrier();
+template <bool SEGMAX, bool PANELS>
 __global__ __launch_bounds__(256, 2) void packed_layer_pipe_kernel(const PLBatch bt)
 {
     const PLProblem pb = bt.p[blockIdx.z];
@@ -60,28 +63,32 @@
     f32x16 acc0 = {0}, acc1 = {0};
     const __amdgpu_buffer_rsrc_t wrs = __builtin_amdgcn_make_buffer_rsrc((void *)pb.W, 0, K * N * 4, 0x00020000);
     const unsigned int row_bytes = (unsigned int)N * 4u;
-    const unsigned int lane_off = ((unsigned int)(64 * h) * (unsigned int)N + (unsigned int)(n0 + 32 * w + j)) * 4u;
+    const unsigned int lane_off = pl_w_lane<PANELS>(lane, N, n0 + 32 * w);
     const long left = rows - t * PL_ROWS;
     const unsigned int a_row_bytes = (unsigned int)pb.lda * 4u;
     const __amdgpu_buffer_rsrc_t ars = __builtin_amdgcn_make_buffer_rsrc(
         (void *)(pb.A + t * PL_ROWS * pb.lda), 0, (int)((left < PL_ROWS ? left : PL_ROWS) * (long)a_row_bytes), 0x00020000);
     const unsigned int a_lane = (unsigned int)r0 * a_row_bytes + 16u * chunk;
-    float wa[64], wb[64];
+    f32x4 wa[16], wb[16];
     PL_LOAD_W(wa, 0)
     PL_FETCH_TILE(tiles, 8, 0)
     const int np = K >> 7;
-    for (int p = 0; p < np; ++p) {
-        PL_VM_DRAIN
-        lds_barrier();
-        const float *T = tiles + (p & 1) * (PL_ROWS * PL_LD);
-        float *TN = tiles + ((p + 1) & 1) * (PL_ROWS * PL_LD);
-        if (p + 1 < np) {
-            PL_STAGE_PREFETCH(T, TN, wa, wb, (p + 1) * 128)
-#pragma unroll
-            for (int s = 0; s < 64; ++s) wa[s] = wb[s];
-        } else {
-            PL_STAGE(T, wa)
-        }
+    float *const T0 = tiles, *const T1 = tiles + PL_ROWS * PL_LD;
+    int p = 0;
+    for (; p + 2 < np; p += 2) {
+        PL_PANEL_TOP
+        PL_STAGE_PREFETCH(T0, T1, wa, wb, (p + 1) * 128)
+        PL_PANEL_TOP
+        PL_STAGE_PREFETCH(T1, T0, wb, wa, (p + 2) * 128)
+    }
+    if (p + 2 == np) {
+        PL_PANEL_TOP
+        PL_STAGE_PREFETCH(T0, T1, wa, wb, (p + 1) * 128)
+        PL_PANEL_TOP
+        PL_STAGE(T1, wb)
+    } else {
+        PL_PANEL_TOP
+        PL_STAGE(T0, wa)
     }
     if constexpr (!SEGMAX) {
         if (n0 + 128 <= pb.n_store && !pb.addG) {
@@ -92,7 +99,7 @@
     pl_epilogue<SEGMAX>(acc0, acc1, tiles, ctr, t, rows, n0, pb);
 }
 
-template <bool ADD>
+template <bool ADD, bool PANELS>
 __global__ __launch_bounds__(256, 2) void packed_layer_persist_kernel(const PLProblem pb, unsigned int *__restrict__ ticket)
 {
     __shared__ float tiles[2 * PL_ROWS * PL_LD];
@@ -115,14 +122,12 @@
         return __builtin_amdgcn_make_buffer_rsrc((void *)(pb.A + (long)t * PL_ROWS * pb.lda), 0,
                                                  (int)((left < PL_ROWS ? left : PL_ROWS) * (long)a_row_bytes), 0x00020000);
     };
-    auto loff = [&](unsigned int cb) __attribute__((always_inline)) {
-        return ((unsigned int)(64 * h) * (unsigned int)N + (cb * 128u + (unsigned int)(32 * w + j))) * 4u;
-    };
+    auto loff = [&](unsigned int cb) __attribute__((always_inline)) { return pl_w_lane<PANELS>(lane, N, (int)cb * 128 + 32 * w); };
     unsigned int item = blockIdx.x;
     unsigned int t = item / col_blocks, cb = item - t * col_blocks;
     __amdgpu_buffer_rsrc_t ars = tile_rsrc(t);
     unsigned int lane_off = loff(cb);
-    float wa[64], wb[64];
+    f32x4 wa[16], wb[16];
     PL_LOAD_W(wa, 0)
     PL_FETCH_TILE(tiles, 8, 0)
     int pp = 0;
@@ -144,7 +149,7 @@
             if (p + 1 < np) {
                 PL_STAGE_PREFETCH(T, TN, wa, wb, (p + 1) * 128)
 #pragma unroll
-                for (int s2 = 0; s2 < 64; ++s2) wa[s2] = wb[s2];
+                for (int q = 0; q < 16; ++q) wa[q] = wb[q];
             } else {
                 next = s_item[slot];
                 if (next < n_items) {
@@ -153,7 +158,7 @@
                     const unsigned int loff_n = loff(cbn);
                     PL_STAGE_PREFETCH_X(T, TN, wa, wb, 0, ars_n, loff_n)
 #pragma unroll
-                    for (int s2 = 0; s2 < 64; ++s2) wa[s2] = wb[s2];
+                    for (int q = 0; q < 16; ++q) wa[q] = wb[q];
                     PL_VM_DRAIN
                 } else {
                     PL_STAGE(T, wa)
@@ -176,6 +181,7 @@
     if (tid == 0) ticket_release(ticket);
 }
 
+template <bool PANELS>
 __global__ __launch_bounds__(256, 2) void packed_layer_stream_kernel(const PLProblem pb)
 {
     __shared__ float tiles[2 * PL_ROWS * PL_LD];
@@ -190,8 +196,8 @@
     if (t >= ntiles || n0 >= pb.n_store) return;
     const __amdgpu_buffer_rsrc_t wrs = __builtin_amdgcn_make_buffer_rsrc((void *)pb.W, 0, 128 * N * 4, 0x00020000);
     const unsigned int row_bytes = (unsigned int)N * 4u;
-    const unsigned int lane_off = ((unsigned int)(64 * h) * (unsigned int)N + (unsigned int)(n0 + 32 * w + j)) * 4u;
-    float wf[64];
+    const unsigned int lane_off = pl_w_lane<PANELS>(lane, N, n0 + 32 * w);
+    f32x4 wf[16];
     PL_LOAD_W(wf, 0)
     const unsigned int a_row_bytes = (unsigned int)pb.lda * 4u;
     const __amdgpu_buffer_rsrc_t ars = __builtin_amdgcn_make_buffer_rsrc((void *)pb.A, 0, (int)(rows * (long)a_row_bytes), 0x00020000);
@@ -223,6 +229,10 @@
     }
 }
 
+#define PL32_STAGE_PREFETCH(T, TN, wf, wn, kn)                                                          \
+    { PL_STAGE_HEAD(T, PL_ONE_HALF) PL_STAGE_GROUPS(wf, PL_ONE_HALF, PL32_NEXT_PANEL_STATE(kn), PL32_NEXT_PANEL(TN, wn, kn) PL_FENCE) }
+#define PL32_STAGE(T, wf) { PL_STAGE_HEAD(T, PL_ONE_HALF) PL_STAGE_GROUPS(wf, PL_ONE_HALF, PL_NO_SIDE, PL_FENCE) }
+template <bool PANELS>
 __global__ __launch_bounds__(256, 2) void packed_layer_pipe32_kernel(const PLBatch bt)
 {
     const PLProblem pb = bt.p[blockIdx.z];
@@ -239,29 +249,32 @@
     f32x16 acc0 = {0};
     const __amdgpu_buffer_rsrc_t wrs = __builtin_amdgcn_make_buffer_rsrc((void *)pb.W, 0, K * N * 4, 0x00020000);
     const unsigned int row_bytes = (unsigned int)N * 4u;
-    const unsigned int lane_off = ((unsigned int)(64 * h) * (unsigned int)N + (unsigned int)(n0 + 32 * w + j)) * 4u;
+    const unsigned int lane_off = pl_w_lane<PANELS>(lane, N, n0 + 32 * w);
     const long left = rows - t * R;
     const unsigned int a_row_bytes = (unsigned int)pb.lda * 4u;
     const __amdgpu_buffer_rsrc_t ars =
         __builtin_amdgcn_make_buffer_rsrc((void *)(pb.A + t * R * pb.lda), 0, (int)((left < R ? left : R) * (long)a_row_bytes), 0x00020000);
     const unsigned int a_lane = (unsigned int)r0 * a_row_bytes + 16u * chunk;
-    float wa[64], wb[64];
+    f32x4 wa[16], wb[16];
     PL_LOAD_W(wa, 0)
     PL_FETCH_TILE(tiles, R / 8, 0)
     const int np = K >> 7;
-    for (int p = 0; p < np; ++p) {
-        PL_VM_DRAIN
-        lds_barrier();
-        const float *T = tiles + (p & 1) * (R * PL_LD);
-        float *TN = tiles + ((p + 1) & 1) * (R * PL_LD);
-        PL_STAGE_HEAD(T, PL_ONE_HALF)
-        if (p + 1 < np) {
-            PL_STAGE_GROUPS(wa, PL_ONE_HALF, f32x4 ar[4];, PL32_NEXT_PANEL(TN, wb, (p + 1) * 128) PL_FENCE)
-#pragma unroll
-            for (int s = 0; s < 64; ++s) wa[s] = wb[s];
-        } else {
-            PL_STAGE_GROUPS(wa, PL_ONE_HALF, PL_NO_SIDE, PL_FENCE)
-        }
+    float *const T0 = tiles, *const T1 = tiles + R * PL_LD;
+    int p = 0;
+    for (; p + 2 < np; p += 2) {
+        PL_PANEL_TOP
+        PL32_STAGE_PREFETCH(T0, T1, wa, wb, (p + 1) * 128)
+        PL_PANEL_TOP
+        PL32_STAGE_PREFETCH(T1, T0, wb, wa, (p + 2) * 128)
+    }
+    if (p + 2 == np) {
+        PL_PANEL_TOP
+        PL32_STAGE_PREFETCH(T0, T1, wa, wb, (p + 1) * 128)
+        PL_PANEL_TOP
+        PL32_STAGE(T1, wb)
+    } else {
+        PL_PANEL_TOP
+        PL32_STAGE(T0, wa)
     }
     const float bcol = pb.bias[n0 + 32 * w + j];
     const int do_relu = pb.do_relu;
@@ -304,36 +317,41 @@
     return {PL_PIPE, tiles, col_blocks};
 }
 
-int pl_launch(PLForm form, const PLBatch &bt, int k, long gx, int gy, bool segmax, hipStream_t st, const char *what)
+template <bool PANELS>
+int pl_launch_w(PLForm form, const PLBatch &bt, int k, long gx, int gy, bool segmax, hipStream_t st, const char *what)
 {
     const dim3 grid((unsigned)gx, gy, k), wg(256);
     switch (form) {
     case PL_ONE:
-        if (segmax) hipLaunchKernelGGL(packed_layer_kernel<true>, grid, wg, 0, st, bt);
-        else hipLaunchKernelGGL(packed_layer_kernel<false>, grid, wg, 0, st, bt);
+        if (segmax) hipLaunchKernelGGL((packed_layer_kernel<true, PANELS>), grid, wg, 0, st, bt);
+        else hipLaunchKernelGGL((packed_layer_kernel<false, PANELS>), grid, wg, 0, st, bt);
         break;
     case PL_PIPE:
-        if (segmax) hipLaunchKernelGGL(packed_layer_pipe_kernel<true>, grid, wg, 0, st, bt);
-        else hipLaunchKernelGGL(packed_layer_pipe_kernel<false>, grid, wg, 0, st, bt);
+        if (segmax) hipLaunchKernelGGL((packed_layer_pipe_kernel<true, PANELS>), grid, wg, 0, st, bt);
+        else hipLaunchKernelGGL((packed_layer_pipe_kernel<false, PANELS>), grid, wg, 0, st, bt);
         break;
-    case PL_PIPE32: hipLaunchKernelGGL(packed_layer_pipe32_kernel, grid, wg, 0, st, bt); break;
-    case PL_STREAM: hipLaunchKernelGGL(packed_layer_stream_kernel, grid, wg, 0, st, bt.p[0]); break;
+    case PL_PIPE32: hipLaunchKernelGGL(packed_layer_pipe32_kernel<PANELS>, grid, wg, 0, st, bt); break;
+    case PL_STREAM: hipLaunchKernelGGL(packed_layer_stream_kernel<PANELS>, grid, wg, 0, st, bt.p[0]); break;
     case PL_PERSIST: {
         unsigned int *ticket = next_ticket(st);
         if (!ticket) { set_error("%s: cannot set up the item ticket", what); return PRCNN_ELAUNCH; }
-        if (bt.p[0].addG) hipLaunchKernelGGL(packed_layer_persist_kernel<true>, grid, wg, 0, st, bt.p[0], ticket);
-        else hipLaunchKernelGGL(packed_layer_persist_kernel<false>, grid, wg, 0, st, bt.p[0], ticket);
+        if (bt.p[0].addG) hipLaunchKernelGGL((packed_layer_persist_kernel<true, PANELS>), grid, wg, 0, st, bt.p[0], ticket);
+        else hipLaunchKernelGGL((packed_layer_persist_kernel<false, PANELS>), grid, wg, 0, st, bt.p[0], ticket);
         break;
     }
     }
     return check_launch(what);
+}
+int pl_launch(PLForm form, const PLBatch &bt, int k, long gx, int gy, bool segmax, hipStream_t st, const char *what)
+{
+    return bt.p[0].w_panels ? pl_launch_w<true>(form, bt, k, gx, gy, segmax, st, what) : pl_launch_w<false>(form, bt, k, gx, gy, segmax, st, what);
 }
 
 PLProblem pl_problem(const prcnn_layer_problem &q, bool segmax)
 {
     PLProblem p = {};
     p.hdr = q.hdr; p.rows_host = q.rows; p.K = q.K; p.N = q.N; p.A = q.A; p.lda = q.lda; p.W = q.W; p.bias = q.bias;
-    p.do_relu = segmax ? 1 : q.relu; p.out = q.out; p.ldo = q.ldo; p.n_store = segmax ? q.N : q.n_store;
+    p.do_relu = segmax ? 1 : q.relu; p.out = q.out; p.ldo = q.ldo; p.n_store = segmax ? q.N : q.n_store; p.w_panels = q.w_panels != 0;
     if (segmax) {
         p.rowinfo = q.rowinfo; p.tilecloud = q.tilecloud; p.m = q.m; p.out_col = q.out_col;
         p.lds_pool = (((uintptr_t)q.out | (uintptr_t)q.bias) & 15) == 0 && (q.ldo & 3) == 0 && (q.out_col & 3) == 0;
@@ -386,7 +404,7 @@
     int gy = 0;
     for (int i = 0; i < k; ++i) {
         plan[i] = pl_plan(bt.p[i], tiles_of[i], segmax, k == 1);
-        together = together && plan[i].form == plan[0].form && (plan[i].form == PL_ONE || plan[i].form == PL_PIPE || plan[i].form == PL_PIPE32);
+        together = together && plan[i].form == plan[0].form && bt.p[i].w_panels == bt.p[0].w_panels && (plan[i].form == PL_ONE || plan[i].form == PL_PIPE || plan[i].form == PL_PIPE32);
         if (plan[i].gx > gx) gx = plan[i].gx;
         if (plan[i].gy > gy) gy = plan[i].gy;
     }
@@ -421,9 +439,9 @@
 }
 
 
-extern "C" int prcnn_packed_layer_interp(long rows, int K, int N, const float *A, long lda, const float *W, const float *bias, int relu,
-                                         float *out, long ldo, int n_per_cloud, int m_known, const float *G, long ldg, const int *idx,
-                                         const float *weight, void *stream)
+static int packed_layer_interp(long rows, int K, int N, const float *A, long lda, const float *W, int w_panels, const float *bias, int relu,
+                               float *out, long ldo, int n_per_cloud, int m_known, const float *G, long ldg, const int *idx,
+                               const float *weight, void *stream)
 {
     PRCNN_REQUIRE(rows >= 0 && K > 0 && N > 0 && K % 128 == 0 && N % 128 == 0, "packed_layer_interp: K=%d, N=%d must be multiples of 128", K, N);
     PRCNN_REQUIRE(lda >= K && lda % 4 == 0 && ldo >= N && ldo % 4 == 0 && ldg >= N && ldg % 4 == 0, "packed_layer_interp: bad leading dimensions");
@@ -435,9 +453,24 @@
     PRCNN_REQUIRE(tiles <= 0x7fffffffL, "packed_layer_interp: too many rows");
     prcnn_layer_problem q = {};
     q.rows = rows; q.K = K; q.N = N; q.n_store = N; q.A = A; q.lda = lda; q.W = W; q.bias = bias; q.relu = relu; q.out = out; q.ldo = ldo;
+    q.w_panels = w_panels;
     PLBatch bt;
     PLProblem &p = bt.p[0] = pl_problem(q, false);
     p.addG = G; p.addIdx = idx; p.addW = weight; p.add_n = n_per_cloud; p.add_m = m_known; p.add_ldg = ldg;
     const PLPlan plan = pl_plan(p, tiles, false, true);
     return pl_launch(plan.form, bt, 1, plan.gx, plan.gy, false, (hipStream_t)stream, "packed_layer_interp");
 }
+
+extern "C" int prcnn_packed_layer_interp(long rows, int K, int N, const float *A, long lda, const float *W, const float *bias, int relu,
+                                         float *out, long ldo, int n_per_cloud, int m_known, const float *G, long ldg, const int *idx,
+                                         const float *weight, void *stream)
+{
+    return packed_layer_interp(rows, K, N, A, lda, W, 0, bias, relu, out, ldo, n_per_cloud, m_known, G, ldg, idx, weight, stream);
+}
+
+extern "C" int prcnn_packed_layer_interp_panels(long rows, int K, int N, const float *A, long lda, const float *Wpanels, const float *bias,
+                                                int relu, float *out, long ldo, int n_per_cloud, int m_known, const float *G, long ldg,
+                                                const int *idx, const float *weight, void *stream)
+{
+    return packed_layer_interp(rows, K, N, A, lda, Wpanels, 1, bias, relu, out, ldo, n_per_cloud, m_known, G, ldg, idx, weight, stream);
+}
diff --git a/3d_adapt_auto_driving_amd/csrc/sa_wide.hpp b/3d_adapt_auto_driving_amd/csrc/sa_wide.hpp
--- a/3d_adapt_auto_driving_amd/csrc/sa_wide.hpp
+++ b/3d_adapt_auto_driving_amd/csrc/sa_wide.hpp
@@ -39,7 +39,20 @@
 }
 
 #define SW_VM_DRAIN __builtin_amdgcn_s_waitcnt(0x0F70);
-#define SW_STAGE(T, wf, wn, RS, VOFF, SOFF, RB, FIRST)                                                    \
+#define SW_NEXT_PLAIN(wn, RS, VOFF, SOFF, RB)                                                             \
+    _Pragma("unroll") for (int q = 0; q < 6; ++q)                                                         \
+        if (6 * g + q < 64)                                                                               \
+            wn[6 * g + q] = __uint_as_float(__builtin_amdgcn_raw_buffer_load_b32(                         \
+                RS, VOFF, (SOFF) + (unsigned int)(6 * g + q) * (RB), 0));
+#define SW_LOAD_PANEL_Q(wn, RS, VOFF, SOFF, Q)                                                            \
+    {                                                                                                     \
+        const f32x4 v_ = __builtin_bit_cast(f32x4, __builtin_amdgcn_raw_buffer_load_b128(RS, VOFF, (SOFF) + (unsigned int)(Q) * 1024u, 0)); \
+        wn[4 * (Q)] = v_.x; wn[4 * (Q) + 1] = v_.y; wn[4 * (Q) + 2] = v_.z; wn[4 * (Q) + 3] = v_.w;      \
+    }
+#define SW_NEXT_PANELS(wn, RS, VOFF, SOFF)                                                                \
+    _Pragma("unroll") for (int q = 0; q < 2; ++q)                                                         \
+        if (g < 8) SW_LOAD_PANEL_Q(wn, RS, VOFF, SOFF, 2 * g + q)
+#define SW_STAGE_W(T, wf, wn, FIRST, NEXT)                                                                \
     {                                                                                                     \
         const float *ap = (T) + j * SW_LD + 64 * h;                                                       \
         f32x4 a = *reinterpret_cast<const f32x4 *>(ap);                                                   \
@@ -53,10 +66,7 @@
             } else {                                                                                      \
                 acc = __builtin_amdgcn_mfma_f32_32x32x2f32(a.x, wf[4 * g + 0], acc, 0, 0, 0);             \
             }                                                                                             \
-            _Pragma("unroll") for (int q = 0; q < 6; ++q)       \
-                if (6 * g + q < 64)                                                                       \
-                    wn[6 * g + q] = __uint_as_float(__builtin_amdgcn_raw_buffer_load_b32(                 \
-                        RS, VOFF, (SOFF) + (unsigned int)(6 * g + q) * (RB), 0));                         \
+            NEXT                                                                                          \
             __builtin_amdgcn_sched_barrier(0);                                                            \
             acc = __builtin_amdgcn_mfma_f32_32x32x2f32(a.y, wf[4 * g + 1], acc, 0, 0, 0);                 \
             acc = __builtin_amdgcn_mfma_f32_32x32x2f32(a.z, wf[4 * g + 2], acc, 0, 0, 0);                 \
@@ -64,5 +74,6 @@
             a = nx;                                                                                       \
         }                                                                                                 \
     }
+#define SW_STAGE(T, wf, wn, RS, VOFF, SOFF, RB, FIRST) SW_STAGE_W(T, wf, wn, FIRST, SW_NEXT_PLAIN(wn, RS, VOFF, SOFF, RB))
 
 }
diff --git a/3d_adapt_auto_driving_amd/csrc/sa_wide3.hip b/3d_adapt_auto_driving_amd/csrc/sa_wide3.hip
--- a/3d_adapt_auto_driving_amd/csrc/sa_wide3.hip
+++ b/3d_adapt_auto_driving_amd/csrc/sa_wide3.hip
@@ -26,6 +26,7 @@
     unsigned int rb, soff;
 };
 
+template <bool PANELS>
 __global__ __launch_bounds__(256, 2) void sa_wide3_kernel(const SaWide3Args a)
 {
     extern __shared__ __align__(16) float sw_lds[];
@@ -51,6 +52,7 @@
     const unsigned int lane_k = (unsigned int)(64 * h), lane_c = (unsigned int)(32 * w + j) * 4u;
     const unsigned int voff1 = lane_k * (unsigned int)a.c1 * 4u + lane_c, voff2 = lane_k * (unsigned int)a.c2 * 4u + lane_c,
                        voff3 = lane_k * (unsigned int)a.c3 * 4u + lane_c;
+    const unsigned int voffp = (unsigned int)w * 16384u + (unsigned int)lane * 16u;
     const float4 *F4 = reinterpret_cast<const float4 *>(a.F);
     const int q0 = a.c0 >> 2;
 
@@ -63,7 +65,7 @@
         else { st.layer = 2; st.kpn = kp2; si = sc - ns1 - ns2; st.rb = (unsigned int)a.c3 * 4u; base = o3; }
         st.nb = si / st.kpn;
         st.kp = si - st.nb * st.kpn;
-        st.soff = base + (unsigned int)(st.kp * 128) * st.rb + (unsigned int)st.nb * 512u;
+        st.soff = base + (unsigned int)(st.kp * 128) * st.rb + (unsigned int)st.nb * (PANELS ? 65536u : 512u);
         return st;
     };
 
@@ -77,8 +79,13 @@
     if (u >= units) { if (tid == 0) ticket_release(a.ticket); return; }
     float wa[64], wb[64];
     f32x16 acc;
-#pragma unroll
-    for (int s = 0; s < 64; ++s) wa[s] = __uint_as_float(__builtin_amdgcn_raw_buffer_load_b32(rs, voff1, (unsigned int)s * (unsigned int)a.c1 * 4u, 0));
+    if constexpr (PANELS) {
+#pragma unroll
+        for (int q = 0; q < 16; ++q) SW_LOAD_PANEL_Q(wa, rs, voffp, 0u, q)
+    } else {
+#pragma unroll
+        for (int s = 0; s < 64; ++s) wa[s] = __uint_as_float(__builtin_amdgcn_raw_buffer_load_b32(rs, voff1, (unsigned int)s * (unsigned int)a.c1 * 4u, 0));
+    }
 
     for (unsigned int served = 0; u < units; ++served) {
         const long t = u >> 1;
@@ -117,7 +124,12 @@
                 const float *T = (st.layer == 0 ? X : (st.layer == 1 ? A1 : X)) + st.kp * SW_PANEL;
                 const unsigned int voffn = nst.layer == 0 ? voff1 : (nst.layer == 1 ? voff2 : voff3);
                 if (st.layer > 0 && st.kp == 0 && st.nb == 0) lds_barrier();
-                if (half == 0) { SW_STAGE(T, wa, wb, rs, voffn, nst.soff, nst.rb, st.kp == 0) } else { SW_STAGE(T, wb, wa, rs, voffn, nst.soff, nst.rb, st.kp == 0) }
+                if constexpr (PANELS) {
+                    if (half == 0) { SW_STAGE_W(T, wa, wb, st.kp == 0, SW_NEXT_PANELS(wb, rs, voffp, nst.soff)) }
+                    else { SW_STAGE_W(T, wb, wa, st.kp == 0, SW_NEXT_PANELS(wa, rs, voffp, nst.soff)) }
+                } else {
+                    if (half == 0) { SW_STAGE(T, wa, wb, rs, voffn, nst.soff, nst.rb, st.kp == 0) } else { SW_STAGE(T, wb, wa, rs, voffn, nst.soff, nst.rb, st.kp == 0) }
+                }
                 SW_VM_DRAIN
                 if (st.kp == st.kpn - 1) {
                     const int col = st.nb * 128 + 32 * w + j;
@@ -170,10 +182,10 @@
     return sa_wide3_lds(c0, c1, c2, c3) <= 96 * 1024 ? 1 : 0;
 }
 
-extern "C" int prcnn_sa_wide_fused3(int b, int n, int m, int c0, int c1, int c2, int c3, long max_tiles, const float *F, const float *wxyz,
-                                    const unsigned int *rowinfo, const float *rowdxyz, const int *tilecloud, const unsigned int *hdr,
-                                    const float *wcat, const float *b1, const float *b2, const float *b3, float *out, int out_stride,
-                                    int out_col, int out_is_zero, void *stream)
+static int sa_wide_fused3(bool panels, int b, int n, int m, int c0, int c1, int c2, int c3, long max_tiles, const float *F, const float *wxyz,
+                          const unsigned int *rowinfo, const float *rowdxyz, const int *tilecloud, const unsigned int *hdr,
+                          const float *wcat, const float *b1, const float *b2, const float *b3, float *out, int out_stride,
+                          int out_col, int out_is_zero, void *stream)
 {
     PRCNN_REQUIRE(b >= 0 && n >= 0 && m >= 0 && max_tiles >= 0, "sa_wide_fused3: bad sizes");
     PRCNN_REQUIRE(prcnn_sa_wide_fused3_supported(c0, c1, c2, c3), "sa_wide_fused3: unsupported widths %d-%d-%d-%d", c0, c1, c2, c3);
@@ -190,7 +202,8 @@
     }
     if (max_tiles == 0) return PRCNN_OK;
     const size_t lds = sa_wide3_lds(c0, c1, c2, c3);
-    const int rc = ensure_dynamic_lds((const void *)sa_wide3_kernel, lds, "sa_wide_fused3");
+    const int rc = panels ? ensure_dynamic_lds((const void *)sa_wide3_kernel<true>, lds, "sa_wide_fused3")
+                          : ensure_dynamic_lds((const void *)sa_wide3_kernel<false>, lds, "sa_wide_fused3");
     if (rc != PRCNN_OK) return rc;
     SaWide3Args a;
     a.n = n; a.m = m; a.c0 = c0; a.c1 = c1; a.c2 = c2; a.c3 = c3; a.hdr = hdr; a.rowdxyz = (const float4 *)rowdxyz; a.F = F; a.wxyz = wxyz;
@@ -200,6 +213,25 @@
     if (!a.ticket) { set_error("sa_wide_fused3: cannot set up the unit ticket"); return PRCNN_ELAUNCH; }
     const long units = 2 * max_tiles;
     const long grid = units < mfma_grid_cap() ? units : mfma_grid_cap();
-    hipLaunchKernelGGL(sa_wide3_kernel, dim3((unsigned)grid), dim3(256), lds, st, a);
+    if (panels) hipLaunchKernelGGL(sa_wide3_kernel<true>, dim3((unsigned)grid), dim3(256), lds, st, a);
+    else hipLaunchKernelGGL(sa_wide3_kernel<false>, dim3((unsigned)grid), dim3(256), lds, st, a);
     return check_launch("sa_wide_fused3");
 }
+
+extern "C" int prcnn_sa_wide_fused3(int b, int n, int m, int c0, int c1, int c2, int c3, long max_tiles, const float *F, const float *wxyz,
+                                    const unsigned int *rowinfo, const float *rowdxyz, const int *tilecloud, const unsigned int *hdr,
+                                    const float *wcat, const float *b1, const float *b2, const float *b3, float *out, int out_stride,
+                                    int out_col, int out_is_zero, void *stream)
+{
+    return sa_wide_fused3(false, b, n, m, c0, c1, c2, c3, max_tiles, F, wxyz, rowinfo, rowdxyz, tilecloud, hdr, wcat, b1, b2, b3, out, out_stride,
+                          out_col, out_is_zero, stream);
+}
+
+extern "C" int prcnn_sa_wide_fused3_panels(int b, int n, int m, int c0, int c1, int c2, int c3, long max_tiles, const float *F,
+                                           const float *wxyz, const unsigned int *rowinfo, const float *rowdxyz, const int *tilecloud,
+                                           const unsigned int *hdr, const float *wcat_panels, const float *b1, const float *b2,
+                                           const float *b3, float *out, int out_stride, int out_col, int out_is_zero, void *stream)
+{
+    return sa_wide_fused3(true, b, n, m, c0, c1, c2, c3, max_tiles, F, wxyz, rowinfo, rowdxyz, tilecloud, hdr, wcat_panels, b1, b2, b3, out,
+                          out_stride, out_col, out_is_zero, stream);
+}
diff --git a/3d_adapt_auto_driving_amd/dropin/pointnet2_cuda.py b/3d_adapt_auto_driving_amd/dropin/pointnet2_cuda.py
--- a/3d_adapt_auto_driving_amd/dropin/pointnet2_cuda.py
+++ b/3d_adapt_auto_driving_amd/dropin/pointnet2_cuda.py
@@ -463,7 +463,25 @@
     return out
 
 
+def weight_panels(wt):
+    p = getattr(wt, "panels", None)
+    if p is None:
+        return None
+    if p.shape != wt.shape or p.dtype != wt.dtype or p.device != wt.device or not p.is_contiguous():
+        raise RuntimeError("pointnet2_cuda: a weight matrix's panel form must be a contiguous tensor of its shape, type and device")
+    return p
+
+
+def _weights(q, wt):
+    p = weight_panels(wt)
+    q.W, q.w_panels = (wt.data_ptr(), 0) if p is None else (p.data_ptr(), 1)
+
+
 def packed_layer_wrapper(a, wt, bias, relu, out, pack=None):
+    if weight_panels(wt) is not None:
+        if pack is not None and pack.tilecloud is None:
+            raise RuntimeError("pointnet2_cuda: packed_layer does not take a list whose rows carry their cloud (its tile count is not in hdr[0])")
+        return packed_layer_batch_wrapper([(a, wt, bias, relu, out, pack)])[0]
     _chk(torch.float32, wt, bias)
     for t in (a, out):
         if not t.is_cuda or t.dtype != torch.float32 or t.dim() != 2 or t.stride(1) != 1:
@@ -525,7 +543,9 @@
     B, n = idx.shape[0], idx.shape[1]
     if wt.size(0) != K or tuple(out.shape) != (R, N) or R != B * n or G.shape[0] != B or G.shape[2] != N or tuple(weight.shape) != tuple(idx.shape):
         raise RuntimeError("pointnet2_cuda: packed_layer_interp shape mismatch")
-    _lib.call("prcnn_packed_layer_interp", R, K, N, a.data_ptr(), a.stride(0), wt.data_ptr(), bias.data_ptr(), int(bool(relu)),
+    panels = weight_panels(wt)
+    _lib.call("prcnn_packed_layer_interp" if panels is None else "prcnn_packed_layer_interp_panels", R, K, N, a.data_ptr(), a.stride(0),
+              (wt if panels is None else panels).data_ptr(), bias.data_ptr(), int(bool(relu)),
               out.data_ptr(), out.stride(0), n, G.shape[1], G.data_ptr(), G.stride(1), idx.data_ptr(), weight.data_ptr(),
               _lib.current_stream(a))
     return out
@@ -557,8 +577,10 @@
     c0w, c1, c2, c3 = (int(v) for v in widths)
     if c0 != c0w or wcat.numel() != c0 * c1 + c1 * c2 + c2 * c3 or wxyz.size(1) != c1 or b1.numel() != c1 or b2.numel() != c2 or b3.numel() != c3:
         raise RuntimeError("pointnet2_cuda: sa_wide_fused3 shape mismatch")
-    _lib.call("prcnn_sa_wide_fused3", b, n, new_xyz.size(1), c0, c1, c2, c3, pack.max_tiles, feats.data_ptr(), wxyz.data_ptr(),
-              pack.rowinfo.data_ptr(), pack.rowdxyz.data_ptr(), _lib.ptr(pack.tilecloud), pack.hdr.data_ptr(), wcat.data_ptr(),
+    panels = weight_panels(wcat)
+    _lib.call("prcnn_sa_wide_fused3" if panels is None else "prcnn_sa_wide_fused3_panels", b, n, new_xyz.size(1), c0, c1, c2, c3,
+              pack.max_tiles, feats.data_ptr(), wxyz.data_ptr(), pack.rowinfo.data_ptr(), pack.rowdxyz.data_ptr(),
+              _lib.ptr(pack.tilecloud), pack.hdr.data_ptr(), (wcat if panels is None else panels).data_ptr(),
               b1.data_ptr(), b2.data_ptr(), b3.data_ptr(), out.data_ptr(), out.size(-1), out_col, int(bool(zeroed)),
               _lib.current_stream(xyz))
     return out
@@ -584,7 +606,8 @@
             raise RuntimeError("pointnet2_cuda: packed_layer expects 2-D float32 CUDA matrices with unit column stride")
         q.K, q.N = wt.shape
         q.n_store = out.size(1)
-        q.A, q.lda, q.W, q.bias, q.relu = a.data_ptr(), a.stride(0), wt.data_ptr(), bias.data_ptr(), int(bool(relu))
+        q.A, q.lda, q.bias, q.relu = a.data_ptr(), a.stride(0), bias.data_ptr(), int(bool(relu))
+        _weights(q, wt)
         q.out, q.ldo = out.data_ptr(), out.stride(0)
         q.hdr, q.rows, q.max_tiles = (None, a.size(0), 0) if pack is None else (pack.hdr.data_ptr(), 0, pack.max_tiles)
     _lib.call("prcnn_packed_layer_batch", len(problems), arr, 0, _lib.current_stream(problems[0][0]))
@@ -597,7 +620,8 @@
         _chk(torch.float32, a, wt, bias, out)
         q.K, q.N = wt.shape
         q.n_store = q.N
-        q.A, q.lda, q.W, q.bias, q.relu = a.data_ptr(), a.stride(0), wt.data_ptr(), bias.data_ptr(), 1
+        q.A, q.lda, q.bias, q.relu = a.data_ptr(), a.stride(0), bias.data_ptr(), 1
+        _weights(q, wt)
         q.out, q.ldo, q.out_col, q.out_is_zero = out.data_ptr(), out.size(-1), out_col, int(bool(zeroed))
         q.b, q.m = b, m
         q.hdr, q.max_tiles, q.rowinfo, q.tilecloud = pack.hdr.data_ptr(), pack.max_tiles, pack.rowinfo.data_ptr(), pack.tilecloud.data_ptr()
@@ -666,6 +690,8 @@
 
 def packed_layer_segmax_wrapper(a, wt, bias, pack, b, m, out, out_col, zeroed=False):
     _chk(torch.float32, a, wt, bias, out)
+    if weight_panels(wt) is not None:
+        return packed_layer_segmax_batch_wrapper([(a, wt, bias, pack, b, m, out, out_col, zeroed)])[0]
     K, N = wt.shape
     _lib.call("prcnn_packed_layer_segmax", b, m, pack.max_tiles, K, N, a.data_ptr(), a.stride(0), wt.data_ptr(), bias.data_ptr(),
               pack.rowinfo.data_ptr(), pack.tilecloud.data_ptr(), pack.hdr.data_ptr(), out.data_ptr(), out.size(-1), out_col, int(zeroed),
diff --git a/3d_adapt_auto_driving_amd/net/fast_infer.py b/3d_adapt_auto_driving_amd/net/fast_infer.py
--- a/3d_adapt_auto_driving_amd/net/fast_infer.py
+++ b/3d_adapt_auto_driving_amd/net/fast_infer.py
@@ -23,6 +23,7 @@
 USE_RPN_TAIL = os.environ.get("PRCNN_NO_RPN_TAIL") is None
 USE_SCALE_BATCH = True
 USE_SA_NARROW = True
+USE_WEIGHT_PANELS = True
 USE_WIDE_FUSED = True
 EARLY_LEVELS = int(os.environ.get("PRCNN_EARLY_LEVELS", "4"))
 EARLY_FP = int(os.environ.get("PRCNN_EARLY_FP", "2"))
@@ -128,6 +129,48 @@
         return pu.pointnet2.packed_layer_wrapper(a, wt, bias, relu, out)
     y = gemm_bias_act(a, wt, bias, relu)
     return y if n_out == N else y[:, :n_out].contiguous()
+
+
+def pack_weight_panels(w):
+    K, N = w.shape
+    assert K % 128 == 0 and N % 128 == 0, (K, N)
+    return w.reshape(K // 128, 2, 16, 4, N // 32, 32).permute(0, 4, 2, 1, 5, 3).contiguous().view(K, N)
+
+
+def unpack_weight_panels(packed):
+    K, N = packed.shape
+    return packed.reshape(K // 128, N // 32, 16, 2, 32, 4).permute(0, 3, 2, 5, 1, 4).contiguous().view(K, N)
+
+
+def pack_weight_panels_cat(flat, shapes):
+    assert flat.dim() == 1 and flat.numel() == sum(K * N for K, N in shapes)
+    parts = torch.split(flat, [K * N for K, N in shapes])
+    return torch.cat([pack_weight_panels(t.view(K, N)).reshape(-1) for t, (K, N) in zip(parts, shapes)])
+
+
+def _panel_form(w):
+    shapes = getattr(w, "panel_parts", None)
+    return pack_weight_panels(w) if shapes is None else pack_weight_panels_cat(w, shapes)
+
+
+def with_panels(w, parts=None):
+    if parts is None:
+        shapes = [tuple(w.shape)] if w.dim() == 2 else []
+    else:
+        shapes = [tuple(sh) for sh in parts]
+    if USE_WEIGHT_PANELS and shapes and w.is_contiguous() and all(K % 128 == 0 and N % 128 == 0 for K, N in shapes):
+        if parts is not None:
+            w.panel_parts = shapes
+        w.panels = _panel_form(w)
+    return w
+
+
+def panel_rows(w, lo, hi):
+    v = w[lo:hi]
+    p = getattr(w, "panels", None)
+    if p is not None and lo % 128 == 0 and hi % 128 == 0:
+        v.panels = p[lo:hi]
+    return v
 
 
 PackedWeights = typing.NamedTuple("PackedWeights", [(name, torch.Tensor) for name in ("wf", "wx", "b1", "w2", "b2", "w3", "b3")])
@@ -151,7 +194,7 @@
                         src, dst = src + c, dst + _round128(c)
                 else:
                     wt = _pad2(w.t(), _round128(w.shape[1]), np_)
-                self.layers.append((wt.contiguous(), _pad1(b, np_), relu))
+                self.layers.append((with_panels(wt.contiguous()), _pad1(b, np_), relu))
             self.padded = not pad_out
             w, b, relu = layers[-1]
             if self.padded and w.shape[0] <= 4 and not relu:
@@ -181,14 +224,15 @@
             c1, c2, c3 = wf.shape[1], w2.shape[1], w3.shape[1]
             kin = _round128(wf.shape[0]) if PAD128 else wf.shape[0]
             if c1 <= 128 and c2 <= 128 and c3 in (128, 256) and w2.shape[0] == c1 and w3.shape[0] == c2:
-                self.packed = PackedWeights(_pad2(wf, kin, 128), _pad2(wx, 3, 128), _pad1(b1, 128),
+                self.packed = PackedWeights(with_panels(_pad2(wf, kin, 128)), _pad2(wx, 3, 128), _pad1(b1, 128),
                                             _pad2(w2, 128, 128), _pad1(b2, 128), _pad2(w3, 128, c3), b3)
                 self.packed_widths = (c1, c2)
             elif c3 % 128 == 0 and w2.shape[0] == c1 and w3.shape[0] == c2:
                 c1p, c2p = _round128(c1), _round128(c2)
-                self.wide = PackedWeights(_pad2(wf, kin, c1p), _pad2(wx, 3, c1p), _pad1(b1, c1p),
-                                          _pad2(w2, c1p, c2p), _pad1(b2, c2p), _pad2(w3, c2p, c3), b3)
-                self.wide_cat = torch.cat([t.reshape(-1) for t in (self.wide.wf, self.wide.w2, self.wide.w3)]).contiguous()
+                self.wide = PackedWeights(with_panels(_pad2(wf, kin, c1p)), _pad2(wx, 3, c1p), _pad1(b1, c1p),
+                                          with_panels(_pad2(w2, c1p, c2p)), _pad1(b2, c2p), with_panels(_pad2(w3, c2p, c3)), b3)
+                self.wide_cat = with_panels(torch.cat([t.reshape(-1) for t in (self.wide.wf, self.wide.w2, self.wide.w3)]).contiguous(),
+                                            parts=[t.shape for t in (self.wide.wf, self.wide.w2, self.wide.w3)])
 
     @property
     def out_width(self):
@@ -310,7 +354,7 @@
             and all(c1 == 64 and c2 in (64, 96) for c1, c2 in (sc.mlp.packed_widths for sc in scales))
             and pk[0].wf.shape[0] == pk[1].wf.shape[0] and pk[0].wf.shape[0] % 128 == 0):
         return None
-    return (torch.cat([p.wf[:, :64] for p in pk], 1).contiguous(), torch.cat([p.b1[:64] for p in pk]).contiguous())
+    return (with_panels(torch.cat([p.wf[:, :64] for p in pk], 1).contiguous()), torch.cat([p.b1[:64] for p in pk]).contiguous())
 
 
 class FastPointRCNN:
@@ -359,7 +403,7 @@
             c0, r0 = self.rcnn_cls.layers[0], self.rcnn_reg.layers[0]
             if (USE_POINT_LAYER and USE_PACKED and len(self.rcnn_cls.layers) > 1 and len(self.rcnn_reg.layers) > 1 and c0[2] and r0[2] and
                     c0[0].shape == r0[0].shape and c0[0].shape[0] % 128 == 0 and c0[0].shape[1] % 128 == 0):
-                self.rcnn_head1 = (torch.cat([c0[0], r0[0]], 1).contiguous(), torch.cat([c0[1], r0[1]]).contiguous(), c0[0].shape[1])
+                self.rcnn_head1 = (with_panels(torch.cat([c0[0], r0[0]], 1).contiguous()), torch.cat([c0[1], r0[1]]).contiguous(), c0[0].shape[1])
 
     def _covered(self):
         try:
@@ -452,6 +496,9 @@
             fused_mlp.refold_in_place(m, folds[id(m)])
         for (_, old), (_, t) in zip(mine, new):
             old.copy_(t)
+        for _, old in mine:
+            if getattr(old, "panels", None) is not None:
+                old.panels.copy_(_panel_form(old))
         if SPLIT_BF16 and getattr(pu.pointnet2, "IS_HIP_EXTENSION", False) and has_entry(pu.pointnet2, "resplit_weights_bf16x3"):
             pu.pointnet2.resplit_weights_bf16x3([t for _, t in mine])
         self._state = _state_tensors(model)
@@ -768,9 +815,9 @@
                 and wt.shape[1] % 128 == 0 and len(mlp.layers) >= 2 and has_entry(ext, "packed_layer_interp_wrapper")):
             m = known_feat.shape[1]
             N1 = wt.shape[1]
-            G = point_layer(known_feat.view(B * m, c2), wt[:c2], self._zero_bias[:N1], False).view(B, m, N1)
+            G = point_layer(known_feat.view(B * m, c2), panel_rows(wt, 0, c2), self._zero_bias[:N1], False).view(B, m, N1)
             y1 = torch.empty((B * n, N1), dtype=torch.float32, device=known_feat.device)
-            ext.packed_layer_interp_wrapper(skip.view(B * n, c1), wt[c2:], b1, relu1, y1, G, idx, weight)
+            ext.packed_layer_interp_wrapper(skip.view(B * n, c1), panel_rows(wt, c2, c2 + c1), b1, relu1, y1, G, idx, weight)
             return mlp(y1, start=1).view(B, n, -1)
         buf = torch.empty((B, n, c2 + c1), dtype=torch.float32, device=known_feat.device)
         if c1 and c1 % 4 == 0 and c2 % 4 == 0 and has_entry(ext, "three_interpolate_cat_pm_wrapper"):
diff --git a/include/prcnn_hip.h b/include/prcnn_hip.h
--- a/include/prcnn_hip.h
+++ b/include/prcnn_hip.h
@@ -120,6 +120,10 @@
                          const unsigned int *rowinfo, const float *rowdxyz, const int *tilecloud, const unsigned int *hdr,
                          const float *wcat, const float *b1, const float *b2, const float *b3, float *out, int out_stride,
                          int out_col, int out_is_zero, void *stream);
+int prcnn_sa_wide_fused3_panels(int b, int n, int m, int c0, int c1, int c2, int c3, long max_tiles, const float *F, const float *wxyz,
+                                const unsigned int *rowinfo, const float *rowdxyz, const int *tilecloud, const unsigned int *hdr,
+                                const float *wcat_panels, const float *b1, const float *b2, const float *b3, float *out, int out_stride,
+                                int out_col, int out_is_zero, void *stream);
 
 typedef struct prcnn_gather_problem {
     int b, n, c1; long max_tiles; const float *P; const float *wxyz; const unsigned int *rowinfo; const float *rowdxyz;
@@ -129,6 +133,7 @@
     const unsigned int *hdr; long rows; long max_tiles; int K, N, n_store; const float *A; long lda; const float *W;
     const float *bias; int relu; float *out; long ldo;
     int b, m; const unsigned int *rowinfo; const int *tilecloud; int out_col, out_is_zero;
+    int w_panels;
 } prcnn_layer_problem;
 typedef struct prcnn_sa_problem {
     int b, n, m, c3; long max_tiles; const float *P; const float *wxyz; const unsigned int *rowinfo; const float *rowdxyz;
@@ -150,6 +155,9 @@
 int prcnn_packed_layer_interp(long rows, int K, int N, const float *A, long lda, const float *W, const float *bias, int relu,
                               float *out, long ldo, int n_per_cloud, int m_known, const float *G, long ldg, const int *idx,
                               const float *weight, void *stream);
+int prcnn_packed_layer_interp_panels(long rows, int K, int N, const float *A, long lda, const float *Wpanels, const float *bias, int relu,
+                                     float *out, long ldo, int n_per_cloud, int m_known, const float *G, long ldg, const int *idx,
+                                     const float *weight, void *stream);
 int prcnn_sa_xyz_mlp_packed(int b, int m, int c1, int c2, int c3, long max_tiles, const unsigned int *rowinfo,
                             const float *rowdxyz, const int *tilecloud, const unsigned int *hdr, const float *w1,
                             const float *b1, const float *w2, const float *b2, const float *w3, const float *b3,
```
